# relife957/FastApriori

Hardware: AMD Instinct MI355X
Metric: itemsets/sec (mining wall-clock), T10I4D100M min_sup=0.001 (higher is better)
Workload: dtype int32/uint64-bitmap (exact integer counts); 1 GPU; model=T10I4D100M, global_batch=100000000, parallelism=dp1, n_itemsets=33139, min_count=100000

## Files before the change

### csrc/hip/count.hip

```cpp
#include <algorithm>
#include <cstdlib>

#include "fa_hip.h"
#include "../host/fa_dl.h"
#include "../host/fa_limits.h"
#include "../host/fa_slab.h"

namespace fa {

constexpr int kPB = 128;

__device__ __forceinline__ void tri_index(int pid, int nb, int& bi, int& bj) {
  bi = 0;
  int rem = pid;
  while (rem >= nb - bi) { rem -= nb - bi; ++bi; }
  bj = bi + rem;
}

__device__ __forceinline__ int64_t lower_bound_i32(const int32_t* __restrict__ a, int64_t lo, int64_t hi,
                                                   int32_t key) {
  while (lo < hi) {
    int64_t mid = (lo + hi) >> 1;
    if (a[mid] < key) lo = mid + 1; else hi = mid;
  }
// ... 959 lines not shown
        const uint32_t v = (uint32_t)(acc[i][j][g] + 0.5f);
        if (row < col && col < F1 && v) atomicAdd(&out[(int64_t)row * F1 + col], v * scale);
      }
}

constexpr int kWPT = 8;

template <bool kWeighted>
__global__ __launch_bounds__(256) void k_count_candidates(
    const uint64_t* __restrict__ bm, int64_t Wp, int64_t W, const int32_t* __restrict__ prefix, int m,
    const int64_t* __restrict__ ext_off, const int32_t* __restrict__ ext,
    const int32_t* __restrict__ gb_start, int ngb, const int32_t* __restrict__ wword,
    uint32_t* __restrict__ out) {
  __shared__ uint32_t acc[kMaxBlockExt];
  const uint32_t logical = xcd_remap(blockIdx.x, gridDim.x);
  const int gb = logical % ngb;
  const int64_t sc = logical / ngb;
  const int g0 = gb_start[gb], g1 = gb_start[gb + 1];
  const int64_t e_base = ext_off[g0];
  const int n_ext = (int)(ext_off[g1] - e_base);
  for (int i = threadIdx.x; i < n_ext; i += blockDim.x) acc[i] = 0;
  const int64_t w0 = sc * (256 * kWPT) + threadIdx.x;
  bool valid[kWPT];
  int32_t wt[kWPT];
#pragma unroll
  for (int q = 0; q < kWPT; ++q) {
    valid[q] = w0 + q * 256 < W;
    wt[q] = (kWeighted && valid[q]) ? wword[w0 + q * 256] : 1;
  }
  __syncthreads();
  for (int g = g0; g < g1; ++g) {
    uint64_t p[kWPT];
    const int32_t* pr = prefix + (int64_t)g * m;
    {
      const uint64_t* row = bm + (int64_t)pr[0] * Wp + w0;
#pragma unroll
      for (int q = 0; q < kWPT; ++q) p[q] = valid[q] ? row[q * 256] : 0ull;
    }
    for (int j = 1; j < m; ++j) {
      const uint64_t* row = bm + (int64_t)pr[j] * Wp + w0;
#pragma unroll
      for (int q = 0; q < kWPT; ++q) p[q] &= valid[q] ? row[q * 256] : 0ull;
    }
    for (int64_t e = ext_off[g]; e < ext_off[g + 1]; ++e) {
      const uint64_t* row = bm + (int64_t)ext[e] * Wp + w0;
      uint32_t s = 0;
#pragma unroll
      for (int q = 0; q < kWPT; ++q) {
        const uint64_t v = valid[q] ? (p[q] & row[q * 256]) : 0ull;
        if (kWeighted) s += popc64_acc(v, 0) * (uint32_t)wt[q];
        else s = popc64_acc(v, s);
      }
      s = wave_sum_u32(s);
      if (lane_id() == 0 && s) atomicAdd(&acc[e - e_base], s);
    }
  }
  __syncthreads();
  for (int i = threadIdx.x; i < n_ext; i += blockDim.x)
    if (acc[i]) atomicAdd(&out[e_base + i], acc[i]);
}

enum { kBuildCols = 0, kBuildContig = 1, kBuildBM = 2 };

struct MapGlobal {
  const int32_t* __restrict__ p;
  __device__ __forceinline__ int operator()(int r) const { return p[r]; }
};
struct MapLds {
  const uint16_t* p;
  __device__ __forceinline__ int operator()(int r) const {
    const int v = p[r];
    return v == 0xFFFF ? -1 : v;
  }
};

struct WordSpan {
  int64_t st, base, end;
};
__device__ __forceinline__ WordSpan word_span(const int64_t* __restrict__ roff, int64_t col0, int64_t ncols) {
  const int lane = threadIdx.x & 63;
  return WordSpan{roff[min(col0 + lane, ncols)], roff[col0], roff[min(col0 + 64, ncols)]};
}

template <class Map>
__device__ __forceinline__ void slab_build_word_span(uint64_t* __restrict__ slab, int swp, int q, const WordSpan& ws,
                                                     const int32_t* __restrict__ ranks, Map item_map, int h,
                                                     int nsub, unsigned long long* words, int swz);

template <class Map = MapGlobal>
__device__ __forceinline__ void slab_build_word_m(uint64_t* __restrict__ slab, int swp, int q, int64_t col0,
                                                  int64_t ncols, const int64_t* __restrict__ roff,
                                                  const int32_t* __restrict__ ranks, Map item_map, int h,
                                                  int nsub, unsigned long long* words, int swz = 0) {
  slab_build_word_span(slab, swp, q, word_span(roff, col0, ncols), ranks, item_map, h, nsub, words, swz);
}

template <class Map>
__device__ __forceinline__ void slab_build_word_span(uint64_t* __restrict__ slab, int swp, int q, const WordSpan& ws,
                                                     const int32_t* __restrict__ ranks, Map item_map, int h,
                                                     int nsub, unsigned long long* words, int swz) {
  const int lane = threadIdx.x & 63;
  const int64_t st = ws.st, base = ws.base, end = ws.end;
  const int srel = (int)(st - base);
  const int n = (int)(end - base);
  const unsigned long long le = lanes_le_mask();
  constexpr int U = 2;
  const int step = 64 * U * nsub;
  int rn[U], rn2[U];
#pragma unroll
  for (int u = 0; u < U; ++u) {
    const int p = 64 * U * h + 64 * u + lane;
    rn[u] = p < n ? ranks[base + p] : -1;
    rn2[u] = p + step < n ? ranks[base + p + step] : -1;
  }
  for (int p0 = 64 * U * h; p0 < n; p0 += step) {
    int r[U];
#pragma unroll
    for (int u = 0; u < U; ++u) {
      r[u] = rn[u];
      rn[u] = rn2[u];
      const int p = p0 + 2 * step + 64 * u + lane;
      rn2[u] = p < n ? ranks[base + p] : -1;
    }
    const int cs0 = __popcll(__ballot(srel < p0));
    unsigned long long S[U];
    window_starts<U>(words, srel, p0, S);
    int cs = cs0;
#pragma unroll
    for (int u = 0; u < U; ++u) {
      const int l = cs + __popcll(S[u] & le) - 1;
      const int uu = r[u] >= 0 ? item_map(r[u]) : -1;
      if (uu >= 0) atomicOr((unsigned long long*)(slab + (size_t)uu * swp + (q ^ ((uu << 2) & swz))), 1ull << l);
      cs += __popcll(S[u]);
    }
  }
}

__device__ __forceinline__ void slab_build_word(uint64_t* __restrict__ slab, int swp, int q, int64_t col0,
                                                int64_t ncols, const int64_t* __restrict__ roff,
                                                const int32_t* __restrict__ ranks,
                                                const int32_t* __restrict__ item_map, int h, int nsub,
                                                unsigned long long* words, int swz = 0) {
  slab_build_word_m(slab, swp, q, col0, ncols, roff, ranks, MapGlobal{item_map}, h, nsub, words, swz);
}

template <int SW, int ROWW, bool kSwz>
__device__ __forceinline__ void slab_copy_bm(uint4* lds4, int n_used, const uint64_t* __restrict__ bm, int64_t Wp,
                                             const int32_t* __restrict__ bm_rows, int64_t w0, int64_t W) {
  constexpr int QW = SW / 2;
  constexpr int KMAX = 4;
  const int total = n_used * QW;
  for (int base = 0; base < total; base += KMAX * kSlabThreads) {
    int32_t br[KMAX];
    uint4 v[KMAX];
#pragma unroll
    for (int k = 0; k < KMAX; ++k) {
      const int i = base + (int)threadIdx.x + k * kSlabThreads;
      br[k] = i < total ? (bm_rows ? bm_rows[i / QW] : i / QW) : 0;
    }
#pragma unroll
    for (int k = 0; k < KMAX; ++k) {
      const int i = base + (int)threadIdx.x + k * kSlabThreads;
      const int64_t w = w0 + 2 * (i % QW);
      v[k] = make_uint4(0, 0, 0, 0);
      const int64_t at = Wp > 0 ? (int64_t)br[k] * Wp + w : (w >> 3) * -Wp + (int64_t)br[k] * 8 + (w & 7);
      if (i < total && w < W) v[k] = *reinterpret_cast<const uint4*>(bm + at);
    }
#pragma unroll
    for (int k = 0; k < KMAX; ++k) {
      const int i = base + (int)threadIdx.x + k * kSlabThreads;
      if (i < total) {
        const int u = i / QW, q = i % QW;
        const int qq = kSwz ? (q ^ (((u << 2) & (SW - 4)) >> 1)) : q;
        lds4[(size_t)u * (ROWW / 2) + qq] = v[k];
      }
    }
  }
}

constexpr int kMapLdsMax = kSlabMapMaxF1;

__device__ __forceinline__ uint32_t bcnt_acc(uint32_t x, uint32_t acc) {
  uint32_t r;
  __asm__("v_bcnt_u32_b32 %0, %1, %2" : "=v"(r) : "v"(x), "v"(acc));
  return r;
}

__device__ __forceinline__ uint32_t and3(uint32_t a, uint32_t b, uint32_t c) {
  return __builtin_amdgcn_bitop3_b32(a, b, c, 0x80);
}

__device__ __forceinline__ int u16_at(const int4& v, int k) {
  const int w = (k >> 1) == 0 ? v.x : (k >> 1) == 1 ? v.y : (k >> 1) == 2 ? v.z : v.w;
  return (k & 1) ? (int)((uint32_t)w >> 16) : (w & 0xFFFF);
}

template <int SW, bool kWeighted, int kBuild, bool kCls = false, int kAccB = 4>
__global__ __launch_bounds__(kSlabThreads) void k_count_slab_rec(
    const int64_t* __restrict__ roff, const int32_t* __restrict__ ranks, const int32_t* __restrict__ src,
    int64_t ncols, const int32_t* __restrict__ item_map, int F1, int n_used, const int32_t* __restrict__ gpre,
    const int4* __restrict__ rec, int G_arg, int C, const int32_t* __restrict__ wword, uint32_t* __restrict__ out,
    const uint64_t* __restrict__ bm, int64_t Wp, const int32_t* __restrict__ bm_rows, int flags,
    const int32_t* __restrict__ g_dev) {
  const int G = g_dev ? *g_dev : G_arg;
  extern __shared__ uint4 lds4[];
  __shared__ unsigned long long build_words[kSlabThreads / 64 * 2];
  constexpr int SWP = SW + 2;
  constexpr int RS = SWP / 2;
  uint64_t* slab = reinterpret_cast<uint64_t*>(lds4);
  static_assert(kAccB == 4 || kAccB == 2 || kAccB == 1, "accumulator bytes");
  constexpr bool acc16 = !kWeighted && kAccB == 2;
  constexpr bool acc8 = !kWeighted && kAccB == 1;
  const int nacc = acc16 ? (C + 1) >> 1 : acc8 ? (C + 3) >> 2 : C;
  constexpr int kFlush16 = 65535 / (SW * 64);
  uint32_t* acc = reinterpret_cast<uint32_t*>(slab + (size_t)n_used * SWP);
  uint8_t* acc8p = reinterpret_cast<uint8_t*>(acc);
  uint16_t* smap = reinterpret_cast<uint16_t*>(acc + ((nacc + 3) & ~3));
  const bool map_lds = kBuild == kBuildContig && F1 <= kMapLdsMax;
  for (int i = threadIdx.x; i < nacc; i += blockDim.x) acc[i] = 0;
  if (map_lds) {
    for (int i = threadIdx.x; i < F1; i += blockDim.x) {
      const int v = item_map[i];
      smap[i] = v < 0 ? (uint16_t)0xFFFF : (uint16_t)v;
    }
  }
  const int64_t W = (ncols + 63) >> 6;
  const int64_t nslabs = (W + SW - 1) / SW;
  const int4 z4 = make_int4(0, 0, 0, 0);
  const int ppart = (flags >> kSlabFlagPartShift) & kSlabFlagPartMask;
  const int npart = ((flags >> kSlabFlagNpartsShift) & kSlabFlagPartMask) + 1;
  const int gstep = kSlabThreads * npart;
  const int g0 = (ppart + npart * (int)(threadIdx.x >> 6)) * 64 + (int)(threadIdx.x & 63);
  int4 ra = z4, rb = z4, rc = z4;
  if (g0 < G) { ra = rec[3 * g0]; rb = rec[3 * g0 + 1]; rc = rec[3 * g0 + 2]; }

  auto and_row = [&](uint4 (&p)[SW / 2], int u) {
    const uint4* r = lds4 + (size_t)u * RS;
#pragma unroll
    for (int q = 0; q < SW / 2; ++q) {
      const uint4 v = r[q];
      p[q].x &= v.x; p[q].y &= v.y; p[q].z &= v.z; p[q].w &= v.w;
    }
  };
  auto and_row2 = [&](uint4 (&p)[SW / 2], int u, int w) {
    const uint4* r = lds4 + (size_t)u * RS;
    const uint4* t = lds4 + (size_t)w * RS;
#pragma unroll
    for (int q = 0; q < SW / 2; ++q) {
      const uint4 v = r[q], x = t[q];
      p[q].x = and3(p[q].x, v.x, x.x); p[q].y = and3(p[q].y, v.y, x.y);
      p[q].z = and3(p[q].z, v.z, x.z); p[q].w = and3(p[q].w, v.w, x.w);
    }
  };
  auto pid = [&](int j) { return j < 4 ? u16_at(ra, 4 + j) : u16_at(rc, j - 4); };
  auto and_prefix = [&](uint4 (&p)[SW / 2], int j0, int j1) {
#pragma unroll
    for (int j = 1; j < 12; j += 2) {
      if (j >= j0 && j < j1) {
        if (j + 1 < j1) and_row2(p, pid(j), pid(j + 1));
        else and_row(p, pid(j));
      }
    }
  };
  auto acc_add = [&](int e, uint32_t v) {
    if (acc8) {
      uint32_t t = (uint32_t)acc8p[e] + v;
      if (t > 255u) { atomicAdd(&out[e], t); t = 0; }
      acc8p[e] = (uint8_t)t;
    } else if (acc16) {
      atomicAdd(&acc[e >> 1], v << ((e & 1) << 4));
    } else {
      atomicAdd(&acc[e], v);
    }
  };
  auto flush = [&]() {
    for (int i = threadIdx.x; i < nacc; i += blockDim.x) {
      const uint32_t v = acc[i];
      if (!v) continue;
      if (acc8) {
#pragma unroll
        for (int b = 0; b < 4; ++b) {
          const uint32_t c = (v >> (8 * b)) & 0xFFu;
          if (c && 4 * i + b < C) atomicAdd(&out[4 * i + b], c);
        }
        acc[i] = 0;
      } else if (acc16) {
        if (v & 0xFFFFu) atomicAdd(&out[2 * i], v & 0xFFFFu);
        if ((v >> 16) && 2 * i + 1 < C) atomicAdd(&out[2 * i + 1], v >> 16);
        acc[i] = 0;
      } else {
        atomicAdd(&out[i], v);
      }
    }
  };
  int nsl = 0;
  constexpr int kNW = kSlabThreads / 64;
  constexpr bool kOneWord = kBuild == kBuildContig && SW <= 8 && SW * (kNW > SW ? kNW / SW : 1) == kNW;
  const int my_q = (int)(threadIdx.x >> 6) / (kNW > SW ? kNW / SW : 1);
  WordSpan span{0, 0, 0};
  auto load_span = [&](int64_t sb_) {
    const int64_t col0 = (sb_ * SW + my_q) * 64;
    if (kOneWord && sb_ < nslabs && col0 < ncols) span = word_span(roff, col0, ncols);
  };
  load_span(blockIdx.x);

  for (int64_t sb = blockIdx.x; sb < nslabs; sb += gridDim.x) {
    const int64_t w0 = sb * SW;
    __syncthreads();
    if (acc16 && ++nsl > kFlush16) {
      flush();
      nsl = 1;
    }
    if (kBuild == kBuildBM) {
      slab_copy_bm<SW, SWP, false>(lds4, n_used, bm, Wp, bm_rows, w0, W);
    } else {
      {
        const uint4 z = make_uint4(0, 0, 0, 0);
        for (int i = threadIdx.x; i < n_used * RS; i += blockDim.x) lds4[i] = z;
      }
      __syncthreads();
      if (kBuild == kBuildContig) {
        constexpr int NW = kSlabThreads / 64;
        constexpr int NSUB = NW > SW ? NW / SW : 1;
        const int wv = threadIdx.x >> 6;
        if (kOneWord) {
          const int q = wv / NSUB;
          if ((w0 + q) * 64 < ncols) {
            if (map_lds)
              slab_build_word_span(slab, SWP, q, span, ranks, MapLds{smap}, wv % NSUB, NSUB, build_words + wv * 2, 0);
            else
              slab_build_word_span(slab, SWP, q, span, ranks, MapGlobal{item_map}, wv % NSUB, NSUB,
                                   build_words + wv * 2, 0);
          }
        } else {
          for (int q = wv / NSUB; q < SW; q += NW / NSUB) {
            if ((w0 + q) * 64 >= ncols) continue;
            if (map_lds)
              slab_build_word_m(slab, SWP, q, (w0 + q) * 64, ncols, roff, ranks, MapLds{smap}, wv % NSUB, NSUB,
                                build_words + wv * 2);
            else
              slab_build_word_m(slab, SWP, q, (w0 + q) * 64, ncols, roff, ranks, MapGlobal{item_map}, wv % NSUB,
                                NSUB, build_words + wv * 2);
          }
        }
      } else {
        for (int j = threadIdx.x; j < SW * 64; j += blockDim.x) {
          const int64_t col = w0 * 64 + j;
          if (col >= ncols) break;
          const int64_t row = src ? (int64_t)src[col] : col;
          if (row < 0) continue;
          const unsigned long long bit = 1ull << (j & 63);
          uint64_t* base = slab + (j >> 6);
          for (int64_t r = roff[row], r1 = roff[row + 1]; r < r1; ++r) {
            const int uu = item_map[ranks[r]];
            if (uu >= 0) atomicOr((unsigned long long*)(base + (size_t)uu * SWP), bit);
          }
        }
      }
    }
    __syncthreads();
    load_span(sb + gridDim.x);
    uint32_t wt[SW];
#pragma unroll
    for (int q = 0; q < SW; ++q) wt[q] = kWeighted ? ((w0 + q < W) ? (uint32_t)wword[w0 + q] : 0u) : 1u;
    uint4 p[SW / 2], qv[SW / 2];
    for (int g = g0; g < G; g += gstep) {
      const int gn = g + gstep < G ? g + gstep : g0;
      const int4 na = rec[3 * gn], nb = rec[3 * gn + 1], nc = rec[3 * gn + 2];
      const int n_ext = ra.y & 0xFF, m = (ra.y >> 8) & 0xFF;
      if constexpr (kCls) {
        const int fl = (ra.y >> 17) & 3;
        if (!(fl & 1)) {
          const uint4* r0 = lds4 + (size_t)(ra.z & 0xFFFF) * RS;
#pragma unroll
          for (int q = 0; q < SW / 2; ++q) qv[q] = r0[q];
          and_prefix(qv, 1, m - 1);
        }
        if (!(fl & 2)) {
          const uint4* rl = lds4 + (size_t)((uint32_t)ra.y >> 19) * RS;
#pragma unroll
          for (int q = 0; q < SW / 2; ++q) {
            const uint4 v = rl[q];
            p[q].x = qv[q].x & v.x; p[q].y = qv[q].y & v.y; p[q].z = qv[q].z & v.z; p[q].w = qv[q].w & v.w;
          }
        }
      } else {
      {
        const uint4* r0 = lds4 + (size_t)(ra.z & 0xFFFF) * RS;
#pragma unroll
        for (int q = 0; q < SW / 2; ++q) p[q] = r0[q];
      }
      if (!((ra.y >> 16) & 1)) {
        and_prefix(p, 1, m);
      } else {
        const int32_t* pr = gpre + rc.x;
        int j = 1;
        for (; j + 1 < m; j += 2) and_row2(p, pr[j], pr[j + 1]);
        if (j < m) and_row(p, pr[j]);
      }
      }
      uint32_t any = flags & kSlabFlagDense;
      if (!any) {
#pragma unroll
        for (int q = 0; q < SW / 2; ++q) any |= p[q].x | p[q].y | p[q].z | p[q].w;
      }
      if (any) {
        const int e0 = ra.x;
        constexpr int UE = SW <= 8 ? 2 : 1;
#pragma unroll
        for (int k = 0; k < 8; k += UE) {
          if (k >= n_ext) break;
          uint32_t s[UE];
          const uint4* r[UE];
#pragma unroll
          for (int x = 0; x < UE; ++x) {
            s[x] = 0;
            r[x] = lds4 + (size_t)u16_at(rb, k + x < n_ext ? k + x : k) * RS;
          }
#pragma unroll
          for (int q = 0; q < SW / 2; ++q) {
#pragma unroll
            for (int x = 0; x < UE; ++x) {
              const uint4 v = r[x][q];
              if (kWeighted) {
                s[x] += (uint32_t)(__popc(p[q].x & v.x) + __popc(p[q].y & v.y)) * wt[2 * q] +
                        (uint32_t)(__popc(p[q].z & v.z) + __popc(p[q].w & v.w)) * wt[2 * q + 1];
              } else {
                s[x] = bcnt_acc(p[q].x & v.x, s[x]); s[x] = bcnt_acc(p[q].y & v.y, s[x]);
                s[x] = bcnt_acc(p[q].z & v.z, s[x]); s[x] = bcnt_acc(p[q].w & v.w, s[x]);
              }
            }
          }
#pragma unroll
          for (int x = 0; x < UE; ++x)
            if (k + x < n_ext && s[x]) acc_add(e0 + k + x, s[x]);
        }
      }
      ra = na; rb = nb; rc = nc;
    }
  }
  __syncthreads();
  flush();
}

struct MapIdent {
  __device__ __forceinline__ int operator()(int r) const { return r; }
};

constexpr int kBwThreads = 1024;

template <class Map>
__global__ __launch_bounds__(kBwThreads) void k_build_bitmaps_w(const int64_t* __restrict__ roff,
                                                         const int32_t* __restrict__ ranks, int64_t ncols, int F1,
                                                         int64_t rs, int64_t bs, int WT, uint64_t* __restrict__ bm,
                                                         Map map) {
  extern __shared__ uint64_t btile[];
  __shared__ unsigned long long bwords[kBwThreads / 64 * 2];
  for (int i = threadIdx.x; i < F1 * WT; i += blockDim.x) btile[i] = 0ull;
  __syncthreads();
  const int wv = threadIdx.x >> 6;
  constexpr int NW = kBwThreads / 64;
  const int nsub = NW > WT ? NW / WT : 1;
  for (int q = wv / nsub; q < WT; q += NW / nsub) {
    const int64_t col0 = ((int64_t)blockIdx.x * WT + q) * 64;
    if (col0 < ncols)
      slab_build_word_span(btile, WT, q, word_span(roff, col0, ncols), ranks, map, wv % nsub, nsub, bwords + wv * 2,
                           0);
  }
  __syncthreads();
  const int64_t w0 = (int64_t)blockIdx.x * WT;
  for (int i = threadIdx.x; i < F1 * WT; i += blockDim.x) {
    const int u = i / WT, w = i - u * WT;
    bm[((w0 + w) >> 3) * bs + (int64_t)u * rs + ((w0 + w) & 7)] = btile[i];
  }
}

}

using namespace fa;

FA_API int fa_hip_build_bitmaps_wave(const int64_t* roff, const int32_t* ranks, int64_t ncols, int32_t F1, int64_t Wp,
                                     int WT, uint64_t* bm, const int32_t* item_map, int blocked, hipStream_t st) {
  const size_t lds = (size_t)F1 * WT * 8;
  if (F1 <= 0 || WT <= 0 || Wp % WT || Wp % 8 || lds > 64 * 1024) return 2;
  const int64_t rs = blocked ? 8 : Wp, bs = blocked ? 8 * (int64_t)F1 : 8;
  dim3 g((unsigned)(Wp / WT));
  if (item_map) {
    (void)hipFuncSetAttribute((const void*)k_build_bitmaps_w<MapGlobal>, hipFuncAttributeMaxDynamicSharedMemorySize,
                              (int)lds);
    hipLaunchKernelGGL(k_build_bitmaps_w<MapGlobal>, g, dim3(kBwThreads), lds, st, roff, ranks, ncols, F1, rs, bs, WT, bm,
                       MapGlobal{item_map});
  } else {
    (void)hipFuncSetAttribute((const void*)k_build_bitmaps_w<MapIdent>, hipFuncAttributeMaxDynamicSharedMemorySize,
                              (int)lds);
    hipLaunchKernelGGL(k_build_bitmaps_w<MapIdent>, g, dim3(kBwThreads), lds, st, roff, ranks, ncols, F1, rs, bs, WT, bm,
                       MapIdent{});
  }
  FA_LAUNCH_RET();
}


FA_API int fa_hip_pair_gram_mfma(const uint64_t* bm, int32_t F1, int64_t rs, int64_t bs, int woff, int64_t W,
                                 uint32_t* out, int target_wgs, uint32_t scale, int fp4, hipStream_t st) {
  if (woff < 0 || woff > 7) return -22;
  const BmView v{bm, rs, bs, woff};
  if (W <= 0 || F1 < 2) return 0;
  const int nt = (F1 + kMT4 - 1) / kMT4;
  const int ntp = nt * (nt + 1) / 2;
  int64_t nk = std::max<int64_t>(1, (target_wgs + ntp - 1) / ntp);
  int64_t kchunk = (W + nk - 1) / nk;
  kchunk = std::max<int64_t>(kMW, (kchunk + kMW - 1) / kMW * kMW);
  if (fp4) kchunk = std::min<int64_t>(kchunk, (int64_t)1 << 18);
  nk = (W + kchunk - 1) / kchunk;
  if (fp4)
    hipLaunchKernelGGL(k_pair_gram_fp4, dim3((unsigned)(nk * ntp)), dim3(256), 0, st, v, F1, W, nt,
                       ntp, kchunk, out, scale);
  else
    hipLaunchKernelGGL(k_pair_gram_mfma4<false>, dim3((unsigned)(nk * ntp)), dim3(256), 0, st, v, F1, W, nt,
                       ntp, kchunk, out, scale);
  FA_LAUNCH_RET();
}

FA_API int fa_hip_pair_gram_popc(const uint64_t* bm, int32_t F1, int64_t rs, int64_t bs, int woff, int64_t W,
                                 const int32_t* wword, uint32_t* out, int target_wgs, hipStream_t st) {
  if (woff < 0 || woff > 7) return -22;
  if (W <= 0 || F1 < 2) return 0;
  const BmView v{bm, rs, bs, woff};
  const int nt = (F1 + kGT - 1) / kGT;
  const int ntp = nt * (nt + 1) / 2;
  int64_t nk = std::max<int64_t>(1, (target_wgs + ntp - 1) / ntp);
  int64_t kchunk = (W + nk - 1) / nk;
  kchunk = std::max<int64_t>(kGK, (kchunk + kGK - 1) / kGK * kGK);
  nk = (W + kchunk - 1) / kchunk;
  dim3 g((unsigned)(nk * ntp));
  if (wword)
    hipLaunchKernelGGL(k_pair_gram_popc<true>, g, dim3(256), 0, st, v, F1, W, wword, nt, ntp, kchunk, out);
  else
    hipLaunchKernelGGL(k_pair_gram_popc<false>, g, dim3(256), 0, st, v, F1, W, wword, nt, ntp, kchunk, out);
  FA_LAUNCH_RET();
}

FA_API int fa_hip_count_candidates(const uint64_t* bm, int64_t Wp, int64_t W, const int32_t* prefix,
                                   int m, const int64_t* ext_off, const int32_t* ext,
                                   const int32_t* gb_start, int ngb, const int32_t* wword,
                                   uint32_t* out, hipStream_t st) {
  if (ngb <= 0 || W <= 0) return 0;
  const int64_t nsc = (W + 256 * kWPT - 1) / (256 * kWPT);
  dim3 g((unsigned)(nsc * ngb));
  if (wword)
    hipLaunchKernelGGL(k_count_candidates<true>, g, dim3(256), 0, st, bm, Wp, W, prefix, m, ext_off, ext, gb_start, ngb, wword, out);
// ... 74 lines not shown
  {
    uint64_t m = m0, mk = ~m0 << 1;
#pragma unroll
    for (int i = 0; i < 6; ++i) {
      uint64_t mp = mk ^ (mk << 1);
      mp ^= mp << 2; mp ^= mp << 4; mp ^= mp << 8; mp ^= mp << 16; mp ^= mp << 32;
      mv[i] = mp & m;
      m = (m ^ mv[i]) | (mv[i] >> (1 << i));
      mk &= ~mp;
    }
  }
  for (int u0 = 0; u0 < n_items; u0 += kWinBatch) {
    const int nb = min(kWinBatch, n_items - u0);
    uint64_t x[kWinBatch];
#pragma unroll
    for (int b = 0; b < kWinBatch; ++b) x[b] = (n && b < nb) ? bm_word(bm, ld, rows[u0 + b], q) : 0ull;
    for (int i = lane; i < nb * 66; i += 64) (&buf[0][0])[i] = 0ull;
    wave_lds_sync();
    if (n) {
      const int w = s >> 6, sh = s & 63;
#pragma unroll
      for (int b = 0; b < kWinBatch; ++b) {
        if (b >= nb) break;
        uint64_t y = x[b] & m0;
#pragma unroll
        for (int i = 0; i < 6; ++i) {
          const uint64_t t = y & mv[i];
          y = (y ^ t) | (t >> (1 << i));
        }
        atomicOr(&buf[b][w], (unsigned long long)(y << sh));
        if (sh + n > 64) atomicOr(&buf[b][w + 1], (unsigned long long)(y >> (64 - sh)));
      }
    }
    wave_lds_sync();
    for (int b = 0; b < nb; ++b) {
      const int64_t u = u0 + b;
      for (int j = lane; j < nwords; j += 64) {
        const unsigned long long v = buf[b][j];
        const int64_t gw = w0 + j;
        uint64_t* o = ldo > 0 ? out + u * ldo + gw : out + (gw >> 3) * -ldo + u * 8 + (gw & 7);
        if (j == 0 || j == nwords - 1) {
          if (v) atomicOr(reinterpret_cast<unsigned long long*>(o), v);
        } else {
          *o = v;
        }
      }
    }
    wave_lds_sync();
  }
}

FA_API int fa_hip_win_alive(const uint64_t* bm, int64_t ld, const int32_t* rows, int n_items, int64_t W, int k,
                            uint64_t* alive, int32_t* cnt, hipStream_t st) {
  if (W <= 0) return 0;
  int planes = 1;
  while ((1 << planes) <= n_items) ++planes;
  if (n_items < 1 || planes > kWinPlanes || k < 1 || ld == 0) return 1;
  hipLaunchKernelGGL(k_win_alive, dim3((unsigned)((W + 255) / 256)), dim3(256), 0, st, bm, ld, rows, n_items, W, k,
                     planes, alive, cnt);
  FA_LAUNCH_RET();
}

FA_API int fa_hip_win_compact(const uint64_t* bm, int64_t ld, const int32_t* rows, int n_items, int64_t W,
                              const uint64_t* alive, const int64_t* off, uint64_t* out, int64_t ldo, hipStream_t st) {
  if (W <= 0 || n_items < 1) return 0;
  if (ld == 0 || ldo == 0) return 1;
  hipLaunchKernelGGL(k_win_compact, dim3((unsigned)((W + 255) / 256)), dim3(256), 0, st, bm, ld, rows, n_items, W,
                     alive, off, out, ldo);
  FA_LAUNCH_RET();
}

static int g_slab_max_wg = 0;
FA_API void fa_hip_debug_slab_max_wg(int n) { g_slab_max_wg = n; }
static int g_piece_part = 0, g_piece_nparts = 1;
FA_API int fa_hip_set_piece_part(int part, int nparts) {
  if (nparts < 1 || nparts > 256 || part < 0 || part >= nparts) return 1;
  g_piece_part = part;
  g_piece_nparts = nparts;
  return 0;
}

FA_API int fa_hip_count_slab_rec_cls(const int64_t* roff, const int32_t* ranks, const int32_t* src, int64_t ncols,
                                     const int32_t* item_map, int F1, int n_used, const int32_t* gpre,
                                     const void* rec, int G, int C, const int32_t* wword, uint32_t* out, int sw,
                                     int n_wg, const uint64_t* bm, int64_t Wp, hipStream_t st,
                                     const int32_t* bm_rows, const int32_t* g_dev, int cls) {
  if ((G <= 0 && !g_dev) || C <= 0 || ncols <= 0) return 0;
  if (g_piece_nparts > 1) cls &= ~kSlabCls;
  const int accb = slab_mode_acc_bytes(cls, wword != nullptr);
  const bool acc16 = accb == 2;
  const int64_t n_acc = slab_acc_count(C, accb);
  const bool contig = !bm && !src;
  const size_t lds = (size_t)slab_kernel_lds(n_used, sw, slab_acc_words(n_acc), contig ? slab_map_lds(F1) : 0);
  if (lds > 160 * 1024 - 256) return 3;
  if (g_slab_max_wg > 0) n_wg = std::min(n_wg, g_slab_max_wg);
  using KernT = void (*)(const int64_t*, const int32_t*, const int32_t*, int64_t, const int32_t*, int, int,
                         const int32_t*, const int4*, int, int, const int32_t*, uint32_t*, const uint64_t*, int64_t,
                         const int32_t*, int, const int32_t*);
  KernT kern = nullptr;
#define FA_REC_MODE(S, B)                                                                              \
  kern = wword ? (KernT)k_count_slab_rec<S, true, B>                                                   \
         : (cls & kSlabCls) ? (accb == 1 ? (KernT)k_count_slab_rec<S, false, B, true, 1>               \
                               : accb == 2 ? (KernT)k_count_slab_rec<S, false, B, true, 2>             \
                                           : (KernT)k_count_slab_rec<S, false, B, true, 4>)            \
                            : (accb == 1 ? (KernT)k_count_slab_rec<S, false, B, false, 1>              \
                               : accb == 2 ? (KernT)k_count_slab_rec<S, false, B, false, 2>            \
                                           : (KernT)k_count_slab_rec<S, false, B, false, 4>);
#define FA_REC_CASE(S)                                    \
  if (sw == S) {                                          \
    if (bm) { FA_REC_MODE(S, kBuildBM) }                  \
    else if (src) { FA_REC_MODE(S, kBuildCols) }          \
    else { FA_REC_MODE(S, kBuildContig) }                 \
  }
  FA_REC_CASE(4)
  FA_REC_CASE(8)
  FA_REC_CASE(16)
  FA_REC_CASE(32)
#undef FA_REC_CASE
#undef FA_REC_MODE
  if (!kern) return 1;
  (void)hipFuncSetAttribute((const void*)kern, hipFuncAttributeMaxDynamicSharedMemorySize, (int)lds);
  const int flags = ((cls & kSlabDense) ? kSlabFlagDense : 0) | (acc16 ? kSlabFlagAcc16 : 0) |
                    (g_piece_part << kSlabFlagPartShift) | ((g_piece_nparts - 1) << kSlabFlagNpartsShift);
  hipLaunchKernelGGL(kern, dim3((unsigned)n_wg), dim3(kSlabThreads), lds, st, roff, ranks, src, ncols, item_map, F1,
                     n_used, gpre, (const int4*)rec, G, C, wword, out, bm, Wp, bm_rows, flags, g_dev);
  FA_LAUNCH_RET();
}

FA_API int fa_hip_block_counts(const int64_t* roff, const int32_t* ranks, int64_t T, int32_t F1, uint8_t* cnt,
                               int64_t* bsum, int pb, hipStream_t st) {
  if (T <= 0) return 0;
  const int nb = (F1 + pb - 1) / pb;
  const int64_t nbatch = (T + 63) / 64;
  const int lpb = __builtin_ctz((unsigned)pb);
  if (nb <= kWBMaxNB && (1 << lpb) == pb)
    hipLaunchKernelGGL(k_block_counts_w, dim3((unsigned)((nbatch + 3) / 4)), dim3(256), 0, st, roff, ranks, T, nb,
                       cnt, bsum, nbatch, lpb);
  else
    hipLaunchKernelGGL(k_block_counts, dim3((unsigned)((nbatch + 3) / 4)), dim3(256), 0, st, roff, ranks, T, nb, cnt,
                       bsum, nbatch, pb);
  FA_LAUNCH_RET();
}

FA_API int fa_hip_block_scatter(const int64_t* roff, const int32_t* ranks, int64_t T, int32_t F1,
                                const uint8_t* cnt, const int64_t* base, uint8_t* lr, int pb, hipStream_t st) {
  if (T <= 0) return 0;
  const int nb = (F1 + pb - 1) / pb;
  const int64_t nbatch = (T + 63) / 64;
  const int lpb = __builtin_ctz((unsigned)pb);
  if (nb <= kWBMaxNB && (1 << lpb) == pb)
    hipLaunchKernelGGL(k_block_scatter_w, dim3((unsigned)((nbatch + 3) / 4)), dim3(256), 0, st, roff, ranks, T, nb,
                       cnt, base, nbatch, lr, lpb);
  else
    hipLaunchKernelGGL(k_block_scatter, dim3((unsigned)((nbatch + 3) / 4)), dim3(256), 0, st, roff, ranks, T, nb, cnt,
                       base, nbatch, lr, pb);
  FA_LAUNCH_RET();
}

FA_API int fa_hip_pair_blocked(const uint8_t* cnt, const int64_t* base, const uint8_t* lr, int64_t T,
                               const int32_t* wrow, int32_t F1, uint32_t* out, int64_t chunk_rows, hipStream_t st) {
  if (T <= 0 || F1 < 2) return 0;
  const int nb = (F1 + kPB - 1) / kPB;
  const int nbp = nb * (nb + 1) / 2;
  const int64_t nbatch = (T + 63) / 64;
  const int64_t chunk_b = std::max<int64_t>(kPW, (chunk_rows + 63) / 64);
  const int64_t nch = (nbatch + chunk_b - 1) / chunk_b;
  hipLaunchKernelGGL(k_pair_blocked, dim3((unsigned)(nch * nbp)), dim3(64 * kPW), 0, st, cnt, base, lr, T, nbatch,
                     wrow, F1, nb, nbp, chunk_b, out);
  FA_LAUNCH_RET();
}

FA_API int fa_hip_pair_queue16(const uint8_t* cnt, const int64_t* base, const uint8_t* lr, int64_t T, int32_t F1,
                               int64_t ld, int* qctr, uint32_t* out, int n_wg, hipStream_t st) {
  if (T <= 0 || F1 < 2) return 0;
  const int nb = (F1 + kPB16 - 1) / kPB16;
  const int nbp = nb * (nb + 1) / 2;
  const int64_t nbatch = (T + 63) / 64;
  const int nsub = (int)((nbatch + kQSubB - 1) / kQSubB);
  if (n_wg <= 0) {
    int dev = 0, ncu = 256;
    if (hipGetDevice(&dev) == hipSuccess) hipDeviceGetAttribute(&ncu, hipDeviceAttributeMultiprocessorCount, dev);
    n_wg = ncu;
  }
  n_wg = (int)std::min<int64_t>(n_wg, (int64_t)nsub * nbp);
  hipLaunchKernelGGL(k_pair_queue16, dim3((unsigned)n_wg), dim3(64 * kPW), 0, st, cnt, base, lr, T, nbatch, F1, ld,
                     nb, nbp, qctr, nsub, out);
  FA_LAUNCH_RET();
}

FA_API int fa_hip_pairs_compact(const uint32_t* pc, int64_t ld, int32_t F1, int64_t mc, int32_t* row_cnt,
                                int64_t* row_off, int32_t* rows, int32_t* cnt, int64_t* n_out, hipStream_t st) {
  if (F1 < 2) return 1;
  hipLaunchKernelGGL(k_pairs_keep_count, dim3((unsigned)F1), dim3(256), 0, st, pc, ld, F1, mc, row_cnt);
  hipLaunchKernelGGL(k_pairs_scan, dim3(1), dim3(1024), 0, st, row_cnt, F1, row_off, n_out);
  hipLaunchKernelGGL(k_pairs_emit, dim3((unsigned)F1), dim3(256), 0, st, pc, ld, F1, mc, row_off, rows, cnt);
  FA_LAUNCH_RET();
}
```

### csrc/hip/gen.hip

```cpp
#include <hipcub/hipcub.hpp>

#include <algorithm>
#include <cmath>

#include "fa_hip.h"
#include "../host/fa_dl.h"
#include "../host/fa_limits.h"
#include "../host/fa_slab.h"

namespace fa {

__device__ __forceinline__ uint64_t ag_mix(uint64_t x) {
  x ^= x >> 33; x *= 0xff51afd7ed558ccdull; x ^= x >> 33; x *= 0xc4ceb9fe1a85ec53ull; x ^= x >> 33;
  return x;
}

__device__ __forceinline__ uint64_t ag_hash_drop(const int32_t* __restrict__ r, int m, int skip) {
  uint64_t h = 0x9E3779B97F4A7C15ull ^ (uint64_t)(m - 1);
  for (int q = 0; q < m; ++q)
    if (q != skip) h = ag_mix(h ^ (uint32_t)r[q]);
  return h;
}

__device__ __forceinline__ bool ag_eq_drop(const int32_t* __restrict__ a, const int32_t* __restrict__ b, int m,
// ... 618 lines not shown
    nz += v[u] > 0;
  }
  const int tz[2] = {t, nz};
  int64_t pre[2], tot[2];
  wg_scan_excl<16>(tz, wpart, pre, tot);
  int64_t run = pre[0];
#pragma unroll
  for (int u = 0; u < 4; ++u) {
    const int64_t i = b0 + 4 * (int64_t)threadIdx.x + u;
    run += v[u];
    if (i < n) off[i + 1] = run;
  }
  if (threadIdx.x == 0) {
    bs[blockIdx.x] = tot[0];
    bs[nblk + blockIdx.x] = tot[1];
  }
}

__global__ __launch_bounds__(1024) void k_ds_decide0(int64_t* __restrict__ off, long long* __restrict__ c,
                                                     int64_t* __restrict__ bs, int nblk, int64_t c_bound) {
  if (c[kDlStop]) return;
  __shared__ int64_t part[16];
  if (threadIdx.x == 0) off[0] = 0;
  int64_t z = 0;
  const int64_t C = wg_scan_chunks<16>(
      nblk, 0, part, [&](int64_t q) { return bs[q]; },
      [&](int64_t q, int64_t before, int64_t) {
        bs[2 * nblk + q] = before;
        z += bs[nblk + q];
      });
  const int64_t gz = wg_sum<16>(z, part);
  if (threadIdx.x != 0) return;
  c[kDlCl] = C;
  c[kDlGl] = gz;
  if (C == 0) { c[kDlEnd] = 1; c[kDlStop] = 1; return; }
  if (C > c_bound) { c[kDlMulti] = 1; c[kDlStop] = 1; return; }
  c[kDlLevels] = 1; c[kDlTotal] = C; c[kDlLastC] = C; c[kDlNl + 1] = C;
}

__global__ __launch_bounds__(1024) void k_ds_add(int64_t* __restrict__ off, const long long* __restrict__ c,
                                                 const int64_t* __restrict__ bs, int nblk) {
  if (c[kDlOverBound]) return;
  const int64_t n = c[kDlNl];
  const int64_t b0 = (int64_t)blockIdx.x * kDsBlk;
  if (b0 >= n || blockIdx.x == 0) return;
  const int64_t base = bs[2 * nblk + blockIdx.x];
  for (int k = threadIdx.x; k < kDsBlk; k += 1024) {
    const int64_t i = b0 + k;
    if (i < n) off[i + 1] += base;
  }
}

__global__ __launch_bounds__(256) void k_dl_mark(const int32_t* __restrict__ rows, int m1,
                                                 long long* __restrict__ c, int w32) {
  __shared__ uint32_t lb[2 * kDlBitsW];
  if (c[kDlStop] && !c[kDlMulti]) return;
  for (int q = threadIdx.x; q < w32; q += 256) lb[q] = 0u;
  __syncthreads();
  const int64_t n = c[kDlMulti] ? 0 : c[kDlCl] * (int64_t)m1;
  for (int64_t i = (int64_t)blockIdx.x * 256 + threadIdx.x; i < n; i += (int64_t)gridDim.x * 256)
    atomicOr(&lb[rows[i] >> 5], 1u << (rows[i] & 31));
  __syncthreads();
  uint32_t* mk = reinterpret_cast<uint32_t*>(c + kDlBits);
  for (int q = threadIdx.x; q < w32; q += 256)
    if (lb[q]) atomicOr(&mk[q], lb[q]);
}

__global__ __launch_bounds__(64) void k_dl_post0(long long* __restrict__ c, double lds, double accb, int w32) {
  if (blockIdx.x != 0) return;
  const uint32_t* mk = reinterpret_cast<const uint32_t*>(c + kDlBits);
  uint32_t part = 0;
  for (int q = threadIdx.x; q < w32; q += 64) part += __popc(mk[q]);
  const int64_t n_used = (int64_t)wave_sum_u32(part);
  if (threadIdx.x != 0) return;
  c[kDlNUsed] = n_used;
  if (c[kDlLevels] == 1 && c[kDlCl] > slab_cap(n_used, c[kDlCl], lds, accb)) {
    c[kDlMulti] = 1;
    c[kDlStop] = 1;
  }
}

__global__ __launch_bounds__(1024) void k_dl_decide(const int32_t* __restrict__ cnt, int64_t* __restrict__ off,
                                                     long long* __restrict__ c, int l, double growth, int64_t c_bound,
                                                     double lds, double accb) {
  if (c[kDlStop]) return;
  int64_t g = 0;
  const int64_t C = agd_block_scan<true>(cnt, off, c[kDlNl + l], &g);
  if (threadIdx.x != 0) return;
  const int64_t total = c[kDlTotal], last = c[kDlLastC];
  if (C == 0 || (double)C > growth * (double)last || C > c_bound ||
      total + C > slab_cap(c[kDlNUsed], total + C, lds, accb)) {
    c[kDlStop] = 1;
    if (C == 0) c[kDlEmpty] = 1;
    return;
  }
  c[kDlCl + l] = C;
  c[kDlGl + l] = g;
  c[kDlLevels] = l + 1;
  c[kDlTotal] = total + C;
  c[kDlLastC] = C;
  c[kDlNl + l + 1] = C;
}

template <bool kEmit, int NWL = 1>
__global__ __launch_bounds__(256) void k_dl_rows(const int32_t* __restrict__ P, int m,
                                                 const int32_t* __restrict__ table, uint32_t mask, int nw,
                                                 const unsigned long long* __restrict__ ext, int32_t* __restrict__ cnt,
                                                 const int64_t* __restrict__ off, int32_t* __restrict__ rows,
                                                 const long long* __restrict__ c, int l, int32_t* __restrict__ ntab,
                                                 uint32_t ncap, unsigned long long* __restrict__ next_ext) {
  if (c[kDlStop]) return;
  const int64_t n = c[kDlNl + l];
  if (!kEmit && ntab) {
    const int64_t stride = (int64_t)gridDim.x * blockDim.x;
    for (int64_t q = (int64_t)blockIdx.x * blockDim.x + threadIdx.x; q < (int64_t)ncap; q += stride) ntab[q] = -1;
  }
  const int lane = threadIdx.x & 63;
  const int64_t nwave = (int64_t)gridDim.x * (blockDim.x / 64);
  for (int64_t i = (int64_t)blockIdx.x * (blockDim.x / 64) + (threadIdx.x >> 6); i < n; i += nwave) {
    unsigned long long a[NWL];
    const int cc = ag_row_bits<NWL>(P, i, m, table, mask, nw, ext, lane, a);
    const int incl = wave_scan_incl_dpp(cc);
    if (!kEmit) {
      if (lane == 63) cnt[i] = incl;
      continue;
    }
    const int64_t o = off[i];
    ag_emit<NWL>(a, lane, P + i * m, m, o + (incl - cc), cnt + n, rows);
    if (next_ext && wave_last(incl) > 0) {
#pragma unroll
      for (int j = 0; j < NWL; ++j)
        if (lane * NWL + j < nw) next_ext[o * nw + lane * NWL + j] = a[j];
      if (lane == 0) {
        const int32_t* x = P + i * m;
        uint64_t h = 0x9E3779B97F4A7C15ull ^ (uint64_t)m;
        for (int q = 0; q < m; ++q) h = ag_mix(h ^ (uint32_t)x[q]);
        uint32_t at = (uint32_t)h & (ncap - 1);
        while (atomicCAS(&ntab[at], -1, (int32_t)o) != -1) at = (at + 1) & (ncap - 1);
      }
    }
  }
}

}

FA_API int fa_hip_dl_level0(const int32_t* P0, const long long* n_src, int64_t n_const, int64_t n_bound, int m0,
                            int F1, void* ws, int64_t ws_bytes, long long* ctl, long long* ctl_host,
                            int64_t c_bound, double lds, double accb, int64_t* info, int sync, hipStream_t st) {
  if (m0 < 2 || F1 > kAgMaxF1 || F1 < 1 || n_bound < 0 || c_bound < 1) return 1;
  auto al = [](int64_t b) { return (b + 255) & ~(int64_t)255; };
  const int nw = (F1 + 63) / 64;
  const int64_t nb = std::max<int64_t>(n_bound, 1);
  uint32_t cap = 16;
  while (cap < 2 * (uint64_t)nb) cap <<= 1;
  const int nds = nb > 4 * kDsBlk ? (int)((nb + kDsBlk - 1) / kDsBlk) : 0;
  const int64_t need = al(4 * (int64_t)cap) + al(8 * nb * nw) + al(8 * (nb + 1)) + al(4 * (nb + c_bound)) +
                       al(4 * c_bound * (m0 + 1)) + al(8 * 3 * (int64_t)nds);
  info[0] = need;
  if (need > ws_bytes) return 5;
  char* w = static_cast<char*>(ws);
  int32_t* table = reinterpret_cast<int32_t*>(w); w += al(4 * (int64_t)cap);
  unsigned long long* ext = reinterpret_cast<unsigned long long*>(w); w += al(8 * nb * nw);
  int64_t* off = reinterpret_cast<int64_t*>(w); w += al(8 * (nb + 1));
  int32_t* cnt = reinterpret_cast<int32_t*>(w); w += al(4 * (nb + c_bound));
  int32_t* rows = reinterpret_cast<int32_t*>(w); w += al(4 * c_bound * (m0 + 1));
  int64_t* ds = reinterpret_cast<int64_t*>(w);
  info[1] = (int64_t)(intptr_t)cnt; info[2] = (int64_t)(intptr_t)off; info[3] = (int64_t)(intptr_t)rows;
  hipLaunchKernelGGL(k_dl_setup0, dim3(1), dim3(kDlCtl), 0, st, ctl, n_src, n_const, m0 + 1, nb);
  AgdClear clr{};
  clr.p[0] = reinterpret_cast<uint32_t*>(table); clr.len[0] = cap; clr.val[0] = ~0u;
  clr.p[1] = reinterpret_cast<uint32_t*>(ext); clr.len[1] = 2 * nb * nw; clr.val[1] = 0u;
  clr.nreg = 2;
  const int64_t clr_max = std::max<int64_t>(cap, 2 * nb * nw);
  hipLaunchKernelGGL(k_agd_clear, dim3((unsigned)std::min<int64_t>((clr_max + 255) / 256, 1024)), dim3(256), 0, st,
                     clr, ctl);
  const dim3 g((unsigned)std::min<int64_t>((nb + 255) / 256, 512));
  hipLaunchKernelGGL(k_agd_insert, g, dim3(256), 0, st, P0, m0, table, cap - 1, ctl, 0);
  hipLaunchKernelGGL(k_agd_ext, g, dim3(256), 0, st, P0, m0, table, cap - 1, nw, ext, ctl, 0);
  const unsigned nwg = (unsigned)std::min<int64_t>((nb + 3) / 4, 2048);
#define FA_DL0_ROWS(E, N)                                                                                   \
  hipLaunchKernelGGL((k_agd_rows<E, N>), dim3(nwg), dim3(256), 0, st, P0, m0, table, cap - 1, nw, ext, cnt, off, \
                     rows, ctl, 0);
#define FA_DL0_CNT(N) FA_DL0_ROWS(false, N)
#define FA_DL0_EMIT(N) FA_DL0_ROWS(true, N)
  FA_AG_NWL_SWITCH(nw, FA_DL0_CNT)
  if (nds) {
    hipLaunchKernelGGL(k_ds_blocks, dim3((unsigned)nds), dim3(1024), 0, st, cnt, off, ctl, ds, nds);
    hipLaunchKernelGGL(k_ds_decide0, dim3(1), dim3(1024), 0, st, off, ctl, ds, nds, c_bound);
    hipLaunchKernelGGL(k_ds_add, dim3((unsigned)nds), dim3(1024), 0, st, off, ctl, ds, nds);
  } else {
    hipLaunchKernelGGL(k_dl_decide0, dim3(1), dim3(1024), 0, st, cnt, off, ctl, c_bound);
  }
  FA_AG_NWL_SWITCH(nw, FA_DL0_EMIT)
#undef FA_DL0_EMIT
#undef FA_DL0_CNT
#undef FA_DL0_ROWS
  const int w32 = (F1 + 31) / 32;
  hipLaunchKernelGGL(k_dl_mark, dim3((unsigned)std::min<int64_t>((c_bound * (m0 + 1) + 255) / 256, 1024)), dim3(256),
                     0, st, rows, m0 + 1, ctl, w32);
  hipLaunchKernelGGL(k_dl_post0, dim3(1), dim3(64), 0, st, ctl, lds, accb, w32);
  if (sync) {
    (void)hipMemcpyAsync(ctl_host, ctl, sizeof(long long) * kDlCtl, hipMemcpyDeviceToHost, st);
    if (hipStreamSynchronize(st) != hipSuccess) return 7;
  }
  FA_LAUNCH_RET();
}

static void dl_post(DlPost* P, const DlDesc* desc, int L, long long* ctl, const long long* ch, int F1,
                    double accb_rule, hipStream_t st) {
  P->done = 0;
  if (ch[kDlStop] && ch[kDlLevels] == 0) return;
  if (ch[kDlOverBound] || ch[kDlMulti] || ch[kDlEnd] || L < 1) return;
  int64_t C = 0, R = 0;
  for (int l = 0; l < L; ++l) { C += desc[l].C; R += desc[l].n; }
  const int64_t n_used = ch[kDlNUsed];
  P->C = C;
  if (C < 1 || C > P->rec_cap || C > P->out_cap || 8 * ((R + 255) / 256) > P->part_cap) return;
  int64_t cap = 0;
  int sw = slab_width(n_used, C, P->lds_budget, accb_rule, &cap);
  if (sw == 0 || C > cap) return;
  double accb = accb_rule;
  if (!P->wword) slab_acc_upgrade(n_used, C, P->lds_budget, P->accb, &sw, &cap, &accb);
  P->accb = accb;
  if (fa_hip_dl_plan(desc, L, ctl, F1, P->item_map, P->rec, C, P->part, P->part_cap, P->gpre, P->gpre_cap, sw,
                     st) != 0)
    return;
  (void)hipMemsetAsync(P->out, 0, 4 * (size_t)C, st);
  P->sw = sw;
  P->cap = cap;
  P->done = 1;
  P->trim = 0;
  if (!P->trim_ok || P->T <= 0) {
  } else if (!P->len_hist || P->T < P->trim_min_rows) {
    if (!P->len_hist && P->T >= P->trim_min_rows) return;
  } else {
    const uint64_t* mk = reinterpret_cast<const uint64_t*>(ch + kDlBits);
    double num = 0.0, den = 0.0;
    for (int r = 0; r < F1; ++r) {
      if (P->alive[r]) den += (double)P->c1[r];
      if ((mk[r >> 6] >> (r & 63)) & 1ull) num += (double)P->c1[r];
    }
    if (den > 0.0) {
      double est_rows = 0.0, est_nnz = 0.0;
      trim_estimate(P->len_hist, kTrimHist, num / den, (int)P->k, &est_rows, &est_nnz);
      const double T = (double)std::max<int64_t>(P->T, 1), nnz = (double)std::max<int64_t>(P->nnz, 1);
      P->trim = (est_rows < P->trim_rows_frac * T || est_nnz < P->trim_nnz_frac * nnz) ? 1 : 0;
    }
  }
  if (P->trim) return;
  const int64_t W = (P->ncols + 63) / 64, nslabs = (W + sw - 1) / sw;
  const bool weighted = P->wword != nullptr;
  const int64_t nacc = slab_acc_count(C, slab_acc_bytes(P->accb, weighted));
  P->n_wg = slab_workgroups(nslabs, (int64_t)P->lds_kernel,
                            slab_kernel_lds(n_used, sw, slab_acc_words(nacc), slab_map_lds(F1)));
  if (fa_hip_count_slab_rec_cls(P->roff, P->ranks, P->src, P->ncols, P->item_map, F1, (int)n_used, P->gpre, P->rec,
                                0, (int)C, P->wword, P->out, sw, (int)P->n_wg, nullptr, 0, st, nullptr,
                                reinterpret_cast<const int32_t*>(ctl + kDlPiecesI32),
                                slab_acc_mode(P->accb, weighted)) != 0)
    return;
  P->done = 2;
}

FA_API int fa_hip_dl_more(int F1, void* ws, int64_t ws_bytes, int64_t ws_used, long long* ctl, long long* ctl_host,
                          double growth, int max_levels, double lds, double accb, int64_t n1_bound, fa::DlDesc* desc,
                          int64_t* info, hipStream_t st, void* post) {
  using namespace fa;
  auto al = [](int64_t b) { return (b + 255) & ~(int64_t)255; };
  const int nw = (F1 + 63) / 64;
  char* const w0 = static_cast<char*>(ws);
  char* w = w0 + ws_used;
  const int LM = std::min(max_levels, kDlMaxLevels);
  const int64_t acc_max = (int64_t)(lds / accb);
  int64_t nb = n1_bound;
  int m = (int)desc[0].m + 1;
  const int32_t* P = reinterpret_cast<const int32_t*>((intptr_t)desc[0].rows);
  struct Lv { int32_t* cnt; int64_t* off; int32_t* rows; int m; };
  Lv lv[kDlMaxL];
  static long long* mirror = nullptr;
  static hipEvent_t ev[2];
  if (!mirror) {
    if (hipHostMalloc(reinterpret_cast<void**>(&mirror), 2 * sizeof(long long) * kDlCtl) != hipSuccess) return 7;
    for (int k = 0; k < 2; ++k) (void)hipEventCreateWithFlags(&ev[k], hipEventDisableTiming);
  }
  int nbatch = 0;
  struct Tab { int32_t* table = nullptr; uint32_t cap = 0; unsigned long long* ext = nullptr; };
  Tab cur;
  auto tab_alloc = [&](int64_t rows, Tab& t) -> bool {
    uint32_t cap = 16;
    while (cap < 2 * (uint64_t)rows) cap <<= 1;
    const int64_t need = al(4 * (int64_t)cap) + al(8 * rows * nw);
    if ((w - w0) + need > ws_bytes) { info[0] = 2 * ((w - w0) + need); return false; }
    t.table = reinterpret_cast<int32_t*>(w); w += al(4 * (int64_t)cap);
    t.ext = reinterpret_cast<unsigned long long*>(w); w += al(8 * rows * nw);
    t.cap = cap;
    return true;
  };
  auto enqueue = [&](int l0) -> int {
    const int l1 = std::min(LM - 1, l0 + kAgdBatch - 1);
    for (int l = l0; l <= l1; ++l) {
      const int64_t cb = std::min<int64_t>(acc_max, (int64_t)(growth * (double)nb) + 1);
      if (l == 1) {
        if (!tab_alloc(nb, cur)) return 5;
        AgdClear clr{};
        clr.p[0] = reinterpret_cast<uint32_t*>(cur.table); clr.len[0] = cur.cap; clr.val[0] = ~0u;
        clr.p[1] = reinterpret_cast<uint32_t*>(cur.ext); clr.len[1] = 2 * nb * nw; clr.val[1] = 0u;
        clr.nreg = 2;
        const int64_t clr_max = std::max<int64_t>(cur.cap, 2 * nb * nw);
        hipLaunchKernelGGL(k_agd_clear, dim3((unsigned)std::min<int64_t>((clr_max + 255) / 256, 1024)), dim3(256), 0,
                           st, clr, ctl);
        const dim3 g((unsigned)std::min<int64_t>((nb + 255) / 256, 512));
        hipLaunchKernelGGL(k_agd_insert, g, dim3(256), 0, st, P, m, cur.table, cur.cap - 1, ctl, l);
        hipLaunchKernelGGL(k_agd_ext, g, dim3(256), 0, st, P, m, cur.table, cur.cap - 1, nw, cur.ext, ctl, l);
      }
      const int64_t need = al(8 * (nb + 1)) + al(4 * (nb + cb)) + al(4 * cb * (m + 1));
      if ((w - w0) + need > ws_bytes) {
        info[0] = 2 * ((w - w0) + need);
        return 5;
      }
      lv[l].off = reinterpret_cast<int64_t*>(w); w += al(8 * (nb + 1));
      lv[l].cnt = reinterpret_cast<int32_t*>(w); w += al(4 * (nb + cb));
      lv[l].rows = reinterpret_cast<int32_t*>(w); w += al(4 * cb * (m + 1));
      lv[l].m = m;
      Tab nxt;
      if (l + 1 < LM && !tab_alloc(cb, nxt)) return 5;
      const unsigned nwg = (unsigned)std::min<int64_t>((nb + 3) / 4, 2048);
#define FA_DLR(E, N)                                                                                          \
      hipLaunchKernelGGL((k_dl_rows<E, N>), dim3(nwg), dim3(256), 0, st, P, m, cur.table, cur.cap - 1, nw,      \
                         cur.ext, lv[l].cnt, lv[l].off, lv[l].rows, ctl, l, nxt.table, nxt.cap, nxt.ext);
#define FA_DLR_CNT(N) FA_DLR(false, N)
#define FA_DLR_EMIT(N) FA_DLR(true, N)
      FA_AG_NWL_SWITCH(nw, FA_DLR_CNT)
      hipLaunchKernelGGL(k_dl_decide, dim3(1), dim3(1024), 0, st, lv[l].cnt, lv[l].off, ctl, l, growth, cb, lds,
                         accb);
      FA_AG_NWL_SWITCH(nw, FA_DLR_EMIT)
#undef FA_DLR_EMIT
#undef FA_DLR_CNT
#undef FA_DLR
      P = lv[l].rows;
      cur = nxt;
      nb = cb;
      ++m;
    }
    long long* hb = mirror + (nbatch & 1) * kDlCtl;
    (void)hipMemcpyAsync(hb, ctl, sizeof(long long) * kDlCtl, hipMemcpyDeviceToHost, st);
    (void)hipEventRecord(ev[nbatch & 1], st);
    ++nbatch;
    return 0;
  };
  int next = 1;
  int rc = 0;
  for (int q = 0; q < 2 && next < LM && rc == 0; ++q, next += kAgdBatch) rc = enqueue(next);
  for (int waited = 0; rc == 0 && waited < nbatch; ++waited) {
    if (hipEventSynchronize(ev[waited & 1]) != hipSuccess) return 7;
    if (mirror[(waited & 1) * kDlCtl + kDlStop]) break;
    if (next < LM) { rc = enqueue(next); next += kAgdBatch; }
  }
  (void)hipMemcpyAsync(ctl_host, ctl, sizeof(long long) * kDlCtl, hipMemcpyDeviceToHost, st);
  if (hipStreamSynchronize(st) != hipSuccess) return 7;
  if (rc) return rc;
  desc[0].n = ctl_host[kDlNl];
  desc[0].C = ctl_host[kDlCl];
  desc[0].base = 0;
  const int L = (int)ctl_host[kDlLevels];
  for (int l = 1; l < L; ++l) {
    DlDesc& d = desc[l];
    d.P = desc[l - 1].rows;
    d.cnt = (int64_t)(intptr_t)lv[l].cnt;
    d.off = (int64_t)(intptr_t)lv[l].off;
    d.rows = (int64_t)(intptr_t)lv[l].rows;
    d.m = lv[l].m;
    d.n = ctl_host[kDlNl + l];
    d.C = ctl_host[kDlCl + l];
    d.base = desc[l - 1].base + desc[l - 1].C;
  }
  info[0] = w - w0;
  if (post) dl_post(static_cast<DlPost*>(post), desc, L, ctl, ctl_host, F1, accb, st);
  FA_LAUNCH_RET();
}
```

### csrc/hip/levels.hip

```cpp
#include "fa_hip.h"
#include "../host/fa_dl.h"

namespace fa {

struct DlLevels {
  const int32_t* P[kDlMaxL];
  const int32_t* cnt[kDlMaxL];
  const int64_t* off[kDlMaxL];
  const int32_t* rows[kDlMaxL];
  int64_t n[kDlMaxL];
  int64_t C[kDlMaxL];
  int64_t base[kDlMaxL];
  int64_t rbase[kDlMaxL + 1];
  int m[kDlMaxL];
  int64_t gbase[kDlMaxL];
  int32_t* gpre;
  int64_t w0, w1;
  int L;
};

__device__ __forceinline__ int dl_level_of(const DlLevels& D, int64_t t) {
  int l = 0;
  while (l + 1 < D.L && t >= D.rbase[l + 1]) ++l;
  return l;
}

__global__ __launch_bounds__(64) void k_dl_map(const uint64_t* __restrict__ mk, int F1, int32_t* __restrict__ item_map) {
  __shared__ int pre[kDlBitsW];
  const int lane = threadIdx.x;
  const int nwd = (F1 + 63) >> 6;
  int cnt8[8], tot = 0;
#pragma unroll
  for (int j = 0; j < 8; ++j) {
    const int w = lane * 8 + j;
    cnt8[j] = w < nwd ? __popcll(mk[w]) : 0;
    tot += cnt8[j];
  }
  int run = wave_scan_incl_dpp(tot) - tot;
#pragma unroll
  for (int j = 0; j < 8; ++j) {
    pre[lane * 8 + j] = run;
    run += cnt8[j];
  }
  __syncthreads();
  for (int r = lane; r < F1; r += 64) {
    const uint64_t ww = mk[r >> 6];
    const int b = r & 63;
    item_map[r] = ((ww >> b) & 1ull) ? pre[r >> 6] + __popcll(ww & ((1ull << b) - 1ull)) : -1;
  }
}

constexpr int kDlPB = 256;

__device__ __forceinline__ int dl_bucket_count(int cc, int b) { return b == 8 ? (cc >> 3) : ((cc & 7) == b ? 1 : 0); }

__device__ __forceinline__ int dl_row_window(const DlLevels& D, int64_t t, int64_t R, int64_t* first) {
  if (t >= R) return 0;
  const int l = dl_level_of(D, t);
  const int64_t i = t - D.rbase[l];
  const int cc = D.cnt[l][i];
  if (cc == 0) return 0;
  const int64_t cb = D.base[l] + D.off[l][i], ce = cb + cc;
  const int64_t a = cb > D.w0 ? cb : D.w0, b = ce < D.w1 ? ce : D.w1;
  if (first) *first = a;
  return b > a ? (int)(b - a) : 0;
}

__device__ __forceinline__ int dl_row_count(const DlLevels& D, int64_t t, int64_t R) {
  return dl_row_window(D, t, R, nullptr);
}

__global__ __launch_bounds__(kDlPB) void k_dl_pieces_count(const DlLevels D, int32_t* __restrict__ part) {
  __shared__ int sh[8 * (kDlPB / 64)];
  const int64_t R = D.rbase[D.L];
  const int64_t t = (int64_t)blockIdx.x * kDlPB + threadIdx.x;
  const int cc = dl_row_count(D, t, R);
  int v[8], tot[8];
#pragma unroll
  for (int b = 1; b <= 8; ++b) v[b - 1] = dl_bucket_count(cc, b);
  wg_sum<kDlPB / 64>(v, sh, tot);
  if (threadIdx.x == 0) {
#pragma unroll
    for (int b = 0; b < 8; ++b) part[(int64_t)blockIdx.x * 8 + b] = tot[b];
  }
// ... 23 lines not shown
  for (int k = 0; k < 8; ++k) e8[k] = k < n_ext ? item_map[ex[k]] : 0;
  int4 a, b, cc;
  a.x = (int)cand;
  a.y = n_ext | (m << 8) | (goff >= 0 ? 1 << 16 : 0);
  a.z = (int)dl_pk(ids[0], ids[1]);
  a.w = (int)dl_pk(ids[2], ids[3]);
  b.x = (int)dl_pk(e8[0], e8[1]); b.y = (int)dl_pk(e8[2], e8[3]);
  b.z = (int)dl_pk(e8[4], e8[5]); b.w = (int)dl_pk(e8[6], e8[7]);
  cc.x = (int)dl_pk(ids[4], ids[5]); cc.y = (int)dl_pk(ids[6], ids[7]);
  cc.z = (int)dl_pk(ids[8], ids[9]); cc.w = (int)dl_pk(ids[10], ids[11]);
  if (goff >= 0) cc.x = (int)goff;
  rec[3 * p] = a; rec[3 * p + 1] = b; rec[3 * p + 2] = cc;
}

__global__ __launch_bounds__(kDlPB) void k_dl_pieces_emit(const DlLevels D, const int32_t* __restrict__ part,
                                                          const int32_t* __restrict__ item_map,
                                                          int4* __restrict__ rec) {
  __shared__ int sh[8 * (kDlPB / 64)];
  const int64_t R = D.rbase[D.L];
  const int64_t t = (int64_t)blockIdx.x * kDlPB + threadIdx.x;
  int64_t first = 0;
  const int cc = dl_row_window(D, t, R, &first);
  int v[8], excl[8], tot[8];
#pragma unroll
  for (int b = 1; b <= 8; ++b) v[b - 1] = dl_bucket_count(cc, b);
  wg_scan_excl<kDlPB / 64>(v, sh, excl, tot);
  if (cc == 0) return;
  int64_t slot[9];
#pragma unroll
  for (int b = 1; b <= 8; ++b) slot[b] = (int64_t)part[(int64_t)blockIdx.x * 8 + (b - 1)] + excl[b - 1];
  const int l = dl_level_of(D, t);
  const int64_t i = t - D.rbase[l];
  const int m = D.m[l];
  const int32_t* x = D.P[l] + i * m;
  int ids[kDlInline];
#pragma unroll
  for (int q = 0; q < kDlInline; ++q) ids[q] = q < m ? item_map[x[q]] : 0;
  int64_t goff = -1;
  if (m > kDlInline) {
    goff = D.gbase[l] + i * m;
    for (int q = 0; q < m; ++q) D.gpre[goff + q] = item_map[x[q]];
  }
  const int64_t o = D.off[l][i] + (first - (D.base[l] + D.off[l][i]));
  const int32_t* ex = D.cnt[l] + D.n[l] + o;
  const int64_t cand = first - D.w0;
  const int full = cc >> 3;
  for (int j = 0; j < full; ++j)
    dl_write_rec(rec, slot[8] + j, cand + 8 * j, 8, m, ids, ex + 8 * j, item_map, goff);
  const int rem = cc & 7;
  if (rem) dl_write_rec(rec, slot[rem], cand + 8 * full, rem, m, ids, ex + 8 * full, item_map, goff);
}

constexpr int kLaWs = 4;
constexpr int kLaMaxPos = kDlInline + 8;

__device__ __forceinline__ int la_u16(const int4& v, int k) {
  const int w = (k >> 1) == 0 ? v.x : (k >> 1) == 1 ? v.y : (k >> 1) == 2 ? v.z : v.w;
  return (k & 1) ? (int)((uint32_t)w >> 16) : (w & 0xFFFF);
}

__device__ __forceinline__ int la_row(const int4& a, const int4& b, const int4& c, int m, int pos) {
  if (pos < m) return pos < 4 ? la_u16(a, 4 + pos) : la_u16(c, pos - 4);
  return la_u16(b, pos - m);
}

__device__ __forceinline__ int la_row_min(int v) {
  v = min(v, __builtin_amdgcn_update_dpp(v, v, 0x128, 0xf, 0xf, false));
  v = min(v, __builtin_amdgcn_update_dpp(v, v, 0x124, 0xf, 0xf, false));
  v = min(v, __builtin_amdgcn_update_dpp(v, v, 0x122, 0xf, 0xf, false));
  v = min(v, __builtin_amdgcn_update_dpp(v, v, 0x121, 0xf, 0xf, false));
  return v;
}

__device__ __forceinline__ int la_qsum(int v) {
  const auto a = __builtin_amdgcn_permlane16_swap(v, v, false, false);
  v = (int)a[0] + (int)a[1];
  const auto b = __builtin_amdgcn_permlane32_swap(v, v, false, false);
  return (int)b[0] + (int)b[1];
}

__global__ __launch_bounds__(64) void k_la_qsum_probe(int* out) { out[threadIdx.x] = la_qsum((int)threadIdx.x); }

__global__ __launch_bounds__(64) void k_dl_lane_assign(int4* __restrict__ rec, const long long* __restrict__ c,
                                                       int rs) {
  constexpr int NW = 64 * kLaWs, NG = 4 * kLaWs;
  constexpr int kPq = kLaMaxPos / 4;
  __shared__ int4 win[3 * NW];
  __shared__ uint16_t rws[NW][kLaMaxPos];
  __shared__ uint32_t st[kLaMaxPos][16][NG];
  __shared__ int16_t dst[NW];
  const int G = reinterpret_cast<const int32_t*>(c + kDlPiecesI32)[0];
  const int64_t base = (int64_t)blockIdx.x * NW;
  if (base + NW > G) return;
  const int lane = threadIdx.x;
  for (int i = lane; i < 3 * NW; i += 64) win[i] = rec[3 * base + i];
  for (int i = lane; i < NG * kLaMaxPos * 16; i += 64) (&st[0][0][0])[i] = 0xFFFFu;
  wave_lds_sync();
  const int y0 = win[0].y & 0x1FFFF;
  bool same = true;
  for (int i = lane; i < NW; i += 64) same = same && (win[3 * i].y & 0x1FFFF) == y0;
  if (__ballot(!same) != 0ull) return;
  const int n_ext = y0 & 0xFF, m = (y0 >> 8) & 0xFF;
  if ((y0 >> 16) || m > kDlInline || m + n_ext > kLaMaxPos) return;
  const int R = m + n_ext;
  for (int i = lane; i < NW; i += 64) {
    const int4 a = win[3 * i], b = win[3 * i + 1], cc = win[3 * i + 2];
    for (int pos = 0; pos < R; ++pos) rws[i][pos] = (uint16_t)la_row(a, b, cc, m, pos);
  }
  wave_lds_sync();
  const int g = lane & 15, q = lane >> 4;
  int fill = 0;
  int rn[kPq];
#pragma unroll
  for (int t = 0; t < kPq; ++t) {
    const int v = (int)rws[0][q + 4 * t < R ? q + 4 * t : 0];
    rn[t] = q + 4 * t < R ? v : -1;
  }
  for (int i = 0; i < NW; ++i) {
    int rr[kPq];
    uint32_t w[kPq];
#pragma unroll
    for (int t = 0; t < kPq; ++t) rr[t] = rn[t];
    const int i1 = i + 1 < NW ? i + 1 : i;
#pragma unroll
    for (int t = 0; t < kPq; ++t) {
      const int pos = q + 4 * t;
      const bool ok = pos < R;
      const int pc = ok ? pos : 0;
      const uint32_t sv = st[pc][(rr[t] * rs) & 15][g];
      const int rv = (int)rws[i1][pc];
      w[t] = ok ? sv : 0xFFFFu;
      rn[t] = ok ? rv : -1;
    }
    int cost = 0;
#pragma unroll
    for (int t = 0; t < kPq; ++t) {
      const int o = (int)(w[t] & 0xFFFF);
      if (o != 0xFFFF && o != rr[t]) cost += (int)(w[t] >> 16);
    }
    cost = la_qsum(cost);
    if (fill >= 16) cost = 1 << 20;
    const int win_g = la_row_min((cost << 4) | g) & 15;
    if (g == win_g) {
#pragma unroll
      for (int t = 0; t < kPq; ++t) {
        const int pos = q + 4 * t;
        const int o = (int)(w[t] & 0xFFFF);
        const uint32_t nv = o == 0xFFFF ? ((uint32_t)rr[t] | (1u << 16)) : (o != rr[t] ? w[t] + (1u << 16) : w[t]);
        if (pos < R) st[pos][(rr[t] * rs) & 15][g] = nv;
      }
      if (q == 0) {
        const int gg = g & 3, k = fill;
        const int l16 = gg == 0 ? (k < 4 ? k : k < 8 ? 8 + k : 12 + k)
                      : gg == 1 ? (k < 8 ? 4 + k : k < 12 ? 8 + k : 16 + k)
                      : gg == 2 ? 32 + (k < 4 ? k : k < 8 ? 8 + k : 12 + k)
                                : 32 + (k < 8 ? 4 + k : k < 12 ? 8 + k : 16 + k);
        dst[i] = (int16_t)(64 * (g >> 2) + l16);
      }
      ++fill;
    }
  }
  wave_lds_sync();
  for (int i = lane; i < NW; i += 64) {
    const int64_t d = base + dst[i];
    rec[3 * d] = win[3 * i]; rec[3 * d + 1] = win[3 * i + 1]; rec[3 * d + 2] = win[3 * i + 2];
  }
}

struct DlOut {
  int64_t rows_off[kDlMaxL];
  int64_t cnt_off[kDlMaxL];
};

__global__ __launch_bounds__(1024) void k_dl_threshold(const DlLevels D, const DlOut O,
                                                       const uint32_t* __restrict__ counts, int64_t mc,
                                                       int32_t* __restrict__ rows_out, int32_t* __restrict__ cnt_out,
                                                       long long* __restrict__ fsz) {
  __shared__ int part[16];
  for (int l = 0; l < D.L; ++l) {
    const int w = D.m[l] + 1;
    const uint32_t* cl = counts + D.base[l];
    const int32_t* src = D.rows[l];
    int32_t* ro = rows_out + O.rows_off[l];
    int32_t* co = cnt_out + O.cnt_off[l];
    uint32_t v;
    const int64_t kept = wg_scan_chunks<16>(
        D.C[l], 0, part, [&](int64_t e) { v = cl[e]; return (int64_t)v >= mc ? 1 : 0; },
        [&](int64_t e, int64_t at, int keep) {
          if (!keep) return;
          co[at] = (int32_t)v;
          for (int q = 0; q < w; ++q) ro[at * w + q] = src[e * w + q];
        });
    if (threadIdx.x == 0) fsz[l] = kept;
  }
}

constexpr int kThB = 1024;
struct DlThrBlk {
  int64_t blk_base[kDlMaxL + 1];
};

__device__ __forceinline__ int dlt_level(const DlThrBlk& B, int L, int64_t b) {
  int l = 0;
  while (l + 1 < L && b >= B.blk_base[l + 1]) ++l;
  return l;
}

__global__ __launch_bounds__(256) void k_dlt_count(const DlLevels D, const DlThrBlk B,
                                                   const uint32_t* __restrict__ counts, int64_t mc,
                                                   int32_t* __restrict__ part) {
  const int64_t b = blockIdx.x;
  const int l = dlt_level(B, D.L, b);
  const int64_t C = D.C[l], e0 = (b - B.blk_base[l]) * kThB;
  const uint32_t* cl = counts + D.base[l];
  uint32_t k = 0;
#pragma unroll
  for (int u = 0; u < kThB / 256; ++u) {
    const int64_t e = e0 + threadIdx.x + 256 * u;
    k += (e < C && (int64_t)cl[e] >= mc) ? 1u : 0u;
  }
  __shared__ uint32_t ws[4];
  k = wg_sum<4>(k, ws);
  if (threadIdx.x == 0) part[b] = (int32_t)k;
}

__global__ __launch_bounds__(1024) void k_dlt_scan(const DlThrBlk B, int L, int32_t* __restrict__ part,
                                                  long long* __restrict__ fsz) {
  __shared__ int wpart[16];
  for (int l = 0; l < L; ++l) {
    int32_t* pl = part + B.blk_base[l];
    const int64_t kept = wg_scan_chunks<16>(
        B.blk_base[l + 1] - B.blk_base[l], 0, wpart, [&](int64_t i) { return pl[i]; },
// ... 55 lines not shown
  int64_t g = 0;
  for (int l = 0; l < L; ++l) {
    const DlDesc& d = desc[l];
    D->P[l] = reinterpret_cast<const int32_t*>((intptr_t)d.P);
    D->cnt[l] = reinterpret_cast<const int32_t*>((intptr_t)d.cnt);
    D->off[l] = reinterpret_cast<const int64_t*>((intptr_t)d.off);
    D->rows[l] = reinterpret_cast<const int32_t*>((intptr_t)d.rows);
    D->m[l] = (int)d.m;
    D->n[l] = d.n;
    D->C[l] = d.C;
    D->base[l] = d.base;
    D->rbase[l + 1] = D->rbase[l] + d.n;
    if (D->m[l] < 1 || D->m[l] > kDlMaxM) return 1;
    D->gbase[l] = -1;
    if (D->m[l] > kDlInline) {
      D->gbase[l] = g;
      g += d.n * D->m[l];
    }
  }
  if (g > 0 && gpre_cap >= 0 && (gpre == nullptr || g > gpre_cap)) return 1;
  return 0;
}

}

using namespace fa;

FA_API int fa_hip_dl_plan_window(const DlDesc* desc, int L, long long* ctl, int F1, int32_t* item_map, void* rec,
                                 int64_t max_pieces, int32_t* part, int64_t part_cap, int32_t* gpre,
                                 int64_t gpre_cap, int64_t w0, int64_t w1, int sw, hipStream_t st);
FA_API int fa_hip_dl_plan_window_bits(const DlDesc* desc, int L, long long* ctl, int F1, const uint64_t* used_bits,
                                      int32_t* item_map, void* rec, int64_t max_pieces, int32_t* part,
                                      int64_t part_cap, int32_t* gpre, int64_t gpre_cap, int64_t w0, int64_t w1,
                                      int sw, hipStream_t st);

FA_API int fa_hip_debug_la_qsum(int* out, hipStream_t st) {
  hipLaunchKernelGGL(k_la_qsum_probe, dim3(1), dim3(64), 0, st, out);
  FA_LAUNCH_RET();
}

static int g_lane_on = 0;
FA_API void fa_hip_set_lane_deal(int on) { g_lane_on = on; }

FA_API int fa_hip_dl_plan(const DlDesc* desc, int L, long long* ctl, int F1, int32_t* item_map, void* rec,
                          int64_t max_pieces, int32_t* part, int64_t part_cap, int32_t* gpre, int64_t gpre_cap,
                          int sw, hipStream_t st) {
  return fa_hip_dl_plan_window(desc, L, ctl, F1, item_map, rec, max_pieces, part, part_cap, gpre, gpre_cap, 0, -1, sw,
                               st);
}

FA_API int fa_hip_dl_plan_window(const DlDesc* desc, int L, long long* ctl, int F1, int32_t* item_map, void* rec,
                                 int64_t max_pieces, int32_t* part, int64_t part_cap, int32_t* gpre,
                                 int64_t gpre_cap, int64_t w0, int64_t w1, int sw, hipStream_t st) {
  return fa_hip_dl_plan_window_bits(desc, L, ctl, F1, nullptr, item_map, rec, max_pieces, part, part_cap, gpre,
                                    gpre_cap, w0, w1, sw, st);
}

FA_API int fa_hip_dl_plan_window_bits(const DlDesc* desc, int L, long long* ctl, int F1, const uint64_t* used_bits,
                                      int32_t* item_map, void* rec, int64_t max_pieces, int32_t* part,
                                      int64_t part_cap, int32_t* gpre, int64_t gpre_cap, int64_t w0, int64_t w1,
                                      int sw, hipStream_t st) {
  DlLevels D;
  if (dl_levels(desc, L, &D, gpre, gpre_cap)) return 1;
  if (F1 < 1 || F1 > kAgMaxF1) return 1;
  int64_t C = 0;
  for (int l = 0; l < L; ++l) C += D.C[l];
  D.w0 = w0 < 0 ? 0 : w0;
  D.w1 = w1 < 0 ? C : std::min(w1, C);
  if (D.w1 <= D.w0) return 1;
  if (max_pieces < D.w1 - D.w0) return 1;
  const int64_t R = D.rbase[L];
  const int64_t nblk = std::max<int64_t>(1, (R + kDlPB - 1) / kDlPB);
  if (part_cap < 8 * nblk) return 1;
  const uint64_t* mk = used_bits ? used_bits : reinterpret_cast<const uint64_t*>(ctl + kDlBits);
  hipLaunchKernelGGL(k_dl_map, dim3(1), dim3(64), 0, st, mk, F1, item_map);
  hipLaunchKernelGGL(k_dl_pieces_count, dim3((unsigned)nblk), dim3(kDlPB), 0, st, D, part);
  hipLaunchKernelGGL(k_dl_pieces_scan, dim3(1), dim3(1024), 0, st, part, nblk, ctl);
  hipLaunchKernelGGL(k_dl_pieces_emit, dim3((unsigned)nblk), dim3(kDlPB), 0, st, D, part, item_map,
                     static_cast<int4*>(rec));
  if (g_lane_on && sw > 0) {
    const int64_t nwin = (D.w1 - D.w0) / (64 * kLaWs);
    if (nwin > 0)
      hipLaunchKernelGGL(k_dl_lane_assign, dim3((unsigned)nwin), dim3(64), 0, st, static_cast<int4*>(rec), ctl,
                         (sw + 2) / 2);
  }
  FA_LAUNCH_RET();
}

__global__ __launch_bounds__(256) void k_dl_chunk_bits(const int32_t* __restrict__ rows, int64_t C, int w, int chunk,
                                                       int nwd, unsigned long long* __restrict__ out) {
  __shared__ unsigned long long lb[kDlBitsW];
  for (int i = threadIdx.x; i < nwd; i += 256) lb[i] = 0ull;
  __syncthreads();
  const int64_t c0 = (int64_t)blockIdx.x * chunk, c1 = min(C, c0 + chunk);
  for (int64_t e = c0 * w + threadIdx.x; e < c1 * w; e += 256) {
    const int r = rows[e];
    atomicOr(&lb[r >> 6], 1ull << (r & 63));
  }
  __syncthreads();
  for (int i = threadIdx.x; i < nwd; i += 256) out[(int64_t)blockIdx.x * nwd + i] = lb[i];
}

FA_API int fa_hip_dl_chunk_bits(const DlDesc* desc, int F1, int chunk, uint64_t* out, hipStream_t st) {
  const int nwd = (F1 + 63) / 64;
  const int64_t C = desc[0].C;
  if (F1 < 1 || nwd > kDlBitsW || chunk < 1 || C < 1) return 1;
  const int32_t* rows = reinterpret_cast<const int32_t*>((intptr_t)desc[0].rows);
  const int64_t nch = (C + chunk - 1) / chunk;
  hipLaunchKernelGGL(k_dl_chunk_bits, dim3((unsigned)nch), dim3(256), 0, st, rows, C, (int)desc[0].m + 1, chunk, nwd,
                     reinterpret_cast<unsigned long long*>(out));
  FA_LAUNCH_RET();
}

FA_API int fa_hip_dl_threshold(const DlDesc* desc, int L, const uint32_t* counts, int64_t mc, int32_t* rows_out,
                               const int64_t* rows_off, int32_t* cnt_out, const int64_t* cnt_off, long long* fsz,
                               int32_t* scratch, int64_t scratch_cap, hipStream_t st) {
  DlLevels D;
  if (dl_levels(desc, L, &D, nullptr, -1)) return 1;
  DlOut O{};
  for (int l = 0; l < L; ++l) { O.rows_off[l] = rows_off[l]; O.cnt_off[l] = cnt_off[l]; }
  DlThrBlk B{};
  int64_t C = 0;
  for (int l = 0; l < L; ++l) {
    B.blk_base[l + 1] = B.blk_base[l] + (D.C[l] + kThB - 1) / kThB;
    C += D.C[l];
  }
  const int64_t nblk = B.blk_base[L];
  if (C <= 4 * kThB || scratch == nullptr || scratch_cap < nblk || nblk < 1) {
    hipLaunchKernelGGL(k_dl_threshold, dim3(1), dim3(1024), 0, st, D, O, counts, mc, rows_out, cnt_out, fsz);
  } else {
    hipLaunchKernelGGL(k_dlt_count, dim3((unsigned)nblk), dim3(256), 0, st, D, B, counts, mc, scratch);
    hipLaunchKernelGGL(k_dlt_scan, dim3(1), dim3(1024), 0, st, B, L, scratch, fsz);
    hipLaunchKernelGGL(k_dlt_emit, dim3((unsigned)nblk), dim3(256), 0, st, D, O, B, counts, mc, scratch, rows_out,
                       cnt_out);
  }
  FA_LAUNCH_RET();
}

FA_API int64_t fa_hip_dl_threshold_scratch(const DlDesc* desc, int L) {
  int64_t n = 0;
  for (int l = 0; l < L; ++l) n += (desc[l].C + kThB - 1) / kThB;
  return n;
}

FA_API int64_t fa_hip_dl_gpre_need(const DlDesc* desc, int L) {
  int64_t g = 0;
  for (int l = 0; l < L; ++l)
    if (desc[l].m > kDlInline) g += desc[l].n * desc[l].m;
  return g;
}
```

### csrc/host/fa_slab.h

```cpp
#pragma once
#include <math.h>
#include <stdint.h>

#include "fa_dl.h"

#if defined(__HIPCC__)
#define FA_SLAB_FN __host__ __device__ inline
#else
#define FA_SLAB_FN inline
#endif

namespace fa {

constexpr int kSlabBundleTarget = 8192;
constexpr int kSlabMinCap4 = 1024;
constexpr int kSlabMapMaxF1 = 8192;

FA_SLAB_FN int64_t slab_row_bytes(int sw) { return (int64_t)(sw + 2) * 8; }

FA_SLAB_FN int64_t slab_map_lds(int64_t F1) {
  return F1 <= kSlabMapMaxF1 ? ((F1 * 2 + 15) & ~(int64_t)15) : 0;
}

FA_SLAB_FN int slab_width(int64_t n_used, int64_t C, double lds, double accb, int64_t* cap) {
  const int order[4] = {16, 32, 8, 4};
  const int64_t want = C < kSlabBundleTarget ? C : kSlabBundleTarget;
  for (int q = 0; q < 4; ++q) {
    const int sw = order[q];
    const int64_t c = (int64_t)((lds - (double)(n_used * slab_row_bytes(sw))) / accb);
    if (c >= want || (sw == 4 && c >= kSlabMinCap4)) { *cap = c; return sw; }
  }
  *cap = 0;
  return 0;
}

FA_SLAB_FN int64_t slab_cap(int64_t n_used, int64_t C, double lds, double accb) {
  int64_t cap = 0;
  slab_width(n_used, C, lds, accb, &cap);
  return cap;
}

FA_SLAB_FN int64_t slab_total_limit(int64_t n_used, double lds, double accb) {
  int64_t lo = 0, hi = (int64_t)1 << 31;
  while (lo < hi) {
    const int64_t mid = (lo + hi + 1) / 2;
    if (mid <= slab_cap(n_used, mid, lds, accb)) lo = mid; else hi = mid - 1;
  }
  return lo;
}

constexpr int kSlabAcc8 = 8;
static_assert((kSlabAcc8 & (kSlabCls | kSlabDense | kSlabAcc16)) == 0, "a mode bit of its own");

FA_SLAB_FN int slab_acc_bytes(double accb, bool weighted) {
  return weighted ? 4 : accb == 1.0 ? 1 : accb == 2.0 ? 2 : 4;
}
FA_SLAB_FN int slab_acc_mode(double accb, bool weighted) {
  const int b = slab_acc_bytes(accb, weighted);
  return b == 1 ? kSlabAcc8 : b == 2 ? kSlabAcc16 : 0;
}
FA_SLAB_FN int slab_mode_acc_bytes(int cls, bool weighted) {
  return weighted ? 4 : (cls & kSlabAcc8) ? 1 : (cls & kSlabAcc16) ? 2 : 4;
}
FA_SLAB_FN int64_t slab_acc_count(int64_t C, int acc_bytes) {
  return acc_bytes == 1 ? (C + 3) / 4 : acc_bytes == 2 ? (C + 1) / 2 : C;
}

FA_SLAB_FN bool slab_acc_upgrade(int64_t n_used, int64_t C, double lds, double accb_try, int* sw, int64_t* cap,
                                 double* accb) {
  if (*sw == 16 || accb_try >= *accb) return false;
  int64_t c = 0;
  if (slab_width(n_used, C, lds, accb_try, &c) != 16 || C > c) return false;
  *sw = 16;
  *cap = c;
  *accb = accb_try;
  return true;
}

FA_SLAB_FN int64_t slab_acc_words(int64_t n_acc) { return (n_acc + 3) & ~(int64_t)3; }

FA_SLAB_FN int64_t slab_kernel_lds(int64_t n_used, int sw, int64_t n_acc_words, int64_t map_bytes) {
  return n_used * slab_row_bytes(sw) + n_acc_words * 4 + map_bytes;
}

FA_SLAB_FN int64_t slab_workgroups(int64_t nslabs, int64_t budget, int64_t kernel_lds) {
  int64_t per_cu = budget / (kernel_lds > 1 ? kernel_lds : 1);
  per_cu = per_cu < 1 ? 1 : per_cu > 2 ? 2 : per_cu;
  const int64_t n = nslabs < 256 * per_cu ? nslabs : 256 * per_cu;
  return n > 1 ? n : 1;
}


inline double binom_tail(int64_t L, double p, int k) {
  if (L < k) return 0.0;
  if (p <= 0.0) return k <= 0 ? 1.0 : 0.0;
  if (p >= 1.0) return 1.0;
  double pmf = pow(1.0 - p, (double)L), below = 0.0;
  const double r = p / (1.0 - p);
  for (int i = 0; i < k; ++i) {
    below += pmf;
    pmf *= (double)(L - i) / (double)(i + 1) * r;
  }
  const double t = 1.0 - below;
  return t < 0.0 ? 0.0 : t > 1.0 ? 1.0 : t;
}

inline void trim_estimate(const int64_t* len_hist, int64_t n_bins, double p, int k, double* rows, double* nnz) {
  double est_rows = 0.0, est_nnz = 0.0;
  for (int64_t L = 0; L < n_bins; ++L) {
    const double h = (double)len_hist[L];
    if (h == 0.0) continue;
    est_rows += h * binom_tail(L, p, k);
    est_nnz += h * (double)L * p;
  }
  *rows = est_rows;
  *nnz = est_nnz;
}

}
```

### csrc/host/plan.cpp

```cpp
#include <algorithm>
#include <cstring>
#include <vector>

#include "fa_common.h"
#include "fa_limits.h"
#include "fa_slab.h"

using namespace fa;

FA_API int fa_slab_width(int64_t n_used, int64_t C, double lds, double accb, int64_t* cap) {
  return slab_width(n_used, C, lds, accb, cap);
}
FA_API int64_t fa_slab_total_limit(int64_t n_used, double lds, double accb) {
  return slab_total_limit(n_used, lds, accb);
}
FA_API int64_t fa_slab_map_lds(int64_t F1) { return slab_map_lds(F1); }
FA_API int64_t fa_slab_workgroups(int64_t nslabs, int64_t n_used, int sw, int64_t n_acc, int round_acc,
                                  int64_t map_bytes, int64_t budget) {
  return slab_workgroups(nslabs, budget,
                         slab_kernel_lds(n_used, sw, round_acc ? slab_acc_words(n_acc) : n_acc, map_bytes));
}
FA_API int fa_slab_acc_mode(double accb, int weighted, int64_t C, int64_t* n_acc) {
  if (n_acc) *n_acc = slab_acc_count(C, slab_acc_bytes(accb, weighted != 0));
  return slab_acc_mode(accb, weighted != 0);
}
FA_API int fa_slab_acc_upgrade(int64_t n_used, int64_t C, double lds, double accb_try, int* sw, int64_t* cap,
                               double* accb) {
  return slab_acc_upgrade(n_used, C, lds, accb_try, sw, cap, accb) ? 1 : 0;
}
FA_API void fa_trim_estimate(const int64_t* len_hist, int64_t n_bins, double p, int k, double* rows, double* nnz) {
  trim_estimate(len_hist, n_bins, p, k, rows, nnz);
}


struct SlabPiece { int64_t g, lo, hi; };
constexpr int kClsMaxRun = 8;
constexpr double kClsMinGain = 0.8;
constexpr uint8_t kRecKeepQ = 1, kRecKeepP = 2;

static int64_t slot_cost(const std::vector<SlabPiece>& pcs, const std::vector<int64_t>& slots,
                         const std::vector<uint8_t>& flags, int m) {
  int64_t wc[kSlabThreads / 64] = {0};
  const int64_t n = (int64_t)slots.size();
  for (int64_t w0 = 0; w0 < n; w0 += 64) {
    bool q = false, p = false, any = false;
    int64_t e = 0;
    for (int64_t s = w0; s < std::min(n, w0 + 64); ++s) {
      if (slots[s] < 0) continue;
      any = true;
      q = q || !(flags[s] & kRecKeepQ);
      p = p || !(flags[s] & kRecKeepP);
      e = std::max(e, pcs[slots[s]].hi - pcs[slots[s]].lo);
    }
    if (any) wc[(w0 % kSlabThreads) / 64] += (q ? m - 1 : 0) + (p ? 1 : 0) + e + 1;
  }
  return *std::max_element(wc, wc + kSlabThreads / 64);
}

static void cls_layout(const std::vector<SlabPiece>& pcs, int64_t i, int64_t j, const int32_t* Pf,
                       const int64_t* poff, int m, std::vector<int64_t>& slots, std::vector<uint8_t>& flags) {
  struct Run { int64_t k0; int s; };
  std::vector<Run> runs;
  for (int64_t k = i; k < j; ++k) {
    bool same = k > i && runs.back().s < kClsMaxRun;
    if (same && pcs[k].g != pcs[k - 1].g) {
      const int32_t* a = Pf + poff[pcs[k - 1].g];
      const int32_t* b = Pf + poff[pcs[k].g];
      same = std::equal(a, a + m - 1, b);
    }
    if (same) runs.back().s += 1;
    else runs.push_back({k, 1});
  }
  std::stable_sort(runs.begin(), runs.end(), [&](const Run& x, const Run& y) { return x.s > y.s; });
  constexpr int NWv = kSlabThreads / 64;
  struct Row { int64_t r0, r1, cost; };
  std::vector<Row> rows;
  for (int64_t r = 0; r < (int64_t)runs.size();) {
    int64_t r1 = r + 1;
    while (r1 < (int64_t)runs.size() && r1 - r < 64 && runs[r1].s == runs[r].s) ++r1;
    int64_t c = 0;
    for (int e = 0; e < runs[r].s; ++e) {
      int64_t mx = 0;
      bool newp = e == 0;
      for (int64_t x = r; x < r1; ++x) {
        const int64_t k = runs[x].k0 + e;
        mx = std::max(mx, pcs[k].hi - pcs[k].lo);
        newp = newp || pcs[k].g != pcs[k - 1].g;
      }
      c += (e == 0 ? m - 1 : 0) + (newp ? 1 : 0) + mx + 1;
    }
    rows.push_back({r, r1, c});
    r = r1;
  }
  std::stable_sort(rows.begin(), rows.end(), [](const Row& x, const Row& y) { return x.cost > y.cost; });
  std::vector<std::vector<std::pair<int64_t, int64_t>>> rows_of(NWv);
  int64_t load[NWv] = {0}, wcost[NWv] = {0};
  for (const Row& rw : rows) {
    const int w = (int)(std::min_element(wcost, wcost + NWv) - wcost);
    rows_of[w].push_back({rw.r0, rw.r1});
    load[w] += runs[rw.r0].s;
    wcost[w] += rw.cost;
  }
  const int64_t T = *std::max_element(load, load + NWv);
// ... 185 lines not shown
```

### fastapriori_amd/models/apriori.py

```python
from __future__ import annotations

import gc
import math
import os
import time
from dataclasses import dataclass

import numpy as np
import torch

from .. import ops
from ..ops.host import apriori_gen
from ..parallel.comm import Comm
from ..tuning import TUNING
from ..utils.jvm import item_tiebreak_key, min_count
from ..utils.metrics import Logger, Timer, roctx_range
from .data import MiningResult, TransactionShard

HORIZONTAL_PAIRS_PER_S = 2.0e11
GRAM_WORDPAIRS_PER_S = 1.7e13
F1_SKETCH_MIN_VOCAB = 1 << 20
F1_HIST_READBACK = 1 << 16
_TRIU_CACHE: dict = {}
_POW10 = 10 ** np.arange(1, 11, dtype=np.int64)
# ... 196 lines not shown
                self._level_recs.append((rec, f"level{k}"))
                self._ckpt_level(result, kk)
            self.stats["host_levels"] = self.stats.get("host_levels", 0) + len(bundle)
            k += len(bundle)
        while len(levels) > 1 and len(levels[-1]) == 0:
            levels.pop(); counts.pop()
        return self._finish(result, t_start)

    @staticmethod
    def _entered(levels: list, kk: int) -> bool:
        return 2 <= kk - 1 <= len(levels) and len(levels[kk - 2]) >= kk

    def _log_level(self, levels: list, kk: int, groups, n_freq: int, ms: float, cand_line: bool = True) -> None:
        if self._log_stop or not self._entered(levels, kk):
            self._log_stop = True
            return
        if cand_line and self.log.enabled:
            self.log.line(f"{kk} candidate items {groups() if callable(groups) else int(groups)}")
        self.log.line(f"{kk} freq items {n_freq}")
        self.log.line(f"Use Time {kk} items {int(ms)}")
        self._logged_upto = kk

    def _log_tail(self, levels: list) -> None:
        if self.cfg.max_level or self._log_stop:
            return
        kk = self._logged_upto + 1
        while self._entered(levels, kk):
            n = len(levels[kk - 1]) if kk - 1 < len(levels) else 0
            self._log_level(levels, kk, lambda kk=kk: int(apriori_gen(levels[kk - 2])[0].size), n, 0.0)
            kk += 1

    def _log_level2(self, n2: int) -> None:
        F1 = self._F1
        self.log.line(f"2 freq items {n2}")
        self.log.line(f"Use Time 2 items {int(self._level2_ms)}")
        self._logged_upto = max(self._logged_upto, 2)
        self._level_recs.append((dict(phase="level", k=2, candidates=F1 * (F1 - 1) // 2, frequent=n2,
                                      ms=self._level2_ms, strategy=self.stats.get("pair_strategy"),
                                      bytes_reduced=self._level2_bytes,
                                      hbm_bytes_est=self.stats.get("pair_hbm_bytes_est", 0)),
                                 "pairs"))

    def _device_levels_planned(self, resume) -> bool:
        return (TUNING.device_levels and self._dev.type == "cuda"
                and 2 <= self._F1 <= ops.primitives.dl().kAgMaxF1
                and self.cfg.level_kernel in ("auto", "slab") and self.stats["n_lines"] < (1 << 31)
                and (self.cfg.max_level == 0 or self.cfg.max_level >= 3))

    def _device_levels_ok(self, resume, levels: list) -> bool:
        if not self._device_levels_planned(resume):
            return False
        return self._f2_dev is not None or (resume is not None and len(levels) >= 2 and levels[-1] is not None)

    def _ckpt_level(self, result: MiningResult, k: int) -> None:
        if self.ckpt is not None and not self._ckpt_deferred:
            self.ckpt.save_level(result, k)
            self._ckpt_saved = max(self._ckpt_saved, k)

    def _ckpt_upto(self, result: MiningResult, K: int, background: bool) -> None:
        if self.ckpt is not None and K > self._ckpt_saved:
            self.ckpt.save_levels(result, range(self._ckpt_saved + 1, K + 1), background=background)
            self._ckpt_saved = K

    def _mine_device(self, db, levels: list, counts: list, mc: int, result: MiningResult):
        self._piece_part(True)
        try:
            return self._mine_device_loop(db, levels, counts, mc, result)
        finally:
            self._piece_part(False)

    def _mine_device_loop(self, db, levels: list, counts: list, mc: int, result: MiningResult):
        Pm = ops.primitives
        K = Pm.dl()
        S = Pm.device_level_state(self._dev)
        F1 = self._F1
        lds = Pm.dl_lds_budget(F1)
        unit = db["wword"] is None
        self._dl_mp_accb = 2.0 if TUNING.dl_acc16 and unit else 4.0
        acc8 = int(TUNING.dl_acc8_bundles) if unit else 0
        if int(self._count_view(db)["ncols"]) < TUNING.dl_acc8_min_rows:
            acc8 = 0
        accb = self._dl_accb = 1.0 if acc8 == 1 else 2.0 if TUNING.dl_acc16_bundles and unit else 4.0
        self._dl_cnt_accb = 1.0 if acc8 == 2 else accb
        c_bound = int(lds // accb)
        st = torch.cuda.current_stream(self._dev).cuda_stream
        f2 = self._f2_dev
        m0, k = 2, 3
        if f2 is None:
            last = np.ascontiguousarray(levels[-1], dtype=np.int32)
            m0, k = last.shape[1], last.shape[1] + 1
            f2 = self._resume_rows = torch.from_numpy(last.reshape(-1, m0)).to(self._dev)
        if self._f2_n_dev is not None:
            P0, n_src, n_const, n_bound = f2.data_ptr(), self._f2_n_dev.data_ptr(), 0, self._f2_bound
        else:
            P0, n_src, n_const, n_bound = f2.data_ptr(), None, int(f2.shape[0]), int(f2.shape[0])
        if self.ckpt is not None and self._ckpt_deferred:
            self._result_items(result)
            n_host = next((i for i, lv in enumerate(levels) if lv is None), len(levels))
            self._ckpt_upto(result, n_host, background=True)
        pend = []
        tm = self._timer
        nxt = None
        self._dl_stg = dict(n=0, rows=[], cnt=[], f2=None, ev=None, stream=getattr(self, "_dl_stage_stream", None))
        while True:
            if self.cfg.max_level and k > self.cfg.max_level:
                break
            if m0 > K.kDlMaxM:
                nxt = k
                break
            t0 = time.perf_counter()
            b0 = self._bytes_moved()
            with roctx_range(f"dlevel{k}"), tm.phase(f"level{k}"):
                max_lv = min(K.kDlMaxM - m0 + 1, K.kDlMaxLevels)
                if self.cfg.max_level:
                    max_lv = min(max_lv, self.cfg.max_level - k + 1)
                if not TUNING.bundle_levels or k - 1 > TUNING.bundle_max_prefix:
                    max_lv = 1
                post = TUNING.dl_post and max_lv > 1
                S.rows_hint = int(self._count_view(db)["ncols"])
                if post:
                    self._dl_post_setup(S, db, k, F1, c_bound, n_bound, lds)
                if pend:
                    self._dl_stage(S, pend)
                with roctx_range("gen"):
                    c = Pm.dl_bundle_gen(S, P0, n_src, n_const, n_bound, m0, F1, c_bound, lds, TUNING.bundle_growth,
                                         max_lv, st, post=post, accb=accb)
                if c[K.kDlOverBound]:
                    raise RuntimeError(f"device bundle at level {k}: |F_{k - 1}| exceeds its bound {n_bound}")
                if c[K.kDlEnd]:
                    break
                multi = None
                if c[K.kDlMulti]:
                    multi = self._dl_multipass(S, db, k, F1, c, P0, n_src, n_const, n_bound, m0, lds, st)
                    if multi is None:
                        nxt = k
                        break
                    c = multi[0]
                L, n_used = int(c[K.kDlLevels]), int(c[K.kDlNUsed])
                Cs = S.desc["C"][:L].copy()
                C = int(Cs.sum())
                done = int(S.post.done) if post else 0
                sw = int(S.post.sw) if done else 0
                acc_bytes = int(S.post.accb) if done else int(accb)
                if multi is not None:
                    cnt = multi[1]
                    sw = int(Pm.LAST_LEVEL_PLAN.get("sw", 0))
                    acc_bytes = int(self._dl_mp_accb)
                elif done == 2:
                    cnt = S.post_bufs["out"][:C]
                else:
                    nwd = (F1 + 63) // 64
                    bits = np.unpackbits(c[K.kDlBits:K.kDlBits + nwd].view(np.uint8), bitorder="little")[:F1]
                    used = np.flatnonzero(bits)
                    if done == 1:
                        plan = Pm.dl_plan_from_post(S, n_used)
                    else:
                        with roctx_range("plan"):
                            plan = Pm.dl_plan(S, L, F1, n_used, C, lds, self._dev, accb, self._dl_cnt_accb)
                    with tm.phase(f"trim{k}"), roctx_range("trim"):
                        self._trim(db, used, k, C, decided=bool(done == 1 and S.post.trim))
                    with tm.phase("count"), roctx_range("count"):
                        v = self._count_view(db)
                        cnt = Pm.dl_count(S, plan, v["roff"], v["ranks"], v["src"], v["ncols"], F1, v["wword"])
                    sw, acc_bytes = int(plan["sw"]), int(plan.get("accb", 4.0))
                nz = torch.count_nonzero(cnt) if self.cand_par else None
                with tm.phase("count"), roctx_range("count"):
                    self.comm.all_reduce_(cnt)
                    rows_a, cnt_a, ro, co = Pm.dl_threshold(S, L, cnt, mc, k)
            hbm_rows = (db["ranks"].numel() * db["ranks"].element_size()
                        + db["roff"].numel() * db["roff"].element_size())
            pend.append(dict(k=k, L=L, m0=m0, C=Cs, rows=rows_a, cnt=cnt_a, ro=ro, co=co, hbm_rows=int(hbm_rows),
                             n_par=S.desc["n"][:L].copy(), sw=sw, acc_bytes=acc_bytes, used=n_used,
                             T=int(db["roff"].numel() - 1),
                             ms=(time.perf_counter() - t0) * 1e3, bytes=self._bytes_moved() - b0,
                             G=c[K.kDlGl:K.kDlGl + L].copy(), nz=nz))
            P0 = rows_a.data_ptr() + 4 * int(ro[L - 1])
            n_src, n_const, n_bound = S.fsz.data_ptr() + 8 * (k + L - 1), 0, int(Cs[-1])
            m0 += L
            k += L
            if int(Cs[-1]) < k or (multi is None and int(c[K.kDlEmpty])):
                break
        self._dl_flush(S, pend, levels, counts, result)
        if self.cand_par and pend:
            self.stats["cand_counted"] = int(sum(int(p["nz"]) for p in pend if p["nz"] is not None))
            self.stats["cand_total"] = int(sum(int(p["C"].sum()) for p in pend))
        self.stats["device_bundles"] = len(pend)
        self.stats["device_bundle_shapes"] = [(int(p["k"]), int(p["L"]), int(p["C"].sum()), int(p["used"]),
                                               int(p["sw"]), int(p["acc_bytes"])) for p in pend]
        self.stats["device_levels"] = int(sum(p["L"] for p in pend))
        return nxt

    def _dl_multipass(self, S, db, k: int, F1: int, c, P0, n_src, n_const: int, n_bound: int, m0: int, lds: int,
                      st):
        Pm = ops.primitives
        K = Pm.dl()
        if not TUNING.dl_multi or self.cfg.max_level and k > self.cfg.max_level:
            return None
        C0 = int(c[K.kDlCl])
        if int(c[K.kDlLevels]) == 0:
            c = Pm.dl_bundle_gen(S, P0, n_src, n_const, n_bound, m0, F1, C0, lds, TUNING.bundle_growth, 1, st,
                                 accb=self._dl_accb)
            if c[K.kDlOverBound] or c[K.kDlEnd] or int(c[K.kDlLevels]) != 1 or int(c[K.kDlCl]) != C0:
                raise RuntimeError(f"device level {k}: regeneration of {C0} candidates disagrees ({c[:8]})")
        nwd = (F1 + 63) // 64
        bits = np.unpackbits(c[K.kDlBits:K.kDlBits + nwd].view(np.uint8), bitorder="little")[:F1]
        used = np.flatnonzero(bits)
        n_used = int(used.size)
        wide = Pm.slab_width(n_used, C0, lds, self._dl_mp_accb)[0] == 0
        with self._timer.phase(f"trim{k}"), roctx_range("trim"):
            self._trim(db, used, k, C0)
        v = self._count_view(db)
        if wide:
            with self._timer.phase("count"), roctx_range("count_bitmap"):
                cnt = self._dl_bitmap_count(S, v, used)
            self.stats["device_bitmap_levels"] = self.stats.get("device_bitmap_levels", 0) + 1
            return c, cnt
        with self._timer.phase("count"), roctx_range("count_multi"):
            bm, bmap = self._bitmaps(v, used, blocked=True)
            used_t = torch.from_numpy(used.astype(np.int64)).to(self._dev)
            bm_rows = (bmap[used_t] if bmap is not None else used_t).to(torch.int32).contiguous()
            wr = None
            if (self.cfg.trim and TUNING.window_trim and v["wword"] is None and v["src"] is None
                    and v["T"] >= self.cfg.trim_min_rows
                    and v.get("T0", v["T"]) >= TUNING.window_trim_min_rows):
                wr = lambda used_w, nc: self._window_rows(v, used_w, k, bm, bmap, nc)
            cnt = Pm.dl_count_multipass(S, F1, n_used, C0, lds, v["roff"], v["ranks"], v["src"], v["ncols"],
                                        v["wword"], bm, bm_rows,
                                        self.stats["min_count"] / max(1, self.stats["n_lines"]), self._dev,
                                        bmap=bmap, window_rows=wr)
            plan = Pm.LAST_LEVEL_PLAN
            if plan.get("windows_trimmed"):
                self.stats["window_trims"] = self.stats.get("window_trims", 0) + int(plan["windows_trimmed"])
        if cnt is None:
            return None
        self.stats["device_multipass"] = self.stats.get("device_multipass", 0) + 1
        return c, cnt

    def _window_rows(self, db, used_w: np.ndarray, k: int, bm, bmap, n_cand: int):
        if bm is None or used_w.size > ops.primitives.limits().kWinMaxItems:
            return None
        keep = min(TUNING.window_trim_rows_frac,
                   1.0 - TUNING.window_trim_cost * used_w.size / max(1, n_cand * (k + 1)))
        est = self._trim_estimate(db, used_w, k)
        wlog = self.stats.setdefault("window_log", [])
        rec = dict(k=k, items=int(used_w.size), cand=int(n_cand), keep=round(keep, 3),
                   est=None if est is None else round(est / max(1, db["T"]), 3))
        wlog.append(rec)
        if keep <= 0 or est is None or est >= TUNING.window_trim_est_frac * db["T"]:
            return None
        dev = db["ranks"].device
        used_t = torch.from_numpy(used_w.astype(np.int64)).to(dev)
        rows_w = (bmap[used_t] if bmap is not None else used_t).to(torch.int32).contiguous()
        with roctx_range("window_rows"):
            got = ops.primitives.window_bitmap(bm, rows_w, (int(db["ncols"]) + 63) // 64, k,
                                               max_keep=int(keep * db["T"]))
        rec["kept"] = None if got is None else round(got[0] / max(1, db["T"]), 3)
        return got

    @staticmethod
    def _trim_estimate(db, used: np.ndarray, k: int, with_nnz: bool = False):
        hist = db.get("len_hist")
        if hist is None:
            return None
        c1, alive = db["c1"], db["alive"]
        denom = float(c1[alive].sum())
        if denom <= 0:
            return None
        p = min(float(c1[used].sum()) / denom, 1.0)
        rows, nnz = ops.primitives.trim_estimate(hist, p, k)
        return (rows, nnz) if with_nnz else rows

    def _dl_bitmap_count(self, S, db, used: np.ndarray) -> torch.Tensor:
        Pm = ops.primitives
        d0 = S.desc[0]
        m, C = int(d0["m"]), int(d0["C"])
        off = int(d0["rows"]) - S.ws.data_ptr()
        if off < 0 or off % 4 or off + 4 * C * (m + 1) > S.ws.numel():
            raise RuntimeError("device bundle: candidate rows outside the generator workspace")
        rows = S.ws[off:off + 4 * C * (m + 1)].view(torch.int32).view(C, m + 1)
        pre, ext = rows[:, :m], rows[:, m]
        starts = torch.zeros(1, dtype=torch.int64, device=self._dev)
        if C > 1:
            starts = torch.cat([starts, torch.nonzero((pre[1:] != pre[:-1]).any(1)).flatten() + 1])
        gs = starts.cpu().numpy()
        ext_off = np.append(gs, C).astype(np.int64)
        bm, bmap = self._bitmaps(db, used)
        prefix = pre[starts].to(torch.int64)
        ext64 = ext.to(torch.int64)
        if bmap is not None:
            prefix, ext64 = bmap[prefix], bmap[ext64]
        if self.cand_par:
            r, nr = self.comm.rank, self.comm.world_size
            g0, g1 = (int(np.searchsorted(ext_off, C * q // nr, side="left")) for q in (r, r + 1))
            g1 = gs.size if r == nr - 1 else g1
            e0, e1 = int(ext_off[g0]), int(ext_off[g1])
            cnt = torch.zeros(C, dtype=torch.int32, device=self._dev)
            if g1 > g0:
                part = ops.count_candidates(bm, db["W"], prefix[g0:g1].to(torch.int32).contiguous(),
                                            ext_off[g0:g1 + 1] - e0, ext64[e0:e1].to(torch.int32).contiguous(),
                                            db["wword"])
                cnt[e0:e1] = part.to(torch.int32)
            return cnt
        cnt = ops.count_candidates(bm, db["W"], prefix.to(torch.int32).contiguous(), ext_off,
                                   ext64.to(torch.int32).contiguous(), db["wword"])
        Pm.LAST_LEVEL_PLAN.clear()
        Pm.LAST_LEVEL_PLAN.update(kernel="bitmap_dev", rows=int(db["roff"].numel() - 1), used=int(used.size), C=C, m=m)
        return cnt.to(torch.int32)

    def _count_view(self, db) -> dict:
        return db

    def _piece_part(self, on: bool) -> None:
        r, n = (self.comm.rank, self.comm.world_size) if (on and self.cand_par) else (0, 1)
        ops.primitives.set_piece_part(r, n)

    def _dl_post_setup(self, S, db, k: int, F1: int, c_bound: int, n_bound: int, lds: int) -> None:
        Pm = ops.primitives
        m0 = k - 1
        K = Pm.dl()
        gpre_n = n_bound * m0 if m0 > K.kDlInline else (c_bound * (m0 + 4) if m0 + K.kDlMaxLevels > K.kDlInline else 0)
        b = S.post_buffers(F1, c_bound, n_bound + c_bound, min(gpre_n, 1 << 24))
        P = S.post
        P.item_map, P.rec, P.part, P.out = (b["item_map"].data_ptr(), b["rec"].data_ptr(), b["part"].data_ptr(),
                                            b["out"].data_ptr())
        P.rec_cap, P.part_cap, P.out_cap = b["c_cap"], b["part"].numel(), b["c_cap"]
        P.gpre, P.gpre_cap = b["gpre"].data_ptr(), b["gpre"].numel()
        v = self._count_view(db)
        P.roff, P.ranks = v["roff"].data_ptr(), v["ranks"].data_ptr()
        P.src = v["src"].data_ptr() if v["src"] is not None else None
        P.wword = v["wword"].data_ptr() if v["wword"] is not None else None
        P.ncols, P.lds_kernel, P.lds_budget = int(v["ncols"]), float(TUNING.slab_lds_bytes), float(lds)
        P.accb = self._dl_cnt_accb
        c1 = np.ascontiguousarray(db["c1"], dtype=np.int64)
        alive = np.ascontiguousarray(db["alive"], dtype=np.uint8)
        hist, bins = db.get("len_hist"), ops.primitives.limits().kTrimHist
        hist = np.ascontiguousarray(hist, dtype=np.int64) if hist is not None and hist.size == bins else None
        S.post_keep = (c1, alive, hist)
        P.c1, P.alive = c1.ctypes.data, alive.ctypes.data
        P.len_hist = hist.ctypes.data if hist is not None else None
        P.T, P.nnz = int(db["T"]), int(db["ranks"].numel())
        P.trim_min_rows, P.trim_ok, P.k = int(self.cfg.trim_min_rows), int(bool(self.cfg.trim) and db["T"] > 0), k
        P.trim_rows_frac, P.trim_nnz_frac = float(TUNING.trim_rows_frac), float(TUNING.trim_nnz_frac)

    def _dl_stage(self, S, pend: list) -> None:
        Pm = ops.primitives
        stg = self._dl_stg
        todo = []
        if self._f2_n_dev is not None and stg["f2"] is None:
            nb = self._f2_bound
            stg["f2"] = [None] * 3
            todo += [("f2", 0, self._f2_n_dev.view(torch.int32)), ("f2", 1, self._f2_dev[:nb].reshape(-1)),
                     ("f2", 2, self._f2_cnt_dev[:nb])]
        for i in range(stg["n"], len(pend)):
            todo += [("rows", i, pend[i]["rows"]), ("cnt", i, pend[i]["cnt"])]
            stg["rows"].append(None)
            stg["cnt"].append(None)
        first, stg["n"] = stg["n"], len(pend)
        if not todo:
            return
        dev = self._dev
        cs = stg.get("stream")
        if cs is None:
            cs = stg["stream"] = self._dl_stage_stream = torch.cuda.Stream(dev)
        cs.wait_stream(torch.cuda.current_stream(dev))
        ckpt = self.ckpt is not None and self._ckpt_deferred
        with torch.cuda.stream(cs):
            for kind, i, t in todo:
                h = Pm.pinned_stage(f"dl_{kind}{i}").get(4 * t.numel()).view(torch.int32)
                h.copy_(t, non_blocking=True)
                stg[kind][i] = h
            if ckpt:
                fsz_h = Pm.pinned_stage(f"dl_fsz{len(pend)}").get(8 * S.fsz.numel()).view(torch.int64)
                fsz_h.copy_(S.fsz, non_blocking=True)
            ev = torch.cuda.Event()
            ev.record(cs)
        stg["ev"] = ev
        if ckpt:
            self._ckpt_staged(pend, first, todo[0][0] == "f2", fsz_h, ev)

    def _dl_decode_f2(self, n2_h, rows_h, cnt_h):
        n2 = int(n2_h.numpy()[:2].view(np.int64)[0])
        return rows_h.numpy()[:2 * n2].reshape(n2, 2), cnt_h.numpy()[:n2]

    @staticmethod
    def _dl_decode(p: dict, rows_h: np.ndarray, cnt_h: np.ndarray, fsz: np.ndarray) -> list:
        out = []
        for l in range(p["L"]):
            kk, w = p["k"] + l, p["m0"] + l + 1
            F = int(fsz[kk])
            a, b = int(p["ro"][l]), int(p["co"][l])
            out.append((kk, rows_h[a:a + F * w].reshape(F, w), cnt_h[b:b + F]))
        return out

    def _ckpt_staged(self, pend: list, first: int, with_f2: bool, fsz_h, ev) -> None:
        ck, result, stg = self.ckpt, self._result, self._dl_stg
        ks = ([2] if with_f2 else []) + [p["k"] + l for p in pend[first:] for l in range(p["L"])]
        if not ks:
            return
        fault = ck.fault_level(self.comm.rank)
        upto = fault if fault in ks else ks[-1]
        f2 = stg["f2"] if with_f2 else None
        bufs = [(p, stg["rows"][i], stg["cnt"][i]) for i, p in enumerate(pend[first:], first)]

        def work():
            ev.synchronize()
            fsz = fsz_h.numpy()
            lv = []
            if f2 is not None:
                lv.append((2,) + self._dl_decode_f2(*f2))
            for p, rh, ch in bufs:
                lv += self._dl_decode(p, rh.numpy(), ch.numpy(), fsz)
            for k, rows, cnt in lv:
                if k <= upto:
                    ck._write_level(result, k, meta=False, rows=np.ascontiguousarray(rows, np.int32),
                                    counts=cnt.astype(np.int64))
            ck._write_meta(result, upto)

        if ck.rank == 0:
            ck.submit(work)
        self._ckpt_saved = max(self._ckpt_saved, upto)
        if fault in ks:
            ck.wait()
            from ..utils.checkpoint import InjectedFault
            raise InjectedFault(17)

    def _dl_flush(self, S, pend: list, levels: list, counts: list, result: MiningResult) -> None:
        f2 = self._f2_n_dev is not None
        if not pend and not f2:
            return
        self._dl_stage(S, pend)
        stg = self._dl_stg
        fsz = S.fsz.cpu().numpy()
        stg["ev"].synchronize()
        if f2:
            r2, c2 = self._dl_decode_f2(*stg["f2"])
            levels[1] = r2.copy()
            counts[1] = c2.astype(np.int64)
            self._log_level2(len(c2))
            self._f2_n_dev = None
        if not pend:
            return
        for i, p in enumerate(pend):
            for l, (kk, rows, cnt) in enumerate(self._dl_decode(p, stg["rows"][i].numpy(), stg["cnt"][i].numpy(),
                                                                fsz)):
                F = len(cnt)
                levels.append(rows.copy())
                counts.append(cnt.astype(np.int64))
                share = float(p["C"][l]) / max(float(p["C"].sum()), 1.0)
                groups = (lambda kk=kk: int(apriori_gen(levels[kk - 2])[0].size)) if kk > p["k"] else int(p["G"][l])
                self._log_level(levels, kk, groups, F, p["ms"] * share)
                m = p["m0"] + l
                hbm = int(share * p["hbm_rows"] + 4 * int(p["n_par"][l]) * m
                          + 4 * int(p["C"][l]) * (m + 1) + 3 * 4 * int(p["C"][l]))
                self._level_recs.append((dict(phase="level", k=kk, candidates=int(p["C"][l]), frequent=F,
                                              ms=p["ms"] * share, groups=int(p["G"][l]), bundled_with=p["k"],
                                              bytes_reduced=int(p["bytes"] * share), kernel="slab_rec_dev",
                                              hbm_bytes_est=hbm, slab_words=p["sw"], acc_bytes=p["acc_bytes"],
                                              used_items=p["used"],
                                              rows=p["T"], _share=share),
                                         f"level{p['k']}"))

    def _run_deferred(self) -> None:
        for d in self._deferred:
            d.result()
        self._deferred = []

    @staticmethod
    def _result_items(result: MiningResult, wait: bool = True) -> None:
        if wait and not isinstance(result.items, list):
            result.items = result.items.result()

    def _bytes_moved(self) -> int:
        b = self.comm.bytes_reduced
        if getattr(self, "dcomm", self.comm) is not self.comm:
            b += self.dcomm.bytes_reduced
        return b

    @staticmethod
    def _level_hbm_bytes(db, plan: dict) -> int:
        if not plan:
            return 0
        passes = int(plan.get("passes", 1) or 1)
        rows = int(db["ranks"].numel()) * 4 + int(db["roff"].numel()) * 8
        return passes * rows

    def _emit_level_metrics(self) -> None:
        tm = getattr(self, "_timer", None)
        gpu = tm.finish() if (tm is not None and tm.events) else {}
        if tm is not None and tm.events:
            self.stats["gpu_phase_ms"] = {k: round(v, 3) for k, v in gpu.items()}
        for rec, span in getattr(self, "_level_recs", []):
            share = rec.pop("_share", 1.0)
            if span is not None and span in gpu:
                rec["gpu_ms"] = round(gpu[span] * share, 3)
            self.log.metric(**rec)
        self._level_recs = []
        if self.cfg.trace and tm is not None:
            self.stats["trace"] = tm.trace(pid=self.comm.rank)

    def _finish(self, result: MiningResult, t_start: float) -> MiningResult:
        self._result_items(result)
        if getattr(self, "_ckpt_deferred", False):
            self._ckpt_upto(result, len(result.levels), background=True)
        db = getattr(self, "_db_local", None)
        if db is not None:
            sizes = getattr(self, "_layout_sizes", None)
            if sizes is None:
                g = self.dcomm.all_gather_ints([db["T0"], db["ncols0"]])
                sizes = int(g[:, 0].sum()), int(g[:, 1].sum())
            self.stats.update(T=sizes[0], distinct=sizes[1])
            self._db_local = None
        if len(result.levels) >= 2:
            self._log_tail(result.levels)
        total_k2 = sum(len(c) for c in result.counts[1:])
        self.log.line(f"Total freq items sets {total_k2}")
        self.stats["mine_ms"] = (time.perf_counter() - t_start) * 1e3
        self.stats["n_itemsets"] = result.n_itemsets
        self.stats["bytes_reduced"] = self.comm.bytes_reduced
        if ops.primitives.FALLBACKS:
            self.stats["fallbacks"] = list(ops.primitives.FALLBACKS)
            for f in ops.primitives.FALLBACKS:
                self.log.metric(phase="fallback", what=f)
        self._emit_level_metrics()
        if getattr(self, "_timer", None) is not None and self._timer.sync:
            self.stats["phase_ms"] = {k: round(v, 3) for k, v in self._timer.t.items()}
        return result

    def _check_resume(self, resume: MiningResult, fresh: MiningResult) -> None:
        if resume.items != fresh.items or not np.array_equal(resume.counts[0], fresh.counts[0]):
            raise ValueError("checkpoint does not match the input data (different F1)")

    def _frequent_items(self, shard: TransactionShard, mc: int):
        comm, vocab, dev = self.dcomm, shard.vocab, shard.items.device
        thr = max(mc, 1)
        if vocab.numeric:
            V = self._V_max
            got = None
            if self.cfg.f1 == "sketch" or (self.cfg.f1 == "auto" and dev.type == "cuda"
                                              and V >= F1_SKETCH_MIN_VOCAB):
                got = self._f1_heavy_hitters(shard, V, thr)
# ... 579 lines not shown
```

### fastapriori_amd/ops/_native.py

```python
from __future__ import annotations

import ctypes as C
import os
import threading

from . import build as _build

_lock = threading.Lock()
_host = None
_hip = None

i32, i64, u64, dbl = C.c_int32, C.c_int64, C.c_uint64, C.c_double
vp, cp = C.c_void_p, C.c_char_p
I64P = C.POINTER(C.c_int64)
IP = C.POINTER(C.c_int)

_HOST_SIGS = {
    "fa_parse_file": (vp, [cp, i64, i64, C.c_int, C.c_int, IP]),
    "fa_parse_buffer": (vp, [cp, i64, C.c_int, C.c_int]),
    "fa_file_size": (i64, [cp]),
    "fa_next_line_start": (i64, [cp, i64, i64]),
    "fa_chunk_scan": (None, [vp, i64, vp]),
    "fa_txndb_info": (None, [vp, vp]),
    "fa_txndb_export": (None, [vp, vp, vp, vp, C.c_int]),
    "fa_txndb_export_dict": (None, [vp, vp, vp, vp, C.c_int]),
    "fa_hash_tokens": (None, [vp, vp, i64, vp, C.c_int]),
    "fa_txndb_free": (None, [vp]),
    "fa_hash_bytes": (u64, [cp, i64]),
    "fa_quest_generate": (vp, [i64, i64, dbl, dbl, i64, i64, u64, C.c_int, C.c_int]),
    "fa_zipf_generate": (vp, [i64, i64, dbl, dbl, i64, dbl, dbl, i64, u64, C.c_int]),
    "fa_zipf_write": (C.c_int, [cp, i64, dbl, dbl, i64, dbl, dbl, i64, u64, C.c_int, C.c_int]),
    "fa_quest_write": (C.c_int, [cp, i64, dbl, dbl, i64, i64, u64, C.c_int, C.c_int]),
    "fa_apriori_gen": (vp, [vp, i64, C.c_int, C.c_int, vp]),
    "fa_cands_export": (None, [vp, vp, vp, vp]),
    "fa_cands_free": (None, [vp]),
    "fa_level_plan": (C.c_int, [vp, vp, i64, vp, vp, i32, vp, vp, i64, vp, i64, vp]),
    "fa_slab_width": (C.c_int, [i64, i64, dbl, dbl, I64P]),
    "fa_slab_total_limit": (i64, [i64, dbl, dbl]),
    "fa_slab_map_lds": (i64, [i64]),
    "fa_slab_workgroups": (i64, [i64, i64, C.c_int, i64, C.c_int, i64, i64]),
    "fa_slab_acc_mode": (C.c_int, [dbl, C.c_int, i64, I64P]),
    "fa_slab_acc_upgrade": (C.c_int, [i64, i64, dbl, dbl, C.POINTER(C.c_int), I64P, C.POINTER(dbl)]),
    "fa_trim_estimate": (None, [vp, i64, dbl, C.c_int, C.POINTER(dbl), C.POINTER(dbl)]),
    "fa_dl_layout": (cp, [C.c_int, I64P]),
    "fa_limits": (cp, [C.c_int, I64P]),
    "fa_f1_rank_numeric": (i64, [vp, i64, i64, vp, vp, vp]),
    "fa_rules_build": (vp, [vp, vp, vp, C.c_int, vp, C.c_int, vp]),
    "fa_rules_nante": (i64, [vp]),
    "fa_rules_nstats": (i64, [vp]),
    "fa_rules_export": (None, [vp, vp, vp, vp, vp, vp]),
    "fa_rules_free": (None, [vp]),
    "fa_recommend_cpu": (None, [vp, vp, vp, i64, i32, vp, vp, i64, vp, C.c_int]),
    "fa_recommend_topn_cpu": (None, [vp, vp, vp, i64, i32, vp, vp, i64, i32, vp, C.c_int]),
    "fa_condense_cpu": (C.c_int, [vp, vp, vp, vp, C.c_int, vp, vp, C.c_int]),
    "fa_write_freq_itemsets": (C.c_int, [cp, vp, vp, i32, vp, vp, vp, C.c_int, C.c_int, C.c_int]),
    "fa_cpu_histogram": (None, [vp, i64, i64, vp, C.c_int]),
    "fa_build_probe_table": (None, [vp, i64, C.c_int, C.c_uint32, vp, vp]),
    "fa_cpu_txn_freq_count": (None, [vp, vp, i64, vp, vp, C.c_int]),
    "fa_cpu_compress": (None, [vp, vp, vp, vp, i64, vp, vp, C.c_int]),
    "fa_cpu_build_bitmaps": (None, [vp, vp, vp, i64, i64, vp, C.c_int]),
    "fa_cpu_row_hash": (None, [vp, vp, i64, vp, vp, C.c_int]),
    "fa_cpu_pair_gram": (None, [vp, i32, i64, i64, vp, vp, C.c_int]),
    "fa_cpu_pair_horizontal": (None, [vp, vp, i64, vp, i32, vp, C.c_int]),
    "fa_cpu_count_candidates": (None, [vp, i64, i64, vp, i32, vp, vp, i64, vp, vp, C.c_int]),
}

_HIP_SIGS = {
    "fa_hip_histogram": (C.c_int, [vp, i64, i32, vp, vp]),
    "fa_hip_f1_rank": (C.c_int, [vp, i32, i64, C.c_int, vp, vp, vp]),
    "fa_hip_debug_la_qsum": (C.c_int, [vp, vp]),
    "fa_hip_win_alive": (C.c_int, [vp, i64, vp, C.c_int, i64, C.c_int, vp, vp, vp]),
    "fa_hip_win_compact": (C.c_int, [vp, i64, vp, C.c_int, i64, vp, vp, vp, i64, vp]),
    "fa_hip_debug_slab_max_wg": (None, [C.c_int]),
    "fa_hip_pairs_compact": (C.c_int, [vp, i64, i32, i64, vp, vp, vp, vp, vp, vp]),
    "fa_hip_f1_sketch": (C.c_int, [vp, i64, vp, vp, vp]),
    "fa_hip_f1_exact": (C.c_int, [vp, i64, vp, C.c_int, vp, vp]),
    "fa_hip_txn_freq_count": (C.c_int, [vp, vp, i64, i64, vp, vp, vp]),
    "fa_hip_compress_regs": (C.c_int, [C.c_int, vp, vp, vp, vp, i64, vp, vp, vp, vp, vp]),
    "fa_hip_ag_gen": (C.c_int, [vp, i64, C.c_int, C.c_int, vp, i64, vp, i64, vp, vp]),
    "fa_hip_ag_chain": (C.c_int, [vp, i64, C.c_int, C.c_int, vp, i64, vp, i64, C.c_int, dbl, i64, i64, vp, vp,
                                  C.c_int, dbl]),
    "fa_hip_ag_build": (C.c_int, [vp, i64, C.c_int, vp, C.c_uint32, C.c_int, vp, vp]),
    "fa_hip_ag_rows": (C.c_int, [vp, i64, C.c_int, vp, C.c_uint32, C.c_int, vp, vp, vp, vp, C.c_int, vp]),
    "fa_hip_cmp_agg": (C.c_int, [vp, vp, vp, i64, vp, vp, vp, C.c_int, vp]),
    "fa_hip_cmp_scan": (C.c_int, [vp, vp, i64, C.c_int, vp, vp, vp, vp, vp]),
    "fa_hip_cmp_emit": (C.c_int, [vp, vp, vp, i64, vp, vp, vp, vp, vp, vp, vp, vp, C.c_int, vp, vp, i64, vp, vp,
                                  vp]),
    "fa_hip_lr_rows": (C.c_int, [vp, vp, vp, i64, vp, C.c_int, vp, i64, vp]),
    "fa_hip_compress_regs_bc": (C.c_int, [vp, vp, vp, vp, i64, vp, vp, vp, vp, vp, i64, C.c_int, vp]),
    "fa_hip_block_counts_rows": (C.c_int, [vp, vp, vp, i64, vp, i64, C.c_int, vp, vp]),
    "fa_hip_block_bsum": (C.c_int, [vp, i64, i64, C.c_int, vp, vp]),
    "fa_hip_compress_staged": (C.c_int, [vp, vp, vp, i64, vp, vp, vp, vp, vp]),
    "fa_hip_compress_staged64": (C.c_int, [vp, vp, vp, i64, vp, vp, vp, vp, C.c_int, vp]),
    "fa_hip_count_slab_rec_cls": (C.c_int, [vp, vp, vp, i64, vp, C.c_int, C.c_int, vp, vp, C.c_int, C.c_int, vp,
                                            vp, C.c_int, C.c_int, vp, i64, vp, vp, vp, C.c_int]),
    "fa_hip_dl_level0": (C.c_int, [vp, vp, i64, i64, C.c_int, C.c_int, vp, i64, vp, vp, i64, dbl, dbl, vp, C.c_int,
                                   vp]),
    "fa_hip_dl_more": (C.c_int, [C.c_int, vp, i64, i64, vp, vp, dbl, C.c_int, dbl, dbl, i64, vp, vp, vp, vp]),
    "fa_hip_dl_plan": (C.c_int, [vp, C.c_int, vp, C.c_int, vp, vp, i64, vp, i64, vp, i64, C.c_int, vp]),
    "fa_hip_set_lane_deal": (None, [C.c_int]),
    "fa_hip_set_piece_part": (C.c_int, [C.c_int, C.c_int]),
    "fa_hip_dl_gpre_need": (i64, [vp, C.c_int]),
    "fa_hip_dl_plan_window": (C.c_int, [vp, C.c_int, vp, C.c_int, vp, vp, i64, vp, i64, vp, i64, i64, i64, C.c_int,
                                        vp]),
    "fa_hip_dl_plan_window_bits": (C.c_int, [vp, C.c_int, vp, C.c_int, vp, vp, vp, i64, vp, i64, vp, i64, i64, i64,
                                             C.c_int, vp]),
    "fa_hip_dl_chunk_bits": (C.c_int, [vp, C.c_int, C.c_int, vp, vp]),
    "fa_hip_dl_threshold": (C.c_int, [vp, C.c_int, vp, i64, vp, vp, vp, vp, vp, vp, i64, vp]),
    "fa_hip_trim_scan_count": (C.c_int, [vp, vp, i64, vp, C.c_int, C.c_int, vp, vp, vp, vp, vp]),
    "fa_hip_trim_emit": (C.c_int, [vp, vp, vp, C.c_int, i64, vp, vp, vp, vp, vp, vp, vp, vp]),
    "fa_hip_compress_wave": (C.c_int, [vp, vp, vp, vp, i64, vp, vp, vp, C.c_int, vp, vp]),
    "fa_hip_compress_lds": (C.c_int, [vp, vp, vp, vp, i64, vp, vp, vp, vp, vp, vp]),
    "fa_hip_dedup_probe": (C.c_int, [vp, vp, vp, i64, vp, vp, vp]),
    "fa_hip_row_hash": (C.c_int, [vp, vp, i64, vp, vp, vp]),
    "fa_hip_build_bitmaps": (C.c_int, [vp, vp, vp, i64, i32, i64, C.c_int, C.c_int, vp, vp, vp, C.c_int, vp]),
    "fa_hip_block_counts": (C.c_int, [vp, vp, i64, i32, vp, vp, C.c_int, vp]),
    "fa_hip_block_scatter": (C.c_int, [vp, vp, i64, i32, vp, vp, vp, C.c_int, vp]),
    "fa_hip_pair_queue16": (C.c_int, [vp, vp, vp, i64, C.c_int, i64, vp, vp, C.c_int, vp]),
    "fa_hip_pair_blocked": (C.c_int, [vp, vp, vp, i64, vp, i32, vp, i64, vp]),
    "fa_hip_pair_gram_mfma": (C.c_int, [vp, i32, i64, i64, C.c_int, i64, vp, C.c_int, C.c_uint32, C.c_int, vp]),
    "fa_hip_pair_gram_popc": (C.c_int, [vp, i32, i64, i64, C.c_int, i64, vp, vp, C.c_int, vp]),
    "fa_hip_count_candidates": (C.c_int, [vp, i64, i64, vp, C.c_int, vp, vp, vp, C.c_int, vp, vp, vp]),
    "fa_hip_recommend": (C.c_int, [vp, vp, vp, i64, i32, vp, vp, i64, vp, vp]),
    "fa_hip_recommend_indexed": (C.c_int, [vp, vp, vp, vp, vp, i64, i32, vp, vp, i64, vp, vp]),
    "fa_hip_recommend_topn": (C.c_int, [vp, vp, vp, i64, i32, vp, vp, i64, i32, vp, vp]),
    "fa_hip_recommend_topn_indexed": (C.c_int, [vp, vp, vp, vp, vp, i64, i32, vp, vp, i64, i32, vp, vp]),
    "fa_hip_parse_tiles": (i64, [i64]),
    "fa_hip_tparse_tiles": (i64, [i64, i64]),
    "fa_hip_tline_count": (C.c_int, [vp, i64, i64, vp, vp]),
    "fa_hip_tparse": (C.c_int, [vp, i64, i64, i64, C.c_int, i64, vp, vp, vp, vp, vp, vp, vp, vp, vp]),
    "fa_hip_scan_small": (C.c_int, [C.c_int, vp, i64, vp, vp, vp]),
    "fa_hip_tcompact": (C.c_int, [vp, vp, i64, C.c_int, vp, vp, vp, vp, vp, vp, vp, i64, i64, vp, C.c_int, vp, vp, vp]),
    "fa_hip_hist_reduce": (C.c_int, [vp, C.c_int, vp, vp]),
    "fa_hip_line_count": (C.c_int, [vp, i64, vp, vp]),
    "fa_hip_line_ends": (C.c_int, [vp, i64, vp, vp, vp]),
    "fa_hip_parse_lines_dict": (C.c_int, [vp, vp, i64, vp, vp, vp, vp, vp, vp, vp, vp, vp, i64, vp]),
    "fa_hip_slot_remap": (C.c_int, [vp, i64, vp, vp]),
    "fa_hip_dict_verify": (C.c_int, [vp, vp, i64, vp, vp, vp, vp, i64, vp]),
    "fa_hip_compact_lines": (C.c_int, [vp, vp, vp, vp, vp, vp, vp, i64, vp, vp, vp]),
    "fa_hip_rule_gen": (C.c_int, [vp, i64, C.c_int, vp, i64, vp, vp, vp, vp, vp]),
    "fa_hip_rule_cut": (C.c_int, [vp, vp, i64, C.c_int, vp, vp, vp, vp]),
    "fa_hip_rule_emit": (C.c_int, [vp, vp, vp, vp, vp, i64, vp, vp]),
    "fa_hip_sup_mark": (C.c_int, [vp, vp, vp, vp, vp, vp, C.c_int, vp, vp, vp, vp]),
}


def _declare(lib, sigs):
    for name, (res, args) in sigs.items():
        fn = getattr(lib, name)
        fn.restype = res
        fn.argtypes = args
    return lib


BUILD_IDS: dict = {}


def _check_id(kind: str, lib, path: str) -> None:
    fn = lib.fa_build_id
    fn.restype, fn.argtypes = cp, []
    got = fn().decode("ascii", "replace")
    have_src = bool(_build.hip_sources() if kind == "hip" else _build.host_sources())
    want = _build.source_id(kind) if have_src else None
    BUILD_IDS[kind] = (got, want, path)
    override = kind == "hip" and bool(os.environ.get("FA_HIP_LIB"))
    if want is not None and got != want and not override:
        raise RuntimeError(f"{path} was built from other sources (build id {got}, these sources {want}): "
                           "rebuild with `python -m fastapriori_amd.ops.build`")


def host():
    global _host
    if _host is None:
        with _lock:
            if _host is None:
                path = _build.HOST_LIB
                if _build.embedded_id(path) != _build.source_id("host") and _build.host_sources():
                    _build.build_host()
                lib = C.CDLL(path)
                _check_id("host", lib, path)
                _host = _declare(lib, _HOST_SIGS)
    return _host

# ... 22 lines not shown
```

### fastapriori_amd/ops/primitives.py

```python
from __future__ import annotations

import ctypes as C
import ctypes
import functools
import os
import time
from dataclasses import dataclass

import numpy as np
import torch

from ..tuning import TUNING
from ..utils.env import num_threads
from . import _native

_I32, _I64 = torch.int32, torch.int64
PAIR_CHUNK_ROWS = 1 << 18


def _p(t: torch.Tensor | None) -> int | None:
    return None if t is None else t.data_ptr()


def _stream(t: torch.Tensor) -> int:
# ... 573 lines not shown
        nsc = max(1, (W + 2047) // 2048)
        per_block = int(np.clip(C * nsc // 4096, 16, limits().kMaxBlockExt))
        gidx, new_off, starts = _split_groups(ext_off, per_block, limits().kMaxBlockExt)
        pre = prefix[torch.from_numpy(gidx).to(dev)].contiguous() if gidx.size != prefix.shape[0] else prefix
        off_t = torch.from_numpy(new_off).to(dev)
        st_t = torch.from_numpy(starts).to(dev)
        out = torch.zeros(C, dtype=_I32, device=dev)
        _hip_call("fa_hip_count_candidates", _p(bm), bm.stride(0), W, _p(pre), m, _p(off_t), _p(ext),
                  _p(st_t), starts.size - 1, _p(wword), _p(out), _stream(bm))
        return out.to(_I64)
    out = torch.zeros(C, dtype=_I64)
    off_t = torch.from_numpy(np.ascontiguousarray(ext_off, dtype=np.int64))
    _native.host().fa_cpu_count_candidates(_p(bm), bm.stride(0), W, _p(prefix), m, _p(off_t), _p(ext),
                                           prefix.shape[0], _p(wword), _p(out), num_threads())
    return out


def trim_rows(roff, ranks, alive: torch.Tensor, min_len: int, wrow=None):
    T = roff.numel() - 1
    dev = ranks.device
    bins = limits().kTrimHist
    if T == 0:
        return (torch.zeros(0, dtype=_I32, device=dev), roff, ranks, wrow,
                torch.zeros(bins, dtype=_I64, device=dev))
    if ranks.is_cuda:
        st = _stream(ranks)
        nb = (T + 255) // 256
        cnt = torch.empty(T, dtype=_I32, device=dev)
        bk = torch.empty(2, nb, dtype=_I32, device=dev)
        F1 = alive.numel()
        _hip_call("fa_hip_trim_scan_count", _p(roff), _p(ranks), T, _p(alive), F1, int(min_len), _p(wrow), _p(cnt),
                  _p(bk[0]), _p(bk[1]), st)
        bases = torch.zeros(2, nb + 1, dtype=_I64, device=dev)
        torch.cumsum(bk[0], 0, dtype=_I64, out=bases[0, 1:])
        torch.cumsum(bk[1], 0, dtype=_I64, out=bases[1, 1:])
        K, nnz = (int(v) for v in bases[:, -1].tolist())
        nroff = torch.empty(K + 1, dtype=_I64, device=dev)
        nroff[K:] = nnz
        nranks = torch.empty(max(nnz, 1), dtype=_I32, device=dev)
        kept = torch.empty(max(K, 1), dtype=_I32, device=dev)
        hist = torch.zeros(limits().kTrimStripes, bins, dtype=_I64, device=dev)
        if K:
            _hip_call("fa_hip_trim_emit", _p(roff), _p(ranks), _p(alive), F1, T, _p(cnt), _p(bases[0]), _p(bases[1]),
                      _p(nroff), _p(nranks), _p(kept), _p(hist), st)
        kept = kept[:K]
        nw = wrow[kept.to(_I64)].contiguous() if wrow is not None else None
        return kept, nroff, nranks[:nnz], nw, hist.sum(0)
    a = alive[ranks.to(_I64)].to(_I64)
    cs = torch.zeros(ranks.numel() + 1, dtype=_I64)
    torch.cumsum(a, 0, out=cs[1:])
    cnt = (cs[roff[1:]] - cs[roff[:-1]]).to(_I32)
    keep = cnt >= min_len
    if wrow is not None:
        keep &= wrow > 0
    kept = torch.nonzero(keep).flatten().to(_I32)
    K = kept.numel()
    nroff = torch.zeros(K + 1, dtype=_I64, device=dev)
    if K:
        torch.cumsum(cnt[kept.to(_I64)].to(_I64), 0, out=nroff[1:])
    nnz = int(nroff[-1].item())
    nranks = torch.empty(max(nnz, 1), dtype=_I32, device=dev)
    if K:
        lens = roff[1:] - roff[:-1]
        rowmask = torch.zeros(T, dtype=torch.bool)
        rowmask[kept.to(_I64)] = True
        em = torch.repeat_interleave(rowmask, lens) & (alive[ranks.to(_I64)] > 0)
        nranks[:nnz] = ranks[em]
    nw = wrow[kept.to(_I64)].contiguous() if wrow is not None else None
    hist = torch.bincount(cnt[kept.to(_I64)].to(_I64).clamp_(max=bins - 1),
                          minlength=bins) if K else torch.zeros(bins, dtype=_I64)
    return kept, nroff, nranks[:nnz], nw, hist


def slab_width(n_used: int, C: int, lds: int, accb: int = 4) -> tuple[int, int]:
    cap = ctypes.c_int64(0)
    sw = _native.host().fa_slab_width(int(n_used), int(C), float(lds), float(accb), ctypes.byref(cap))
    return int(sw), int(cap.value)


def slab_total_limit(n_used: int, lds: int, accb: int = 4) -> int:
    return int(_native.host().fa_slab_total_limit(int(n_used), float(lds), float(accb)))


def slab_map_lds(F1: int) -> int:
    return int(_native.host().fa_slab_map_lds(int(F1)))


def trim_estimate(len_hist: np.ndarray, p: float, k: int) -> tuple[float, float]:
    hist = np.ascontiguousarray(len_hist, dtype=np.int64)
    rows, nnz = ctypes.c_double(0.0), ctypes.c_double(0.0)
    _native.host().fa_trim_estimate(hist.ctypes.data, hist.size, float(p), int(k), ctypes.byref(rows),
                                    ctypes.byref(nnz))
    return rows.value, nnz.value


def _slab_workgroups(nslabs: int, n_used: int, sw: int, n_acc: int, round_acc: bool, map_bytes: int) -> int:
    return int(_native.host().fa_slab_workgroups(int(nslabs), int(n_used), int(sw), int(n_acc), int(round_acc),
                                                 int(map_bytes), int(TUNING.slab_lds_bytes)))


def _slab_acc_mode(accb: float, weighted: bool, C: int) -> tuple[int, int]:
    n = ctypes.c_int64(0)
    mode = _native.host().fa_slab_acc_mode(float(accb), int(bool(weighted)), int(C), ctypes.byref(n))
    return int(mode), int(n.value)


def _slab_dense(wword, sw: int, sup_frac: float) -> bool:
    return wword is None and TUNING.dense_min_rows > 0 and sup_frac * sw * 64 >= TUNING.dense_min_rows


def _slab_count(*, roff, ranks, src, ncols: int, item_map, F1: int, n_used: int, gpre, rec, C: int, wword, out,
                sw: int, st: int, round_acc: bool, map_bytes: int, G: int = 0, g_dev=None, bm=None, bm_ld: int = 0,
                bm_rows=None, cls: int = 0, accb: float = 4.0, sup_frac: float = 0.0) -> None:
    K = dl()
    nslabs = ((ncols + 63) // 64 + sw - 1) // sw
    acc_mode, nacc = _slab_acc_mode(accb, wword is not None, C)
    n_wg = _slab_workgroups(nslabs, n_used, sw, nacc, round_acc, map_bytes)
    mode = cls | (K.kSlabDense if _slab_dense(wword, sw, sup_frac) else 0) | acc_mode
    _hip_call("fa_hip_count_slab_rec_cls", roff, ranks, src, ncols, item_map, F1, n_used, gpre, rec, G, C, wword,
              out, sw, n_wg, bm, bm_ld, st, bm_rows, g_dev, mode)




def _level_plan_bound(F1: int, C: int, G: int, m: int) -> int:
    return 2 * F1 + C + G * m + 14 * (G + C // 2 + 2) + (m + 16) * (G + C // 8 + 1) + 24


def level_plan_host(prefix: np.ndarray, ext_off: np.ndarray, ext: np.ndarray, F1: int, W: int,
                    lds_bytes: int | None = None, poff: np.ndarray | None = None, cls: int | None = None,
                    accb: int = 4):
    P, po, G, m = _flat_prefix(prefix, poff)
    C = int(ext.size)
    eo = np.ascontiguousarray(ext_off, dtype=np.int64)
    ex = np.ascontiguousarray(ext, dtype=np.int32)
    params = _plan_params(lds_bytes or TUNING.slab_lds_bytes, W, TUNING.slab_cls if cls is None else cls, accb)
    bound = _level_plan_bound(F1, C, G, m)
    passes = np.zeros((G + C + 2, 3), np.int64)
    info = np.zeros(24, np.int64)
    while True:
        buf = np.zeros(bound, np.int32)
        rc = _native.host().fa_level_plan(P.ctypes.data, po.ctypes.data, G, eo.ctypes.data, ex.ctypes.data, F1,
                                          params.ctypes.data, buf.ctypes.data, bound, passes.ctypes.data,
                                          passes.shape[0], info.ctypes.data)
        if rc != 3:
            break
        bound *= 2
    return rc, info, passes[:int(info[6])], buf[:int(info[18])]


def _plan_params(lds_bytes: int, W: int, cls: int, accb: int = 4) -> np.ndarray:
    return np.array([lds_bytes, W, float(accb), cls], dtype=np.float64)


def emulate_level_plan(bits_by_rank: np.ndarray, info, passes, buf, m: int, C: int) -> np.ndarray:
    n_used = int(info[3])
    used = buf[info[13]:info[13] + n_used]
    bits = bits_by_rank[used]
    gext = buf[info[14]:info[14] + C]
    out = np.zeros(C, np.int64)
    npc = int(info[4])
    gpre = buf[info[15]:info[16]]
    loc = buf[info[16]:info[16] + 2 * npc].reshape(-1, 2)
    gpm = buf[info[19]:info[19] + 2 * npc].reshape(-1, 2)
    for a, b, e0 in passes.tolist():
        for pi in range(a, b):
            p = np.logical_and.reduce(bits[gpre[gpm[pi, 0]:gpm[pi, 0] + gpm[pi, 1]]])
            for e in range(loc[pi, 0], loc[pi, 1]):
                out[e0 + e] += int((p & bits[gext[e0 + e]]).sum())
    return out


def emulate_slab_records(bits_by_rank: np.ndarray, info, passes, buf, C: int) -> np.ndarray:
    used = buf[info[13]:info[13] + int(info[3])]
    bits = bits_by_rank[used]
    gpre = buf[info[15]:info[16]]
    rec = buf[info[20]:info[20] + 12 * int(info[4])].view(np.uint32).reshape(-1, 12)
    u16 = np.stack([rec & 0xFFFF, rec >> 16], axis=-1).reshape(-1, 24)
    out = np.zeros(C, np.int64)
    for a, b, e0 in passes.tolist():
        for t in range(min(1024, b - a)):
            q = p = None
            for pi in range(a + t, b, 1024):
                r = rec[pi]
                n_ext, m, long_pre = int(r[1] & 0xFF), int((r[1] >> 8) & 0xFF), bool((r[1] >> 16) & 1)
                fl = int((r[1] >> 17) & 3)
                if long_pre:
                    ids = gpre[int(r[8]):int(r[8]) + m]
                else:
                    ids = np.concatenate([u16[pi, 4:8], u16[pi, 16:24]])[:m]
                if not fl & 1:
                    q = np.logical_and.reduce(bits[ids[:m - 1]])
                if not fl & 2:
                    p = q & bits[ids[m - 1]]
                for k in range(n_ext):
                    out[e0 + int(r[0]) + k] += int((p & bits[u16[pi, 8 + k]]).sum())
    return out


LAST_LEVEL_PLAN: dict = {}
CLS_LEVELS = [0]
# ... 581 lines not shown
        desc = sorted((off, n[7:]) for n, off in self.table.items() if n.startswith("DlDesc."))
        self.desc_dtype = np.dtype(dict(names=[n for _, n in desc], formats=[np.int64] * len(desc),
                                        offsets=[off for off, _ in desc], itemsize=self.table["sizeof(DlDesc)"]))
        self.post_size = self.table["sizeof(DlPost)"]
        self.post_offsets = {n[7:]: off for n, off in self.table.items() if n.startswith("DlPost.")}


class _DescTable(np.ndarray):
    def __setitem__(self, key, value):
        super().__setitem__(key, tuple(value) if isinstance(value, list) else value)


@functools.lru_cache(maxsize=None)
def dl() -> _DlLayout:
    return _DlLayout()


class DlPostC(ctypes.Structure):
    _fields_ = [(n, ctypes.c_void_p) for n in ("item_map", "rec", "part", "out")] + \
               [(n, ctypes.c_int64) for n in ("rec_cap", "part_cap", "out_cap")] + \
               [(n, ctypes.c_void_p) for n in ("roff", "ranks", "src", "wword")] + \
               [("ncols", ctypes.c_int64), ("lds_kernel", ctypes.c_double), ("lds_budget", ctypes.c_double)] + \
               [(n, ctypes.c_void_p) for n in ("c1", "alive", "len_hist")] + \
               [(n, ctypes.c_int64) for n in ("T", "nnz", "trim_min_rows", "trim_ok", "k",
                                               "done", "sw", "cap", "n_wg", "C", "trim")] + \
               [("gpre", ctypes.c_void_p), ("gpre_cap", ctypes.c_int64), ("accb", ctypes.c_double)] + \
               [("trim_rows_frac", ctypes.c_double), ("trim_nnz_frac", ctypes.c_double)]


class DeviceLevelState:

    def __init__(self, dev):
        self.dev = dev
        self.ws = torch.empty(64 << 20, dtype=torch.uint8, device=dev)
        K = dl()
        self.ctl = torch.zeros(K.kDlCtl, dtype=_I64, device=dev)
        self.ctl_h = torch.zeros(K.kDlCtl, dtype=_I64, pin_memory=True)
        self.fsz = torch.zeros(128, dtype=_I64, device=dev)
        self.desc = np.zeros(K.kDlMaxL, dtype=K.desc_dtype).view(_DescTable)
        self.info = np.zeros(4, dtype=np.int64)
        self.post = DlPostC()
        self.post_bufs = None
        self.post_keep = ()
        self.rows_hint = 0

    def grow(self, nbytes: int) -> None:
        self.ws = torch.empty(int(nbytes * 1.25) + (1 << 20), dtype=torch.uint8, device=self.dev)

    def post_buffers(self, F1: int, c_cap: int, rows_cap: int, gpre_n: int = 0):
        part_n = 8 * ((rows_cap + 255) // 256 + 2)
        b = self.post_bufs
        if (b is None or b["F1"] < F1 or b["c_cap"] < c_cap or b["part"].numel() < part_n
                or b["gpre"].numel() < gpre_n):
            F1, c_cap = max(F1, b["F1"] if b else 0), max(c_cap, b["c_cap"] if b else 0)
            part_n = max(part_n, b["part"].numel() if b else 0)
            gpre_n = max(gpre_n, b["gpre"].numel() if b else 1)
            b = self.post_bufs = dict(F1=F1, c_cap=c_cap,
                                      item_map=torch.empty(max(F1, 1), dtype=_I32, device=self.dev),
                                      rec=torch.empty(12 * c_cap + 12, dtype=_I32, device=self.dev),
                                      part=torch.empty(part_n, dtype=_I32, device=self.dev),
                                      out=torch.empty(c_cap, dtype=_I32, device=self.dev),
                                      gpre=torch.empty(max(gpre_n, 1), dtype=_I32, device=self.dev))
        return b


_DL_STATE: dict = {}


def device_level_state(dev) -> DeviceLevelState:
    st = _DL_STATE.get(dev)
    if st is None:
        st = _DL_STATE[dev] = DeviceLevelState(dev)
    return st


def dl_lds_budget(F1: int) -> int:
    return TUNING.slab_lds_bytes - slab_map_lds(F1)




def dl_bundle_gen(S: DeviceLevelState, P0: int, n_src: int | None, n_const: int, n_bound: int, m0: int, F1: int,
                  c_bound: int, lds: int, growth: float, max_levels: int, stream: int, post: bool = False,
                  accb: float = 4.0) -> np.ndarray:
    lib, K = _native.hip(), dl()
    info = np.zeros(2, dtype=np.int64)
    for _ in range(6):
        S.desc[:] = 0
        rc = lib.fa_hip_dl_level0(P0, n_src, n_const, n_bound, m0, F1, _p(S.ws), S.ws.numel(), _p(S.ctl),
                                  _p(S.ctl_h), c_bound, float(lds), float(accb), S.info.ctypes.data,
                                  int(max_levels <= 1), stream)
        if rc == 5:
            S.grow(int(S.info[0]))
            continue
        _native.check(rc, "fa_hip_dl_level0")
        d0 = S.desc[0]
        d0["P"], d0["cnt"], d0["off"], d0["rows"], d0["m"] = P0, S.info[1], S.info[2], S.info[3], m0
        if max_levels <= 1:
            c = S.ctl_h.numpy()
            d0["n"], d0["C"], d0["base"] = c[K.kDlNl], c[K.kDlCl], 0
            return c.copy()
        S.post.done = 0
        lane_deal(lib, S.rows_hint)
        rc = lib.fa_hip_dl_more(F1, _p(S.ws), S.ws.numel(), int(S.info[0]), _p(S.ctl), _p(S.ctl_h), float(growth),
                                int(max_levels), float(lds), float(accb), int(c_bound), S.desc.ctypes.data,
                                info.ctypes.data,
                                stream, ctypes.addressof(S.post) if post else None)
        if rc == 5:
            S.grow(int(info[0]))
            continue
        _native.check(rc, "fa_hip_dl_more")
        return S.ctl_h.numpy().copy()
    raise RuntimeError("device bundle generation: workspace sizing did not converge")


def set_piece_part(part: int, nparts: int) -> None:
    _native.check(_native.hip().fa_hip_set_piece_part(int(part), int(nparts)), "fa_hip_set_piece_part")


def lane_deal(lib, rows: int) -> None:
    lib.fa_hip_set_lane_deal(int(0 <= TUNING.lane_deal_min_rows <= rows))


def dl_plan(S: DeviceLevelState, L: int, F1: int, n_used: int, C: int, lds: int, dev, accb: float = 4.0,
            cnt_accb: float | None = None) -> dict:
    st = torch.cuda.current_stream(dev).cuda_stream
    sw, cap = slab_width(n_used, C, lds, accb)
    if sw == 0 or C > cap:
        raise RuntimeError(f"device bundle of {C} candidates over {n_used} items does not fit one pass")
    if cnt_accb is not None and cnt_accb < accb:
        sw_c, cap_c, accb_c = ctypes.c_int(sw), ctypes.c_int64(cap), ctypes.c_double(accb)
        _native.host().fa_slab_acc_upgrade(int(n_used), int(C), float(lds), float(cnt_accb), ctypes.byref(sw_c),
                                           ctypes.byref(cap_c), ctypes.byref(accb_c))
        sw, cap, accb = int(sw_c.value), int(cap_c.value), float(accb_c.value)
    item_map = torch.empty(max(F1, 1), dtype=_I32, device=dev)
    rec = torch.empty(12 * C + 12, dtype=_I32, device=dev)
    R = int(S.desc["n"][:L].sum())
    part = torch.empty(8 * max(1, (R + 255) // 256), dtype=_I32, device=dev)
    lib = _native.hip()
    gn = int(lib.fa_hip_dl_gpre_need(S.desc.ctypes.data, L))
    gpre = torch.empty(max(gn, 1), dtype=_I32, device=dev)
    lane_deal(lib, S.rows_hint)
    _native.check(lib.fa_hip_dl_plan(S.desc.ctypes.data, L, _p(S.ctl), F1, _p(item_map), _p(rec), C,
                                     _p(part), part.numel(), _p(gpre), gpre.numel(), sw, st), "fa_hip_dl_plan")
    out = torch.zeros(C, dtype=_I32, device=dev)
    return dict(sw=sw, cap=cap, item_map=item_map, rec=rec, out=out, n_used=n_used, C=C, gpre=gpre, accb=accb)


def dl_count_multipass(S: DeviceLevelState, F1: int, n_used: int, C: int, lds: int, roff, ranks, src, ncols: int,
                       wword, bm, bm_rows, sup_frac: float, dev, bmap=None, window_rows=None) -> torch.Tensor | None:
    acc16 = TUNING.dl_acc16 and wword is None
    accb = 2 if acc16 else 4
    sw, cap = slab_width(n_used, C, lds, accb)
    if sw == 0:
        return None
    st = _stream(ranks)
    lib = _native.hip()
    wins = None
    if TUNING.mp_window_items:
        wins = dl_window_plan(S, F1, C, lds, accb, st, dev)
    if not wins:
        cap = min(cap, C)
        cap = -(-C // -(-C // cap))
        wins = [(w0, min(C, w0 + cap), sw, None) for w0 in range(0, C, cap)]
    cap = max(w1 - w0 for w0, w1, _, _ in wins)
    item_map = torch.empty(max(F1, 1), dtype=_I32, device=dev)
    rec = torch.empty(12 * cap + 12, dtype=_I32, device=dev)
    R = int(S.desc[0]["n"])
    part = torch.empty(8 * max(1, (R + 255) // 256) + 16, dtype=_I32, device=dev)
    gn = int(lib.fa_hip_dl_gpre_need(S.desc.ctypes.data, 1))
    gpre = torch.empty(max(gn, 1), dtype=_I32, device=dev)
    out = torch.zeros(C, dtype=_I32, device=dev)
    npass, used_sum, rows_sum, trimmed = 0, 0, 0, 0
    lane_deal(lib, ncols)
    g_dev = _p(S.ctl) + 8 * dl().kDlPiecesI32
    for w0, w1, wsw, bits in wins:
        nu, rows_w, bits_p, bm_w, ncols_w = n_used, bm_rows, None, bm, ncols
        if bits is not None:
            used_w = np.flatnonzero(np.unpackbits(bits.view(np.uint8), bitorder="little")[:F1])
            nu = int(used_w.size)
            bits_t = torch.from_numpy(bits.view(np.int64).copy()).to(dev, non_blocking=False)
            bits_p = bits_t
            got = window_rows(used_w, w1 - w0) if window_rows is not None else None
            if got is not None:
                ncols_w, bm_w = got
                rows_w = None
                trimmed += 1
            else:
                used_t = torch.from_numpy(used_w.astype(np.int64)).to(dev)
                rows_w = (bmap[used_t] if bmap is not None else used_t).to(_I32).contiguous()
        if ncols_w == 0:
            continue
        _native.check(lib.fa_hip_dl_plan_window_bits(S.desc.ctypes.data, 1, _p(S.ctl), F1, _p(bits_p), _p(item_map),
                                                     _p(rec), cap, _p(part), part.numel(), _p(gpre), gpre.numel(),
                                                     w0, w1, wsw, st), "fa_hip_dl_plan_window_bits")
        _slab_count(roff=_p(roff), ranks=_p(ranks), src=_p(src), ncols=ncols_w, item_map=_p(item_map), F1=F1,
                    n_used=nu, gpre=_p(gpre), rec=_p(rec), g_dev=g_dev, C=w1 - w0, wword=_p(wword),
                    out=out.data_ptr() + 4 * w0, sw=wsw, st=st, round_acc=True, map_bytes=0, bm=_p(bm_w),
                    bm_ld=bitmap_ld(bm_w), bm_rows=_p(rows_w), accb=accb, sup_frac=sup_frac)
        npass += 1
        used_sum += nu
        rows_sum += ncols_w
    LAST_LEVEL_PLAN.clear()
    LAST_LEVEL_PLAN.update(kernel="slab_dev_multi", rows=int(roff.numel() - 1), used=n_used, sw=sw, cap=cap,
                           passes=npass, pieces=-1, slab_reads=0, m=int(S.desc[0]["m"]), C=C,
                           window_used_avg=round(used_sum / max(npass, 1), 1),
                           window_rows_avg=round(rows_sum / max(npass, 1)), windows_trimmed=trimmed)
    return out


WINDOW_SAMPLE = 16


def window_bitmap(bm: torch.Tensor, rows_w: torch.Tensor, W: int, k: int, max_keep: int | None = None,
                  blocked: bool = True):
    n = int(rows_w.numel())
    dev = bm.device
    st = _stream(bm)
    ld = bitmap_ld(bm)
    alive = torch.empty(max(W, 1), dtype=_I64, device=dev)
    cnt = torch.empty(max(W, 1), dtype=_I32, device=dev)
    if max_keep is not None and W >= 64 * WINDOW_SAMPLE:
        ws = W // WINDOW_SAMPLE
        _hip_call("fa_hip_win_alive", _p(bm), ld, _p(rows_w), n, ws, int(k), _p(alive), _p(cnt), st)
        if int(cnt[:ws].sum().item()) * (W / ws) > max_keep:
            return None
    _hip_call("fa_hip_win_alive", _p(bm), ld, _p(rows_w), n, W, int(k), _p(alive), _p(cnt), st)
    off = torch.zeros(W + 1, dtype=_I64, device=dev)
    torch.cumsum(cnt[:W], 0, out=off[1:])
    K = int(off[W].item())
    if max_keep is not None and K > max_keep:
        return None
    if K == 0:
        return 0, None
    wp = -(-((K + 63) // 64) // 64) * 64
    if blocked:
        out = torch.zeros((wp // 8, n, 8), dtype=_I64, device=dev)
        ldo = -out.stride(0)
    else:
        out = torch.zeros((n, wp), dtype=_I64, device=dev)
        ldo = out.stride(0)
    _hip_call("fa_hip_win_compact", _p(bm), ld, _p(rows_w), n, W, _p(alive), _p(off), _p(out), ldo, st)
    return K, out


def dl_window_plan(S: DeviceLevelState, F1: int, C: int, lds: int, accb: int, st: int, dev,
                   chunk: int = 1024) -> list | None:
    nwd = (F1 + 63) // 64
    if nwd > dl().kDlBitsW or C < 1:
        return None
    nch = -(-C // chunk)
    bits_d = torch.empty(nch * nwd, dtype=_I64, device=dev)
    _native.check(_native.hip().fa_hip_dl_chunk_bits(S.desc.ctypes.data, F1, chunk, _p(bits_d), st),
                  "fa_hip_dl_chunk_bits")
    bits = bits_d.cpu().numpy().view(np.uint64).reshape(nch, nwd)
    pop8 = np.array([bin(i).count("1") for i in range(256)], dtype=np.int64)
    wins = []
    j = 0
    while j < nch:
        acc = np.zeros(nwd, dtype=np.uint64)
        k, best = j, None
        while k < nch:
            a2 = acc | bits[k]
            n = int(pop8[a2.view(np.uint8)].sum())
            cand = min((k + 1) * chunk, C) - j * chunk
            sw, cap = slab_width(n, cand, lds, accb)
            if sw == 0 or cap < cand:
                break
            acc, best = a2, sw
            k += 1
        if best is None:
            return None
        wins.append((j * chunk, min(k * chunk, C), best, acc))
        j = k
    return wins


def dl_plan_from_post(S: DeviceLevelState, n_used: int) -> dict:
    P, b = S.post, S.post_bufs
    C = int(P.C)
    out = b["out"][:C]
    return dict(sw=int(P.sw), cap=int(P.cap), item_map=b["item_map"], rec=b["rec"], out=out, n_used=n_used, C=C,
                gpre=b["gpre"], accb=float(P.accb))


def dl_count(S: DeviceLevelState, plan: dict, roff, ranks, src, ncols: int, F1: int, wword) -> torch.Tensor:
    st = _stream(ranks)
    sw, cap, n_used, C = plan["sw"], plan["cap"], plan["n_used"], plan["C"]
    item_map, rec, out = plan["item_map"], plan["rec"], plan["out"]
    _slab_count(roff=_p(roff), ranks=_p(ranks), src=_p(src), ncols=ncols, item_map=_p(item_map), F1=F1,
                n_used=n_used, gpre=_p(plan.get("gpre")), rec=_p(rec), g_dev=_p(S.ctl) + 8 * dl().kDlPiecesI32, C=C,
                wword=_p(wword), out=_p(out), sw=sw, st=st, round_acc=True, map_bytes=slab_map_lds(F1),
                accb=plan.get("accb", 4.0))
    LAST_LEVEL_PLAN.clear()
    LAST_LEVEL_PLAN.update(kernel="slab_dev", rows=int(roff.numel() - 1), used=n_used, sw=sw, cap=cap, passes=1,
                           pieces=-1, slab_reads=0, m=-1, C=C)
    return out


def dl_threshold(S: DeviceLevelState, L: int, counts: torch.Tensor, mc: int, k0: int):
    dev = counts.device
    C = S.desc["C"][:L]
    w = S.desc["m"][:L] + 1
    rows_off = np.zeros(L, dtype=np.int64)
    cnt_off = np.zeros(L, dtype=np.int64)
    if L > 1:
        rows_off[1:] = np.cumsum(C * w)[:-1]
        cnt_off[1:] = np.cumsum(C)[:-1]
    rows = torch.empty(max(int((C * w).sum()), 1), dtype=_I32, device=dev)
    nblk = int(((C + 1023) // 1024).sum())
    cnt = torch.empty(max(int(C.sum()), 1) + nblk, dtype=_I32, device=dev)
    scratch = cnt[cnt.numel() - nblk:]
    _native.check(_native.hip().fa_hip_dl_threshold(S.desc.ctypes.data, L, _p(counts), int(mc), _p(rows),
                                                    rows_off.ctypes.data, _p(cnt), cnt_off.ctypes.data,
                                                    _p(S.fsz) + 8 * k0, _p(scratch), nblk, _stream(counts)),
                  "fa_hip_dl_threshold")
    cnt = cnt[:cnt.numel() - nblk]
    return rows, cnt, rows_off, cnt_off
```

### fastapriori_amd/tuning.py

```python
from __future__ import annotations

import os
from contextlib import contextmanager
from dataclasses import dataclass, fields


@dataclass
class Tuning:
    bundle_levels: bool = True
    bundle_growth: float = 1.5
    bundle_max_prefix: int = 9
    device_levels: bool = True
    dl_post: bool = True
    dl_multi: bool = True
    gen_device: bool = True
    gen_chain: bool = True
    gen_device_min_rows: int = 512
    pair_rs_min: int = 1 << 22
    fused_compress: bool = True
    early_compress: bool = True
    f1_rank_device: bool = True
    fused_compress_mean_len: float = 12.0
    fused_layout: bool = True
    compress_wave_mean_len: float = 48.0
    slab_lds_bytes: int = 160 * 1024 - 512
    slab_cls: int = 1
    dense_min_rows: float = 4.0
    dl_acc16: bool = True
    dl_acc16_bundles: bool = False
    dl_acc8_bundles: int = 2
    dl_acc8_min_rows: int = 1 << 20
    mp_window_items: bool = True
    window_trim: bool = True
    window_trim_est_frac: float = 0.95
    window_trim_rows_frac: float = 0.97
    window_trim_cost: float = 100.0
    window_trim_min_rows: int = 1 << 25
    lane_deal_min_rows: int = 1 << 25
    pair_wg: int = 0
    gram_mfma_min_class_words: int = 512
    bitmap_blocked: bool = True
    trim_rows_frac: float = 0.75
    trim_nnz_frac: float = 0.6
    gpu_parse: bool = True
    gpu_parse_dict: bool = True
    stream_parse: bool = True
    ring_slots: int = 16
    bucket_mb: float = 64.0

    @classmethod
    def from_env(cls, spec: str | None = None) -> "Tuning":
        t = cls()
        t.apply(os.environ.get("FA_TUNE", "") if spec is None else spec)
        return t

    def apply(self, spec: str) -> None:
        types = {f.name: f.type for f in fields(self)}
        for part in filter(None, (p.strip() for p in spec.split(","))):
            name, _, val = part.partition("=")
            name = name.strip()
            if name not in types:
                raise ValueError(f"FA_TUNE: unknown knob {name!r} (known: {', '.join(sorted(types))})")
            cur = getattr(self, name)
            if isinstance(cur, bool):
                v = val.strip().lower() in ("1", "true", "yes", "on")
            else:
                v = type(cur)(float(val) if isinstance(cur, int) else val)
            setattr(self, name, v)


TUNING = Tuning.from_env()


@contextmanager
def override(**kw):
    old = {k: getattr(TUNING, k) for k in kw}
    for k in kw:
        if not hasattr(TUNING, k):
            raise AttributeError(f"unknown tuning knob {k}")
    try:
        for k, v in kw.items():
            setattr(TUNING, k, v)
        yield TUNING
    finally:
        for k, v in old.items():
            setattr(TUNING, k, v)


__all__ = ["Tuning", "TUNING", "override"]
```

Before: 873,000 itemsets/s.

## Add packed padded slab row layout so tail levels fit one device bundle

Introduces a packed LDS slab row layout with configurable padding (SlabRows with pad shift) replacing the fixed SW+2 stride and swizzle, and instantiates padded kernel variants for widths 8 and 16. The device-level decision and post logic can now keep tail levels in the current bundle when they fit under the packed layout with smaller accumulators, instead of cutting the bundle and launching another pass. This aims to cut extra level passes and host round trips. The cost is more kernel instantiations, possible LDS bank conflicts from the changed row placement, and extra planning logic.

```diff
diff --git a/csrc/hip/count.hip b/csrc/hip/count.hip
--- a/csrc/hip/count.hip
+++ b/csrc/hip/count.hip
@@ -1065,23 +1065,33 @@
   return WordSpan{roff[min(col0 + lane, ncols)], roff[col0], roff[min(col0 + 64, ncols)]};
 }
 
-template <class Map>
-__device__ __forceinline__ void slab_build_word_span(uint64_t* __restrict__ slab, int swp, int q, const WordSpan& ws,
+template <int SW, int S>
+struct SlabRows {
+  __device__ __forceinline__ int operator()(int u) const { return (int)(slab_row_off(SW, S, u) >> 3); }
+  __device__ __forceinline__ int slot(int u) const { return (int)(slab_row_off(SW, S, u) >> 4); }
+};
+struct TileRows {
+  int stride;
+  __device__ __forceinline__ int operator()(int u) const { return u * stride; }
+};
+
+template <class Map, class Rows>
+__device__ __forceinline__ void slab_build_word_span(uint64_t* __restrict__ slab, Rows rows, int q, const WordSpan& ws,
                                                      const int32_t* __restrict__ ranks, Map item_map, int h,
-                                                     int nsub, unsigned long long* words, int swz);
-
-template <class Map = MapGlobal>
-__device__ __forceinline__ void slab_build_word_m(uint64_t* __restrict__ slab, int swp, int q, int64_t col0,
+                                                     int nsub, unsigned long long* words);
+
+template <class Map, class Rows>
+__device__ __forceinline__ void slab_build_word_m(uint64_t* __restrict__ slab, Rows rows, int q, int64_t col0,
                                                   int64_t ncols, const int64_t* __restrict__ roff,
                                                   const int32_t* __restrict__ ranks, Map item_map, int h,
-                                                  int nsub, unsigned long long* words, int swz = 0) {
-  slab_build_word_span(slab, swp, q, word_span(roff, col0, ncols), ranks, item_map, h, nsub, words, swz);
-}
-
-template <class Map>
-__device__ __forceinline__ void slab_build_word_span(uint64_t* __restrict__ slab, int swp, int q, const WordSpan& ws,
+                                                  int nsub, unsigned long long* words) {
+  slab_build_word_span(slab, rows, q, word_span(roff, col0, ncols), ranks, item_map, h, nsub, words);
+}
+
+template <class Map, class Rows>
+__device__ __forceinline__ void slab_build_word_span(uint64_t* __restrict__ slab, Rows rows, int q, const WordSpan& ws,
                                                      const int32_t* __restrict__ ranks, Map item_map, int h,
-                                                     int nsub, unsigned long long* words, int swz) {
+                                                     int nsub, unsigned long long* words) {
   const int lane = threadIdx.x & 63;
   const int64_t st = ws.st, base = ws.base, end = ws.end;
   const int srel = (int)(st - base);
@@ -1113,21 +1123,13 @@
     for (int u = 0; u < U; ++u) {
       const int l = cs + __popcll(S[u] & le) - 1;
       const int uu = r[u] >= 0 ? item_map(r[u]) : -1;
-      if (uu >= 0) atomicOr((unsigned long long*)(slab + (size_t)uu * swp + (q ^ ((uu << 2) & swz))), 1ull << l);
+      if (uu >= 0) atomicOr((unsigned long long*)(slab + rows(uu) + q), 1ull << l);
       cs += __popcll(S[u]);
     }
   }
 }
 
-__device__ __forceinline__ void slab_build_word(uint64_t* __restrict__ slab, int swp, int q, int64_t col0,
-                                                int64_t ncols, const int64_t* __restrict__ roff,
-                                                const int32_t* __restrict__ ranks,
-                                                const int32_t* __restrict__ item_map, int h, int nsub,
-                                                unsigned long long* words, int swz = 0) {
-  slab_build_word_m(slab, swp, q, col0, ncols, roff, ranks, MapGlobal{item_map}, h, nsub, words, swz);
-}
-
-template <int SW, int ROWW, bool kSwz>
+template <int SW, int S>
 __device__ __forceinline__ void slab_copy_bm(uint4* lds4, int n_used, const uint64_t* __restrict__ bm, int64_t Wp,
                                              const int32_t* __restrict__ bm_rows, int64_t w0, int64_t W) {
   constexpr int QW = SW / 2;
@@ -1154,8 +1156,7 @@
       const int i = base + (int)threadIdx.x + k * kSlabThreads;
       if (i < total) {
         const int u = i / QW, q = i % QW;
-        const int qq = kSwz ? (q ^ (((u << 2) & (SW - 4)) >> 1)) : q;
-        lds4[(size_t)u * (ROWW / 2) + qq] = v[k];
+        lds4[SlabRows<SW, S>{}.slot(u) + q] = v[k];
       }
     }
   }
@@ -1178,7 +1179,7 @@
   return (k & 1) ? (int)((uint32_t)w >> 16) : (w & 0xFFFF);
 }
 
-template <int SW, bool kWeighted, int kBuild, bool kCls = false, int kAccB = 4>
+template <int SW, bool kWeighted, int kBuild, bool kCls = false, int kAccB = 4, int kPad = 0>
 __global__ __launch_bounds__(kSlabThreads) void k_count_slab_rec(
     const int64_t* __restrict__ roff, const int32_t* __restrict__ ranks, const int32_t* __restrict__ src,
     int64_t ncols, const int32_t* __restrict__ item_map, int F1, int n_used, const int32_t* __restrict__ gpre,
@@ -1188,15 +1189,17 @@
   const int G = g_dev ? *g_dev : G_arg;
   extern __shared__ uint4 lds4[];
   __shared__ unsigned long long build_words[kSlabThreads / 64 * 2];
-  constexpr int SWP = SW + 2;
-  constexpr int RS = SWP / 2;
+  static_assert(kPad >= 0 && kPad <= kSlabPadMax, "pad shift");
+  constexpr SlabRows<SW, kPad> rows{};
+  auto row4 = [&](int u) { return lds4 + rows.slot(u); };
+  const int slab_slots = (int)(slab_rows_bytes(SW, kPad, n_used) >> 4);
   uint64_t* slab = reinterpret_cast<uint64_t*>(lds4);
   static_assert(kAccB == 4 || kAccB == 2 || kAccB == 1, "accumulator bytes");
   constexpr bool acc16 = !kWeighted && kAccB == 2;
   constexpr bool acc8 = !kWeighted && kAccB == 1;
   const int nacc = acc16 ? (C + 1) >> 1 : acc8 ? (C + 3) >> 2 : C;
   constexpr int kFlush16 = 65535 / (SW * 64);
-  uint32_t* acc = reinterpret_cast<uint32_t*>(slab + (size_t)n_used * SWP);
+  uint32_t* acc = reinterpret_cast<uint32_t*>(lds4 + slab_slots);
   uint8_t* acc8p = reinterpret_cast<uint8_t*>(acc);
   uint16_t* smap = reinterpret_cast<uint16_t*>(acc + ((nacc + 3) & ~3));
   const bool map_lds = kBuild == kBuildContig && F1 <= kMapLdsMax;
@@ -1218,7 +1221,7 @@
   if (g0 < G) { ra = rec[3 * g0]; rb = rec[3 * g0 + 1]; rc = rec[3 * g0 + 2]; }
 
   auto and_row = [&](uint4 (&p)[SW / 2], int u) {
-    const uint4* r = lds4 + (size_t)u * RS;
+    const uint4* r = row4(u);
 #pragma unroll
     for (int q = 0; q < SW / 2; ++q) {
       const uint4 v = r[q];
@@ -1226,8 +1229,8 @@
     }
   };
   auto and_row2 = [&](uint4 (&p)[SW / 2], int u, int w) {
-    const uint4* r = lds4 + (size_t)u * RS;
-    const uint4* t = lds4 + (size_t)w * RS;
+    const uint4* r = row4(u);
+    const uint4* t = row4(w);
 #pragma unroll
     for (int q = 0; q < SW / 2; ++q) {
       const uint4 v = r[q], x = t[q];
@@ -1295,11 +1298,11 @@
       nsl = 1;
     }
     if (kBuild == kBuildBM) {
-      slab_copy_bm<SW, SWP, false>(lds4, n_used, bm, Wp, bm_rows, w0, W);
+      slab_copy_bm<SW, kPad>(lds4, n_used, bm, Wp, bm_rows, w0, W);
     } else {
       {
         const uint4 z = make_uint4(0, 0, 0, 0);
-        for (int i = threadIdx.x; i < n_used * RS; i += blockDim.x) lds4[i] = z;
+        for (int i = threadIdx.x; i < slab_slots; i += blockDim.x) lds4[i] = z;
       }
       __syncthreads();
       if (kBuild == kBuildContig) {
@@ -1310,19 +1313,19 @@
           const int q = wv / NSUB;
           if ((w0 + q) * 64 < ncols) {
             if (map_lds)
-              slab_build_word_span(slab, SWP, q, span, ranks, MapLds{smap}, wv % NSUB, NSUB, build_words + wv * 2, 0);
+              slab_build_word_span(slab, rows, q, span, ranks, MapLds{smap}, wv % NSUB, NSUB, build_words + wv * 2);
             else
-              slab_build_word_span(slab, SWP, q, span, ranks, MapGlobal{item_map}, wv % NSUB, NSUB,
-                                   build_words + wv * 2, 0);
+              slab_build_word_span(slab, rows, q, span, ranks, MapGlobal{item_map}, wv % NSUB, NSUB,
+                                   build_words + wv * 2);
           }
         } else {
           for (int q = wv / NSUB; q < SW; q += NW / NSUB) {
             if ((w0 + q) * 64 >= ncols) continue;
             if (map_lds)
-              slab_build_word_m(slab, SWP, q, (w0 + q) * 64, ncols, roff, ranks, MapLds{smap}, wv % NSUB, NSUB,
+              slab_build_word_m(slab, rows, q, (w0 + q) * 64, ncols, roff, ranks, MapLds{smap}, wv % NSUB, NSUB,
                                 build_words + wv * 2);
             else
-              slab_build_word_m(slab, SWP, q, (w0 + q) * 64, ncols, roff, ranks, MapGlobal{item_map}, wv % NSUB,
+              slab_build_word_m(slab, rows, q, (w0 + q) * 64, ncols, roff, ranks, MapGlobal{item_map}, wv % NSUB,
                                 NSUB, build_words + wv * 2);
           }
         }
@@ -1336,7 +1339,7 @@
           uint64_t* base = slab + (j >> 6);
           for (int64_t r = roff[row], r1 = roff[row + 1]; r < r1; ++r) {
             const int uu = item_map[ranks[r]];
-            if (uu >= 0) atomicOr((unsigned long long*)(base + (size_t)uu * SWP), bit);
+            if (uu >= 0) atomicOr((unsigned long long*)(base + rows(uu)), bit);
           }
         }
       }
@@ -1354,13 +1357,13 @@
       if constexpr (kCls) {
         const int fl = (ra.y >> 17) & 3;
         if (!(fl & 1)) {
-          const uint4* r0 = lds4 + (size_t)(ra.z & 0xFFFF) * RS;
+          const uint4* r0 = row4(ra.z & 0xFFFF);
 #pragma unroll
           for (int q = 0; q < SW / 2; ++q) qv[q] = r0[q];
           and_prefix(qv, 1, m - 1);
         }
         if (!(fl & 2)) {
-          const uint4* rl = lds4 + (size_t)((uint32_t)ra.y >> 19) * RS;
+          const uint4* rl = row4((int)((uint32_t)ra.y >> 19));
 #pragma unroll
           for (int q = 0; q < SW / 2; ++q) {
             const uint4 v = rl[q];
@@ -1369,7 +1372,7 @@
         }
       } else {
       {
-        const uint4* r0 = lds4 + (size_t)(ra.z & 0xFFFF) * RS;
+        const uint4* r0 = row4(ra.z & 0xFFFF);
 #pragma unroll
         for (int q = 0; q < SW / 2; ++q) p[q] = r0[q];
       }
@@ -1398,7 +1401,7 @@
 #pragma unroll
           for (int x = 0; x < UE; ++x) {
             s[x] = 0;
-            r[x] = lds4 + (size_t)u16_at(rb, k + x < n_ext ? k + x : k) * RS;
+            r[x] = row4(u16_at(rb, k + x < n_ext ? k + x : k));
           }
 #pragma unroll
           for (int q = 0; q < SW / 2; ++q) {
@@ -1447,8 +1450,8 @@
   for (int q = wv / nsub; q < WT; q += NW / nsub) {
     const int64_t col0 = ((int64_t)blockIdx.x * WT + q) * 64;
     if (col0 < ncols)
-      slab_build_word_span(btile, WT, q, word_span(roff, col0, ncols), ranks, map, wv % nsub, nsub, bwords + wv * 2,
-                           0);
+      slab_build_word_span(btile, TileRows{WT}, q, word_span(roff, col0, ncols), ranks, map, wv % nsub, nsub,
+                           bwords + wv * 2);
   }
   __syncthreads();
   const int64_t w0 = (int64_t)blockIdx.x * WT;
@@ -1689,16 +1692,19 @@
 
 FA_API int fa_hip_count_slab_rec_cls(const int64_t* roff, const int32_t* ranks, const int32_t* src, int64_t ncols,
                                      const int32_t* item_map, int F1, int n_used, const int32_t* gpre,
-                                     const void* rec, int G, int C, const int32_t* wword, uint32_t* out, int sw,
+                                     const void* rec, int G, int C, const int32_t* wword, uint32_t* out, int layout,
                                      int n_wg, const uint64_t* bm, int64_t Wp, hipStream_t st,
                                      const int32_t* bm_rows, const int32_t* g_dev, int cls) {
   if ((G <= 0 && !g_dev) || C <= 0 || ncols <= 0) return 0;
-  if (g_piece_nparts > 1) cls &= ~kSlabCls;
+  const int sw = slab_layout_sw(layout), pad = slab_layout_pad(layout);
+  if (g_piece_nparts > 1 || pad > 0) cls &= ~kSlabCls;
   const int accb = slab_mode_acc_bytes(cls, wword != nullptr);
   const bool acc16 = accb == 2;
   const int64_t n_acc = slab_acc_count(C, accb);
   const bool contig = !bm && !src;
-  const size_t lds = (size_t)slab_kernel_lds(n_used, sw, slab_acc_words(n_acc), contig ? slab_map_lds(F1) : 0);
+  if (pad > kSlabPadMax || n_used < 1) return 1;
+  const size_t lds =
+      (size_t)slab_kernel_lds_pack(n_used, sw, pad, slab_acc_words(n_acc), contig ? slab_map_lds(F1) : 0);
   if (lds > 160 * 1024 - 256) return 3;
   if (g_slab_max_wg > 0) n_wg = std::min(n_wg, g_slab_max_wg);
   using KernT = void (*)(const int64_t*, const int32_t*, const int32_t*, int64_t, const int32_t*, int, int,
@@ -1714,7 +1720,7 @@
                                : accb == 2 ? (KernT)k_count_slab_rec<S, false, B, false, 2>            \
                                            : (KernT)k_count_slab_rec<S, false, B, false, 4>);
 #define FA_REC_CASE(S)                                    \
-  if (sw == S) {                                          \
+  if (sw == S && pad == 0) {                              \
     if (bm) { FA_REC_MODE(S, kBuildBM) }                  \
     else if (src) { FA_REC_MODE(S, kBuildCols) }          \
     else { FA_REC_MODE(S, kBuildContig) }                 \
@@ -1725,6 +1731,21 @@
   FA_REC_CASE(32)
 #undef FA_REC_CASE
 #undef FA_REC_MODE
+#define FA_REC_PMODE(S, B, P)                                                            \
+  kern = wword ? (KernT)k_count_slab_rec<S, true, B, false, 4, P>                        \
+         : accb == 1 ? (KernT)k_count_slab_rec<S, false, B, false, 1, P>                 \
+         : accb == 2 ? (KernT)k_count_slab_rec<S, false, B, false, 2, P>                 \
+                     : (KernT)k_count_slab_rec<S, false, B, false, 4, P>;
+#define FA_REC_PCASE(S, P)                                \
+  if (sw == S && pad == P) {                              \
+    if (bm) { FA_REC_PMODE(S, kBuildBM, P) }              \
+    else if (src) { FA_REC_PMODE(S, kBuildCols, P) }      \
+    else { FA_REC_PMODE(S, kBuildContig, P) }             \
+  }
+  FA_REC_PCASE(8, 1) FA_REC_PCASE(8, 2) FA_REC_PCASE(8, 3)
+  FA_REC_PCASE(16, 1) FA_REC_PCASE(16, 2) FA_REC_PCASE(16, 3)
+#undef FA_REC_PCASE
+#undef FA_REC_PMODE
   if (!kern) return 1;
   (void)hipFuncSetAttribute((const void*)kern, hipFuncAttributeMaxDynamicSharedMemorySize, (int)lds);
   const int flags = ((cls & kSlabDense) ? kSlabFlagDense : 0) | (acc16 ? kSlabFlagAcc16 : 0) |
diff --git a/csrc/hip/gen.hip b/csrc/hip/gen.hip
--- a/csrc/hip/gen.hip
+++ b/csrc/hip/gen.hip
@@ -724,14 +724,15 @@
 
 __global__ __launch_bounds__(1024) void k_dl_decide(const int32_t* __restrict__ cnt, int64_t* __restrict__ off,
                                                      long long* __restrict__ c, int l, double growth, int64_t c_bound,
-                                                     double lds, double accb) {
+                                                     double lds, double accb, double accb_pack) {
   if (c[kDlStop]) return;
   int64_t g = 0;
   const int64_t C = agd_block_scan<true>(cnt, off, c[kDlNl + l], &g);
   if (threadIdx.x != 0) return;
   const int64_t total = c[kDlTotal], last = c[kDlLastC];
   if (C == 0 || (double)C > growth * (double)last || C > c_bound ||
-      total + C > slab_cap(c[kDlNUsed], total + C, lds, accb)) {
+      (total + C > slab_cap(c[kDlNUsed], total + C, lds, accb) &&
+       !(accb_pack > 0.0 && slab_pack_fits(c[kDlNUsed], total + C, lds, accb_pack)))) {
     c[kDlStop] = 1;
     if (C == 0) c[kDlEmpty] = 1;
     return;
@@ -848,27 +849,69 @@
   FA_LAUNCH_RET();
 }
 
-static void dl_post(DlPost* P, const DlDesc* desc, int L, long long* ctl, const long long* ch, int F1,
-                    double accb_rule, hipStream_t st) {
+static double g_tail_accb = 0.0;
+static int g_tail_levels = 0;
+FA_API void fa_hip_set_dl_tail(double accb_pack, int end_levels) {
+  g_tail_accb = accb_pack;
+  g_tail_levels = end_levels;
+}
+
+static void dl_tail_cut(const DlDesc* desc, int* L, int Lp, long long* ch) {
+  int64_t total = 0;
+  for (int l = 0; l < Lp; ++l) total += desc[l].C;
+  ch[kDlLevels] = Lp;
+  ch[kDlTotal] = total;
+  ch[kDlLastC] = desc[Lp - 1].C;
+  ch[kDlEmpty] = 0;
+  *L = Lp;
+}
+
+static bool dl_tail(const DlPost* P, const DlDesc* desc, int* L, long long* ch, double accb_rule, double accb_pack,
+                    double lds, int* Lp_out, int* sw, int64_t* cap, int* pad) {
+  int64_t Cl[kDlMaxL], C = 0, R = 0;
+  for (int l = 0; l < *L; ++l) { Cl[l] = desc[l].C; C += desc[l].C; R += desc[l].n; }
+  const int64_t n_used = ch[kDlNUsed];
+  const int Lp = *Lp_out = slab_tail_cut(Cl, *L, n_used, lds, accb_rule);
+  if (Lp == *L) return false;
+  const bool ends = ch[kDlEmpty] || (g_tail_levels > 0 && *L == g_tail_levels);
+  if (ends && C <= P->rec_cap && C <= P->out_cap && 8 * ((R + 255) / 256) <= P->part_cap &&
+      slab_pack_width(n_used, C, lds, accb_pack, cap, pad) == 16 && C <= *cap) {
+    *sw = 16;
+    return true;
+  }
+  dl_tail_cut(desc, L, Lp, ch);
+  return false;
+}
+
+static void dl_post(DlPost* P, const DlDesc* desc, int L, long long* ctl, long long* ch, int F1,
+                    double accb_rule, double accb_pack, double lds, hipStream_t st) {
   P->done = 0;
   if (ch[kDlStop] && ch[kDlLevels] == 0) return;
   if (ch[kDlOverBound] || ch[kDlMulti] || ch[kDlEnd] || L < 1) return;
+  int64_t cap = 0;
+  int sw = 0, pad = 0, Lp = L;
+  const bool packed = accb_pack > 0.0 && dl_tail(P, desc, &L, ch, accb_rule, accb_pack, lds, &Lp, &sw, &cap, &pad);
   int64_t C = 0, R = 0;
   for (int l = 0; l < L; ++l) { C += desc[l].C; R += desc[l].n; }
   const int64_t n_used = ch[kDlNUsed];
   P->C = C;
   if (C < 1 || C > P->rec_cap || C > P->out_cap || 8 * ((R + 255) / 256) > P->part_cap) return;
-  int64_t cap = 0;
-  int sw = slab_width(n_used, C, P->lds_budget, accb_rule, &cap);
-  if (sw == 0 || C > cap) return;
   double accb = accb_rule;
-  if (!P->wword) slab_acc_upgrade(n_used, C, P->lds_budget, P->accb, &sw, &cap, &accb);
+  if (packed) {
+    accb = accb_pack;
+  } else {
+    sw = slab_width(n_used, C, P->lds_budget, accb_rule, &cap);
+    if (sw == 0 || C > cap) return;
+    if (!P->wword) slab_acc_upgrade(n_used, C, P->lds_budget, P->accb, &sw, &cap, &accb);
+  }
   P->accb = accb;
-  if (fa_hip_dl_plan(desc, L, ctl, F1, P->item_map, P->rec, C, P->part, P->part_cap, P->gpre, P->gpre_cap, sw,
-                     st) != 0)
+  if (fa_hip_dl_plan(desc, L, ctl, F1, P->item_map, P->rec, C, P->part, P->part_cap, P->gpre, P->gpre_cap,
+                     slab_layout(sw, pad), st) != 0) {
+    if (packed) dl_tail_cut(desc, &L, Lp, ch);
     return;
+  }
   (void)hipMemsetAsync(P->out, 0, 4 * (size_t)C, st);
-  P->sw = sw;
+  P->sw = slab_layout(sw, pad);
   P->cap = cap;
   P->done = 1;
   P->trim = 0;
@@ -894,9 +937,10 @@
   const bool weighted = P->wword != nullptr;
   const int64_t nacc = slab_acc_count(C, slab_acc_bytes(P->accb, weighted));
   P->n_wg = slab_workgroups(nslabs, (int64_t)P->lds_kernel,
-                            slab_kernel_lds(n_used, sw, slab_acc_words(nacc), slab_map_lds(F1)));
+                            slab_kernel_lds_pack(n_used, sw, pad, slab_acc_words(nacc), slab_map_lds(F1)));
   if (fa_hip_count_slab_rec_cls(P->roff, P->ranks, P->src, P->ncols, P->item_map, F1, (int)n_used, P->gpre, P->rec,
-                                0, (int)C, P->wword, P->out, sw, (int)P->n_wg, nullptr, 0, st, nullptr,
+                                0, (int)C, P->wword, P->out, slab_layout(sw, pad), (int)P->n_wg, nullptr, 0, st,
+                                nullptr,
                                 reinterpret_cast<const int32_t*>(ctl + kDlPiecesI32),
                                 slab_acc_mode(P->accb, weighted)) != 0)
     return;
@@ -913,6 +957,8 @@
   char* w = w0 + ws_used;
   const int LM = std::min(max_levels, kDlMaxLevels);
   const int64_t acc_max = (int64_t)(lds / accb);
+  const DlPost* const tp = static_cast<const DlPost*>(post);
+  const double accb_pack = tp && !tp->wword && F1 <= kSlabMapMaxF1 ? g_tail_accb : 0.0;
   int64_t nb = n1_bound;
   int m = (int)desc[0].m + 1;
   const int32_t* P = reinterpret_cast<const int32_t*>((intptr_t)desc[0].rows);
@@ -973,7 +1019,7 @@
 #define FA_DLR_EMIT(N) FA_DLR(true, N)
       FA_AG_NWL_SWITCH(nw, FA_DLR_CNT)
       hipLaunchKernelGGL(k_dl_decide, dim3(1), dim3(1024), 0, st, lv[l].cnt, lv[l].off, ctl, l, growth, cb, lds,
-                         accb);
+                         accb, accb_pack);
       FA_AG_NWL_SWITCH(nw, FA_DLR_EMIT)
 #undef FA_DLR_EMIT
 #undef FA_DLR_CNT
@@ -1016,6 +1062,6 @@
     d.base = desc[l - 1].base + desc[l - 1].C;
   }
   info[0] = w - w0;
-  if (post) dl_post(static_cast<DlPost*>(post), desc, L, ctl, ctl_host, F1, accb, st);
+  if (post) dl_post(static_cast<DlPost*>(post), desc, L, ctl, ctl_host, F1, accb, accb_pack, lds, st);
   FA_LAUNCH_RET();
 }
diff --git a/csrc/hip/levels.hip b/csrc/hip/levels.hip
--- a/csrc/hip/levels.hip
+++ b/csrc/hip/levels.hip
@@ -1,5 +1,6 @@
 #include "fa_hip.h"
 #include "../host/fa_dl.h"
+#include "../host/fa_slab.h"
 
 namespace fa {
 
@@ -189,7 +190,7 @@
 __global__ __launch_bounds__(64) void k_la_qsum_probe(int* out) { out[threadIdx.x] = la_qsum((int)threadIdx.x); }
 
 __global__ __launch_bounds__(64) void k_dl_lane_assign(int4* __restrict__ rec, const long long* __restrict__ c,
-                                                       int rs) {
+                                                       int sw, int pad) {
   constexpr int NW = 64 * kLaWs, NG = 4 * kLaWs;
   constexpr int kPq = kLaMaxPos / 4;
   __shared__ int4 win[3 * NW];
@@ -234,7 +235,7 @@
       const int pos = q + 4 * t;
       const bool ok = pos < R;
       const int pc = ok ? pos : 0;
-      const uint32_t sv = st[pc][(rr[t] * rs) & 15][g];
+      const uint32_t sv = st[pc][slab_row_col(sw, pad, rr[t])][g];
       const int rv = (int)rws[i1][pc];
       w[t] = ok ? sv : 0xFFFFu;
       rn[t] = ok ? rv : -1;
@@ -254,7 +255,7 @@
         const int pos = q + 4 * t;
         const int o = (int)(w[t] & 0xFFFF);
         const uint32_t nv = o == 0xFFFF ? ((uint32_t)rr[t] | (1u << 16)) : (o != rr[t] ? w[t] + (1u << 16) : w[t]);
-        if (pos < R) st[pos][(rr[t] * rs) & 15][g] = nv;
+        if (pos < R) st[pos][slab_row_col(sw, pad, rr[t])][g] = nv;
       }
       if (q == 0) {
         const int gg = g & 3, k = fill;
@@ -476,7 +477,7 @@
     const int64_t nwin = (D.w1 - D.w0) / (64 * kLaWs);
     if (nwin > 0)
       hipLaunchKernelGGL(k_dl_lane_assign, dim3((unsigned)nwin), dim3(64), 0, st, static_cast<int4*>(rec), ctl,
-                         (sw + 2) / 2);
+                         slab_layout_sw(sw), slab_layout_pad(sw));
   }
   FA_LAUNCH_RET();
 }
diff --git a/csrc/host/fa_slab.h b/csrc/host/fa_slab.h
--- a/csrc/host/fa_slab.h
+++ b/csrc/host/fa_slab.h
@@ -21,6 +21,19 @@
 FA_SLAB_FN int64_t slab_map_lds(int64_t F1) {
   return F1 <= kSlabMapMaxF1 ? ((F1 * 2 + 15) & ~(int64_t)15) : 0;
 }
+
+constexpr int kSlabPadMax = 3;
+
+FA_SLAB_FN int64_t slab_row_off(int sw, int s, int64_t u) { return u * sw * 8 + (u >> s) * 16; }
+FA_SLAB_FN int slab_row_col(int sw, int s, int u) {
+  return (int)(((uint32_t)u * (uint32_t)(sw >> 1) + ((uint32_t)u >> s)) & 15u);
+}
+FA_SLAB_FN int64_t slab_rows_bytes(int sw, int s, int64_t n) {
+  return n * sw * 8 + ((n + ((int64_t)1 << s) - 1) >> s) * 16;
+}
+FA_SLAB_FN int slab_layout(int sw, int s) { return sw | (s << 8); }
+FA_SLAB_FN int slab_layout_sw(int layout) { return layout & 0xFF; }
+FA_SLAB_FN int slab_layout_pad(int layout) { return (layout >> 8) & 0xFF; }
 
 FA_SLAB_FN int slab_width(int64_t n_used, int64_t C, double lds, double accb, int64_t* cap) {
   const int order[4] = {16, 32, 8, 4};
@@ -83,6 +96,32 @@
   return n_used * slab_row_bytes(sw) + n_acc_words * 4 + map_bytes;
 }
 
+FA_SLAB_FN int64_t slab_kernel_lds_pack(int64_t n_used, int sw, int s, int64_t n_acc_words, int64_t map_bytes) {
+  return slab_rows_bytes(sw, s, n_used) + n_acc_words * 4 + map_bytes;
+}
+
+FA_SLAB_FN int slab_pack_width(int64_t n_used, int64_t C, double lds, double accb, int64_t* cap, int* s) {
+  for (int q = 0; q <= kSlabPadMax; ++q) {
+    const int64_t c = (int64_t)((lds - (double)slab_rows_bytes(16, q, n_used)) / accb);
+    if (c >= C) { *cap = c; *s = q; return 16; }
+  }
+  *s = 0;
+  return slab_width(n_used, C, lds, accb, cap);
+}
+FA_SLAB_FN bool slab_pack_fits(int64_t n_used, int64_t C, double lds, double accb) {
+  const int64_t c = (int64_t)((lds - (double)slab_rows_bytes(16, kSlabPadMax, n_used)) / accb);
+  return C >= 1 && c >= C;
+}
+FA_SLAB_FN int slab_tail_cut(const int64_t* C, int L, int64_t n_used, double lds, double accb) {
+  int64_t total = L > 0 ? C[0] : 0;
+  int l = L > 0 ? 1 : 0;
+  for (; l < L; ++l) {
+    if (total + C[l] > slab_cap(n_used, total + C[l], lds, accb)) break;
+    total += C[l];
+  }
+  return l;
+}
+
 FA_SLAB_FN int64_t slab_workgroups(int64_t nslabs, int64_t budget, int64_t kernel_lds) {
   int64_t per_cu = budget / (kernel_lds > 1 ? kernel_lds : 1);
   per_cu = per_cu < 1 ? 1 : per_cu > 2 ? 2 : per_cu;
diff --git a/csrc/host/plan.cpp b/csrc/host/plan.cpp
--- a/csrc/host/plan.cpp
+++ b/csrc/host/plan.cpp
@@ -18,7 +18,18 @@
 FA_API int64_t fa_slab_workgroups(int64_t nslabs, int64_t n_used, int sw, int64_t n_acc, int round_acc,
                                   int64_t map_bytes, int64_t budget) {
   return slab_workgroups(nslabs, budget,
-                         slab_kernel_lds(n_used, sw, round_acc ? slab_acc_words(n_acc) : n_acc, map_bytes));
+                         slab_kernel_lds_pack(n_used, slab_layout_sw(sw), slab_layout_pad(sw),
+                                              round_acc ? slab_acc_words(n_acc) : n_acc, map_bytes));
+}
+FA_API int64_t fa_slab_row_off(int sw, int s, int64_t u) { return slab_row_off(sw, s, u); }
+FA_API int fa_slab_row_col(int sw, int s, int64_t u) { return slab_row_col(sw, s, (int)u); }
+FA_API int64_t fa_slab_rows_bytes(int sw, int s, int64_t n) { return slab_rows_bytes(sw, s, n); }
+FA_API int fa_slab_layout(int sw, int s) { return slab_layout(sw, s); }
+FA_API int fa_slab_pack_width(int64_t n_used, int64_t C, double lds, double accb, int64_t* cap, int* s) {
+  return slab_pack_width(n_used, C, lds, accb, cap, s);
+}
+FA_API int fa_slab_tail_cut(const int64_t* C, int L, int64_t n_used, double lds, double accb) {
+  return slab_tail_cut(C, L, n_used, lds, accb);
 }
 FA_API int fa_slab_acc_mode(double accb, int weighted, int64_t C, int64_t* n_acc) {
   if (n_acc) *n_acc = slab_acc_count(C, slab_acc_bytes(accb, weighted != 0));
diff --git a/fastapriori_amd/models/apriori.py b/fastapriori_amd/models/apriori.py
--- a/fastapriori_amd/models/apriori.py
+++ b/fastapriori_amd/models/apriori.py
@@ -302,6 +302,11 @@
             acc8 = 0
         accb = self._dl_accb = 1.0 if acc8 == 1 else 2.0 if TUNING.dl_acc16_bundles and unit else 4.0
         self._dl_cnt_accb = 1.0 if acc8 == 2 else accb
+        counters = 1 if self.cand_par else max(1, self.comm.world_size)
+        tail_rows = int(self.stats["n_lines"]) // counters
+        self._dl_tail_accb = 0.0
+        if TUNING.dl_tail_bundle and unit and Pm.slab_map_lds(F1) > 0 and tail_rows >= TUNING.dl_acc8_min_rows:
+            self._dl_tail_accb = 1.0 if int(TUNING.dl_acc8_bundles) else 2.0 if TUNING.dl_acc16_bundles else 4.0
         c_bound = int(lds // accb)
         st = torch.cuda.current_stream(self._dev).cuda_stream
         f2 = self._f2_dev
@@ -332,8 +337,9 @@
             b0 = self._bytes_moved()
             with roctx_range(f"dlevel{k}"), tm.phase(f"level{k}"):
                 max_lv = min(K.kDlMaxM - m0 + 1, K.kDlMaxLevels)
-                if self.cfg.max_level:
-                    max_lv = min(max_lv, self.cfg.max_level - k + 1)
+                tail_levels = 0
+                if self.cfg.max_level and self.cfg.max_level - k + 1 <= max_lv:
+                    max_lv = tail_levels = self.cfg.max_level - k + 1
                 if not TUNING.bundle_levels or k - 1 > TUNING.bundle_max_prefix:
                     max_lv = 1
                 post = TUNING.dl_post and max_lv > 1
@@ -344,7 +350,9 @@
                     self._dl_stage(S, pend)
                 with roctx_range("gen"):
                     c = Pm.dl_bundle_gen(S, P0, n_src, n_const, n_bound, m0, F1, c_bound, lds, TUNING.bundle_growth,
-                                         max_lv, st, post=post, accb=accb)
+                                         max_lv, st, post=post, accb=accb,
+                                         tail_accb=self._dl_tail_accb if post else 0.0,
+                                         tail_levels=tail_levels if max_lv > 1 else 0)
                 if c[K.kDlOverBound]:
                     raise RuntimeError(f"device bundle at level {k}: |F_{k - 1}| exceeds its bound {n_bound}")
                 if c[K.kDlEnd]:
@@ -360,11 +368,11 @@
                 Cs = S.desc["C"][:L].copy()
                 C = int(Cs.sum())
                 done = int(S.post.done) if post else 0
-                sw = int(S.post.sw) if done else 0
+                sw, pad = Pm.slab_layout_split(int(S.post.sw)) if done else (0, 0)
                 acc_bytes = int(S.post.accb) if done else int(accb)
                 if multi is not None:
                     cnt = multi[1]
-                    sw = int(Pm.LAST_LEVEL_PLAN.get("sw", 0))
+                    sw, pad = int(Pm.LAST_LEVEL_PLAN.get("sw", 0)), 0
                     acc_bytes = int(self._dl_mp_accb)
                 elif done == 2:
                     cnt = S.post_bufs["out"][:C]
@@ -382,7 +390,7 @@
                     with tm.phase("count"), roctx_range("count"):
                         v = self._count_view(db)
                         cnt = Pm.dl_count(S, plan, v["roff"], v["ranks"], v["src"], v["ncols"], F1, v["wword"])
-                    sw, acc_bytes = int(plan["sw"]), int(plan.get("accb", 4.0))
+                    sw, pad, acc_bytes = int(plan["sw"]), int(plan.get("pad", 0)), int(plan.get("accb", 4.0))
                 nz = torch.count_nonzero(cnt) if self.cand_par else None
                 with tm.phase("count"), roctx_range("count"):
                     self.comm.all_reduce_(cnt)
@@ -390,7 +398,7 @@
             hbm_rows = (db["ranks"].numel() * db["ranks"].element_size()
                         + db["roff"].numel() * db["roff"].element_size())
             pend.append(dict(k=k, L=L, m0=m0, C=Cs, rows=rows_a, cnt=cnt_a, ro=ro, co=co, hbm_rows=int(hbm_rows),
-                             n_par=S.desc["n"][:L].copy(), sw=sw, acc_bytes=acc_bytes, used=n_used,
+                             n_par=S.desc["n"][:L].copy(), sw=sw, pad=pad, acc_bytes=acc_bytes, used=n_used,
                              T=int(db["roff"].numel() - 1),
                              ms=(time.perf_counter() - t0) * 1e3, bytes=self._bytes_moved() - b0,
                              G=c[K.kDlGl:K.kDlGl + L].copy(), nz=nz))
@@ -407,6 +415,11 @@
         self.stats["device_bundles"] = len(pend)
         self.stats["device_bundle_shapes"] = [(int(p["k"]), int(p["L"]), int(p["C"].sum()), int(p["used"]),
                                                int(p["sw"]), int(p["acc_bytes"])) for p in pend]
+        self.stats["device_bundle_pads"] = [int(p["pad"]) for p in pend]
+        for p in pend:
+            self.stats.setdefault("level_info", {})[int(p["k"])] = dict(
+                kernel="slab_dev", bundled=int(p["L"]), C=int(p["C"].sum()), used=int(p["used"]), sw=int(p["sw"]),
+                pad=int(p["pad"]), acc_bytes=int(p["acc_bytes"]))
         self.stats["device_levels"] = int(sum(p["L"] for p in pend))
         return nxt
 
@@ -538,8 +551,10 @@
         Pm = ops.primitives
         m0 = k - 1
         K = Pm.dl()
-        gpre_n = n_bound * m0 if m0 > K.kDlInline else (c_bound * (m0 + 4) if m0 + K.kDlMaxLevels > K.kDlInline else 0)
-        b = S.post_buffers(F1, c_bound, n_bound + c_bound, min(gpre_n, 1 << 24))
+        tail_accb = getattr(self, "_dl_tail_accb", 0.0)
+        c_cap = max(c_bound, int(lds // tail_accb)) if tail_accb else c_bound
+        gpre_n = n_bound * m0 if m0 > K.kDlInline else (c_cap * (m0 + 4) if m0 + K.kDlMaxLevels > K.kDlInline else 0)
+        b = S.post_buffers(F1, c_cap, n_bound + c_cap, min(gpre_n, 1 << 24))
         P = S.post
         P.item_map, P.rec, P.part, P.out = (b["item_map"].data_ptr(), b["rec"].data_ptr(), b["part"].data_ptr(),
                                             b["out"].data_ptr())
@@ -675,7 +690,7 @@
                 self._level_recs.append((dict(phase="level", k=kk, candidates=int(p["C"][l]), frequent=F,
                                               ms=p["ms"] * share, groups=int(p["G"][l]), bundled_with=p["k"],
                                               bytes_reduced=int(p["bytes"] * share), kernel="slab_rec_dev",
-                                              hbm_bytes_est=hbm, slab_words=p["sw"], acc_bytes=p["acc_bytes"],
+                                              hbm_bytes_est=hbm, slab_words=p["sw"], slab_pad=p["pad"], acc_bytes=p["acc_bytes"],
                                               used_items=p["used"],
                                               rows=p["T"], _share=share),
                                          f"level{p['k']}"))
diff --git a/fastapriori_amd/ops/_native.py b/fastapriori_amd/ops/_native.py
--- a/fastapriori_amd/ops/_native.py
+++ b/fastapriori_amd/ops/_native.py
@@ -41,6 +41,12 @@
     "fa_slab_workgroups": (i64, [i64, i64, C.c_int, i64, C.c_int, i64, i64]),
     "fa_slab_acc_mode": (C.c_int, [dbl, C.c_int, i64, I64P]),
     "fa_slab_acc_upgrade": (C.c_int, [i64, i64, dbl, dbl, C.POINTER(C.c_int), I64P, C.POINTER(dbl)]),
+    "fa_slab_row_off": (i64, [C.c_int, C.c_int, i64]),
+    "fa_slab_row_col": (C.c_int, [C.c_int, C.c_int, i64]),
+    "fa_slab_rows_bytes": (i64, [C.c_int, C.c_int, i64]),
+    "fa_slab_layout": (C.c_int, [C.c_int, C.c_int]),
+    "fa_slab_pack_width": (C.c_int, [i64, i64, dbl, dbl, I64P, C.POINTER(C.c_int)]),
+    "fa_slab_tail_cut": (C.c_int, [vp, C.c_int, i64, dbl, dbl]),
     "fa_trim_estimate": (None, [vp, i64, dbl, C.c_int, C.POINTER(dbl), C.POINTER(dbl)]),
     "fa_dl_layout": (cp, [C.c_int, I64P]),
     "fa_limits": (cp, [C.c_int, I64P]),
@@ -99,6 +105,7 @@
     "fa_hip_dl_more": (C.c_int, [C.c_int, vp, i64, i64, vp, vp, dbl, C.c_int, dbl, dbl, i64, vp, vp, vp, vp]),
     "fa_hip_dl_plan": (C.c_int, [vp, C.c_int, vp, C.c_int, vp, vp, i64, vp, i64, vp, i64, C.c_int, vp]),
     "fa_hip_set_lane_deal": (None, [C.c_int]),
+    "fa_hip_set_dl_tail": (None, [dbl, C.c_int]),
     "fa_hip_set_piece_part": (C.c_int, [C.c_int, C.c_int]),
     "fa_hip_dl_gpre_need": (i64, [vp, C.c_int]),
     "fa_hip_dl_plan_window": (C.c_int, [vp, C.c_int, vp, C.c_int, vp, vp, i64, vp, i64, vp, i64, i64, i64, C.c_int,
diff --git a/fastapriori_amd/ops/primitives.py b/fastapriori_amd/ops/primitives.py
--- a/fastapriori_amd/ops/primitives.py
+++ b/fastapriori_amd/ops/primitives.py
@@ -679,6 +679,55 @@
     return int(_native.host().fa_slab_total_limit(int(n_used), float(lds), float(accb)))
 
 
+def slab_layout(sw: int, pad: int = 0) -> int:
+    return int(_native.host().fa_slab_layout(int(sw), int(pad)))
+
+
+def slab_layout_split(layout: int) -> tuple[int, int]:
+    return int(layout) & 0xFF, (int(layout) >> 8) & 0xFF
+
+
+def slab_row_off(sw: int, pad: int, u: int) -> int:
+    return int(_native.host().fa_slab_row_off(int(sw), int(pad), int(u)))
+
+
+def slab_row_col(sw: int, pad: int, u: int) -> int:
+    return int(_native.host().fa_slab_row_col(int(sw), int(pad), int(u)))
+
+
+def slab_rows_bytes(sw: int, pad: int, n: int) -> int:
+    return int(_native.host().fa_slab_rows_bytes(int(sw), int(pad), int(n)))
+
+
+def slab_pack_width(n_used: int, C: int, lds: int, accb: float = 1) -> tuple[int, int, int]:
+    cap, pad = ctypes.c_int64(0), ctypes.c_int(0)
+    sw = _native.host().fa_slab_pack_width(int(n_used), int(C), float(lds), float(accb), ctypes.byref(cap),
+                                           ctypes.byref(pad))
+    return int(sw), int(cap.value), int(pad.value)
+
+
+def slab_tail_cut(Cs, n_used: int, lds: int, accb: float = 4) -> int:
+    c = np.ascontiguousarray(Cs, dtype=np.int64)
+    return int(_native.host().fa_slab_tail_cut(c.ctypes.data, int(c.size), int(n_used), float(lds), float(accb)))
+
+
+def dl_tail_plan(Cs, n_used: int, lds: int, accb: float, cnt_accb: float, ends: bool) -> tuple[int, int, int, int]:
+    Cs = [int(c) for c in Cs]
+    Lp = slab_tail_cut(Cs, n_used, lds, accb)
+    if Lp < len(Cs) and ends:
+        sw, cap, pad = slab_pack_width(n_used, sum(Cs), lds, cnt_accb)
+        if sw == 16 and sum(Cs) <= cap:
+            return len(Cs), sw, pad, cap
+    C = sum(Cs[:Lp])
+    sw, cap = slab_width(n_used, C, lds, accb)
+    if cnt_accb < accb:
+        sw_c, cap_c, accb_c = ctypes.c_int(sw), ctypes.c_int64(cap), ctypes.c_double(accb)
+        _native.host().fa_slab_acc_upgrade(int(n_used), int(C), float(lds), float(cnt_accb), ctypes.byref(sw_c),
+                                           ctypes.byref(cap_c), ctypes.byref(accb_c))
+        sw, cap = int(sw_c.value), int(cap_c.value)
+    return Lp, sw, 0, cap
+
+
 def slab_map_lds(F1: int) -> int:
     return int(_native.host().fa_slab_map_lds(int(F1)))
 
@@ -710,10 +759,11 @@
                 sw: int, st: int, round_acc: bool, map_bytes: int, G: int = 0, g_dev=None, bm=None, bm_ld: int = 0,
                 bm_rows=None, cls: int = 0, accb: float = 4.0, sup_frac: float = 0.0) -> None:
     K = dl()
-    nslabs = ((ncols + 63) // 64 + sw - 1) // sw
+    width = slab_layout_split(sw)[0]
+    nslabs = ((ncols + 63) // 64 + width - 1) // width
     acc_mode, nacc = _slab_acc_mode(accb, wword is not None, C)
     n_wg = _slab_workgroups(nslabs, n_used, sw, nacc, round_acc, map_bytes)
-    mode = cls | (K.kSlabDense if _slab_dense(wword, sw, sup_frac) else 0) | acc_mode
+    mode = cls | (K.kSlabDense if _slab_dense(wword, width, sup_frac) else 0) | acc_mode
     _hip_call("fa_hip_count_slab_rec_cls", roff, ranks, src, ncols, item_map, F1, n_used, gpre, rec, G, C, wword,
               out, sw, n_wg, bm, bm_ld, st, bm_rows, g_dev, mode)
 
@@ -1461,7 +1511,7 @@
 
 def dl_bundle_gen(S: DeviceLevelState, P0: int, n_src: int | None, n_const: int, n_bound: int, m0: int, F1: int,
                   c_bound: int, lds: int, growth: float, max_levels: int, stream: int, post: bool = False,
-                  accb: float = 4.0) -> np.ndarray:
+                  accb: float = 4.0, tail_accb: float = 0.0, tail_levels: int = 0) -> np.ndarray:
     lib, K = _native.hip(), dl()
     info = np.zeros(2, dtype=np.int64)
     for _ in range(6):
@@ -1481,6 +1531,7 @@
             return c.copy()
         S.post.done = 0
         lane_deal(lib, S.rows_hint)
+        lib.fa_hip_set_dl_tail(float(tail_accb) if post else 0.0, int(tail_levels))
         rc = lib.fa_hip_dl_more(F1, _p(S.ws), S.ws.numel(), int(S.info[0]), _p(S.ctl), _p(S.ctl_h), float(growth),
                                 int(max_levels), float(lds), float(accb), int(c_bound), S.desc.ctypes.data,
                                 info.ctypes.data,
@@ -1502,7 +1553,7 @@
 
 
 def dl_plan(S: DeviceLevelState, L: int, F1: int, n_used: int, C: int, lds: int, dev, accb: float = 4.0,
-            cnt_accb: float | None = None) -> dict:
+            cnt_accb: float | None = None, pad: int = 0) -> dict:
     st = torch.cuda.current_stream(dev).cuda_stream
     sw, cap = slab_width(n_used, C, lds, accb)
     if sw == 0 or C > cap:
@@ -1521,9 +1572,11 @@
     gpre = torch.empty(max(gn, 1), dtype=_I32, device=dev)
     lane_deal(lib, S.rows_hint)
     _native.check(lib.fa_hip_dl_plan(S.desc.ctypes.data, L, _p(S.ctl), F1, _p(item_map), _p(rec), C,
-                                     _p(part), part.numel(), _p(gpre), gpre.numel(), sw, st), "fa_hip_dl_plan")
+                                     _p(part), part.numel(), _p(gpre), gpre.numel(), slab_layout(sw, pad), st),
+                  "fa_hip_dl_plan")
     out = torch.zeros(C, dtype=_I32, device=dev)
-    return dict(sw=sw, cap=cap, item_map=item_map, rec=rec, out=out, n_used=n_used, C=C, gpre=gpre, accb=accb)
+    return dict(sw=sw, pad=pad, cap=cap, item_map=item_map, rec=rec, out=out, n_used=n_used, C=C, gpre=gpre,
+                accb=accb)
 
 
 def dl_count_multipass(S: DeviceLevelState, F1: int, n_used: int, C: int, lds: int, roff, ranks, src, ncols: int,
@@ -1659,7 +1712,8 @@
     P, b = S.post, S.post_bufs
     C = int(P.C)
     out = b["out"][:C]
-    return dict(sw=int(P.sw), cap=int(P.cap), item_map=b["item_map"], rec=b["rec"], out=out, n_used=n_used, C=C,
+    sw, pad = slab_layout_split(int(P.sw))
+    return dict(sw=sw, pad=pad, cap=int(P.cap), item_map=b["item_map"], rec=b["rec"], out=out, n_used=n_used, C=C,
                 gpre=b["gpre"], accb=float(P.accb))
 
 
@@ -1669,11 +1723,11 @@
     item_map, rec, out = plan["item_map"], plan["rec"], plan["out"]
     _slab_count(roff=_p(roff), ranks=_p(ranks), src=_p(src), ncols=ncols, item_map=_p(item_map), F1=F1,
                 n_used=n_used, gpre=_p(plan.get("gpre")), rec=_p(rec), g_dev=_p(S.ctl) + 8 * dl().kDlPiecesI32, C=C,
-                wword=_p(wword), out=_p(out), sw=sw, st=st, round_acc=True, map_bytes=slab_map_lds(F1),
-                accb=plan.get("accb", 4.0))
+                wword=_p(wword), out=_p(out), sw=slab_layout(sw, plan.get("pad", 0)), st=st, round_acc=True,
+                map_bytes=slab_map_lds(F1), accb=plan.get("accb", 4.0))
     LAST_LEVEL_PLAN.clear()
     LAST_LEVEL_PLAN.update(kernel="slab_dev", rows=int(roff.numel() - 1), used=n_used, sw=sw, cap=cap, passes=1,
-                           pieces=-1, slab_reads=0, m=-1, C=C)
+                           pieces=-1, slab_reads=0, m=-1, C=C, pad=int(plan.get("pad", 0)))
     return out
 
 
diff --git a/fastapriori_amd/tuning.py b/fastapriori_amd/tuning.py
--- a/fastapriori_amd/tuning.py
+++ b/fastapriori_amd/tuning.py
@@ -30,6 +30,7 @@
     dl_acc16_bundles: bool = False
     dl_acc8_bundles: int = 2
     dl_acc8_min_rows: int = 1 << 20
+    dl_tail_bundle: bool = True
     mp_window_items: bool = True
     window_trim: bool = True
     window_trim_est_frac: float = 0.95
```

After: 904,100 itemsets/s (median of 6 runs). 3.6% higher.
